# abhineet123/MTF

Measured on AMD Instinct MI355X. Metric: LK iters/sec (warp+grad+Hessian), ESM+SSD+Homography 200x200, higher is better.
Workload: dtype f64; 1 GPU; ESM+SSD+Homography 200x200, 64 independent targets per GPU, full mode, solve+update on device; targets_per_gpu=64, n_pix=40000, channels=1, mode=full, frame=1024x1024 float32, parallelism=replicas x1

## Files before the change

### mtf_amd/csrc/api_track.hip

```cpp
#include "mtfhip_api_internal.h"

extern "C" {

int loop_upload_slab(mtfhip_batch *b, hipStream_t st, bool keep_ncc) {
	const size_t Bt = (size_t)b->B;
	std::memcpy(b->h_stage_b + 45 * sizeof(double) * Bt, b->h_stage_a + 45 * sizeof(double) * Bt, 9 * sizeof(double) * Bt);
	fill_stage(b, b->h_stage_b, nullptr, 1, true);
	if (b->h_stage_b_dev) launch_ingest_host(b->h_stage_b_dev, b->d_slab, b->slab_bytes, st, keep_ncc ? 37 * sizeof(double) * Bt : 0, keep_ncc ? 8 * sizeof(double) * Bt : 0);
	else if (keep_ncc) return fail(MTFHIP_ERR_LOGIC, "track: a held template-initialisation record needs the host-visible staging buffer");
	else HIP_TRY(hipMemcpyAsync(b->d_slab, b->h_stage_b, b->slab_bytes, hipMemcpyHostToDevice, st));
	b->warps_dirty = false;
	return MTFHIP_OK;
}
int loop_lm_state(mtfhip_batch *b, const mtfhip_sm_desc *sm, hipStream_t st, double **lm) {
	if (!b->d_lm) HIP_TRY(hipMalloc(&b->d_lm, sizeof(double) * kLmStride * (size_t)b->B));
	std::vector<double> lm0((size_t)kLmStride * b->B, 0.0);
	for (int t = 0; t < b->B; ++t) lm0[(size_t)kLmStride * t + 1] = sm->lm_delta_init;
	HIP_TRY(hipMemcpyAsync(b->d_lm, lm0.data(), sizeof(double) * lm0.size(), hipMemcpyHostToDevice, st));
	HIP_TRY(hipStreamSynchronize(st));
	*lm = b->d_lm;
	return MTFHIP_OK;
}
bool loop_all_stopped(const mtfhip_sm_desc *sm, int max_passes, int it, const int *d_flags, int n, hipStream_t on, std::vector<int> &h_flags, hipError_t *err) {
	if (!(sm->epsilon > 0) || (it + 1) % 8 != 0 || it + 1 >= max_passes) return false;
	h_flags.resize(n);
	hipError_t e = hipMemcpyAsync(h_flags.data(), d_flags, sizeof(int) * n, hipMemcpyDeviceToHost, on);
	if (e == hipSuccess) e = hipStreamSynchronize(on);
	if (e != hipSuccess) { if (err) *err = e; return false; }
	for (int v : h_flags) if (v) return false;
	return true;
}
int loop_read_back(mtfhip_batch *b, hipStream_t st, unsigned long long pub_seq, int *n_iters, double *corners, const char **h_res) {
	*h_res = b->h_pub;
	if (pub_seq) TRY(wait_host_flag(b, pub_seq));
	else if (b->h_pub_dev) {
		const unsigned long long seq = ++b->acc_seq;
		launch_publish_host(b->d_slab, b->h_pub_dev, b->slab_bytes, b->d_fin_count, b->h_flag_dev, seq, st);
		TRY(wait_host_flag(b, seq));
	} else {
		HIP_TRY(hipMemcpyAsync(b->h_stage_b, b->d_slab, b->slab_bytes, hipMemcpyDeviceToHost, st));
		HIP_TRY(hipStreamSynchronize(st));
		*h_res = b->h_stage_b;
	}
	const size_t Bt = (size_t)b->B;
	const double *p = reinterpret_cast<const double *>(*h_res);
	const double *w = p, *s = p + 9 * Bt, *cr = p + 17 * Bt;
	const int *iters = reinterpret_cast<const int *>(*h_res + b->slab_dbl_bytes) + Bt;
	for (int t = 0; t < b->B; ++t) {
		std::memcpy(b->th[t].warp.m, w + 9 * t, sizeof(double) * 9);
		std::memcpy(b->th[t].state, s + 8 * t, sizeof(double) * 8);
		std::memcpy(b->th[t].corners, cr + 8 * t, sizeof(double) * 8);
		if (n_iters) n_iters[t] = iters[t];
		if (corners) std::memcpy(corners + 8 * t, cr + 8 * t, sizeof(double) * 8);
	}
	return MTFHIP_OK;
}
static int iclk_one_launch_max_pix() {
	static const int v = std::getenv("MTFHIP_ICLK_ONE_LAUNCH_MAX") ? std::atoi(std::getenv("MTFHIP_ICLK_ONE_LAUNCH_MAX")) : 4 * kBlock;
	return v < kIclkTrackMaxPix ? v : kIclkTrackMaxPix;
}
bool iclk_one_launch(const mtfhip_batch *b, const mtfhip_sm_desc *sm) {
	return b->C == 1 && !intensity_mapped(b) && sm->sm == MTFHIP_SM_ICLK && (sm->hess_type == 0 || (sm->hess_type == 2 && b->desc.am == MTFHIP_AM_SSD)) &&
		b->N <= iclk_one_launch_max_pix();
}

static int track_chunk(const mtfhip_batch *b, const mtfhip_sm_desc *sm, const FusedArgs &fa) {
	const char *env_px = std::getenv("MTFHIP_TRACK_CHUNK_PX");
	if (!env_px && !(fa.mode == 1 && fa.materialize)) return b->B;
	const double chunk_px = env_px ? std::atof(env_px) : 2.6e6;
	int chunk = (int)(chunk_px / (double)b->N);
	if (chunk < 1) chunk = 1;
	if (chunk >= b->B || sm->max_iters == 1) return b->B;
	const int n_chunks = (b->B + chunk - 1) / chunk;
	return (b->B + n_chunks - 1) / n_chunks;
}
static int track_queues(const mtfhip_batch *b, const FusedArgs &fa) {
	const char *e_want = std::getenv("MTFHIP_TRACK_STREAMS");
	const int want = e_want ? std::atoi(e_want) : 2;
	if (want < 2 || b->B < 2 || b->d_trace) return 1;
	if (!fa.materialize && want < 12) return 1;
	static const double min_rows = std::getenv("MTFHIP_TRACK_STREAMS_MIN_ROWS") ? std::atof(std::getenv("MTFHIP_TRACK_STREAMS_MIN_ROWS")) : 0.5e6;
	if ((double)b->B * b->N < min_rows && want < 12) return 1;
	return std::min(std::min(want % 10, 4), b->B);
}
int mtfhip_batch_track_targets_per_launch(mtfhip_batch *b, const mtfhip_sm_desc *sm) {
	FLUSH(b);
	if (check_sm(b, sm, "track_targets_per_launch") != MTFHIP_OK) return 0;
	if (iclk_one_launch(b, sm)) return b->B;
	FusedArgs fa;
	if (fused_args(b, sm, fa) != MTFHIP_OK) return 0;
	const int chunk = track_chunk(b, sm, fa), nq = track_queues(b, fa);
	return nq >= 2 ? std::min(chunk, (b->B + nq - 1) / nq) : chunk;
}
int mtfhip_batch_track_queues(mtfhip_batch *b, const mtfhip_sm_desc *sm) {
	FLUSH(b);
	if (check_sm(b, sm, "track_queues") != MTFHIP_OK) return 0;
	if (b->desc.am == MTFHIP_AM_MI) return 1;
	if (iclk_one_launch(b, sm)) return 1;
	FusedArgs fa;
	if (fused_args(b, sm, fa) != MTFHIP_OK) return 0;
	return track_queues(b, fa);
}

static bool track_defers_materialisation(const mtfhip_batch *b, const mtfhip_sm_desc *sm, const FusedArgs &fa, int so_term, bool resume, bool use_step) {
	const char *e = std::getenv("MTFHIP_TRACK_DEFER_MAT");
	if (e && e[0] == '0') return false;
	if (!fa.materialize) return false;
	if (fa.mode == 2) return false;
	if (sm->max_iters < 3) return false;
	if (sm->leven_marq) return false;
	if (b->d_trace) return false;
	if (so_term >= 0) return false;
	if (b->desc.am != MTFHIP_AM_SSD && b->desc.am != MTFHIP_AM_NCC) return false;
	if (b->C != 1) return false;
	if (use_step) return false;
	if (resume) return false;
	return true;
}

static int track_core(mtfhip_batch *b, const mtfhip_sm_desc *sm, int *n_iters, double *corners, bool slab_uploaded, bool resume = false, bool region_mode = false);
static void persist_decomposition(const mtfhip_batch *b, int &nblk, int &rows) {
	fused_decomposition(b->N, b->B, nblk, rows);
	const int per_target = b->ctx->n_cus / b->B;
	if (per_target >= 1 && nblk > per_target) {
		const int total_rows = (b->N + kBlock - 1) / kBlock;
		rows = (total_rows + per_target - 1) / per_target;
		nblk = (total_rows + rows - 1) / rows;
	}
	static const int forced = std::getenv("MTFHIP_PERSIST_NBLK") ? std::atoi(std::getenv("MTFHIP_PERSIST_NBLK")) : 0;
	if (forced > 0 && forced < nblk) {
		const int total_rows = (b->N + kBlock - 1) / kBlock;
		rows = (total_rows + forced - 1) / forced;
		nblk = (total_rows + rows - 1) / rows;
	}
}
static int ensure_persist_words(mtfhip_batch *b, hipStream_t st) {
	if (b->d_persist) return MTFHIP_OK;
	HIP_TRY(hipMalloc(&b->d_persist, 2 * sizeof(int) * (size_t)b->B));
	HIP_TRY(hipMemsetAsync(b->d_persist, 0, 2 * sizeof(int) * (size_t)b->B, st));
	return MTFHIP_OK;
}
static unsigned long long persist_timeout_ticks() {
	const char *e = std::getenv("MTFHIP_PERSIST_TIMEOUT_US");
	const double us = e ? std::atof(e) : 20000.0;
	return (unsigned long long)(us * 100.0);
}
static bool persist_fits(const mtfhip_batch *b, const mtfhip_sm_desc *sm, const FusedArgs &fa) {
	const char *e = std::getenv("MTFHIP_PERSIST");
	if (!(e && e[0] == '1') || !b->persist_ok || fa.materialize || b->ctx->n_cus <= 0 || b->B > b->ctx->n_cus || !b->h_pub_dev) return false;
	if (b->C != 1) return false;
	if (intensity_mapped(b)) return false;
	if (b->B > 8) return false;
	if (sm->max_iters < 2) return false;
	int nblk, rows;
	persist_decomposition(b, nblk, rows);
	return (long)nblk * b->B <= b->ctx->n_cus && nblk <= b->nblk_max;
}
static int lscv_after_track(mtfhip_batch *b, int rc) {
	if (rc == MTFHIP_OK && b && (b->desc.am == MTFHIP_AM_LSCV || b->desc.am == MTFHIP_AM_LRSCV)) b->lscv_first_iter = 0;
	return rc;
}
int mtfhip_batch_track(mtfhip_batch *b, const mtfhip_sm_desc *sm, int *n_iters, double *corners) {
	if (sm && alk_sm(sm->sm)) return alk_track(b, sm, n_iters, corners);
	return lscv_after_track(b, track_core(b, sm, n_iters, corners, false));
}

const bool g_track_dbg_timing = std::getenv("MTFHIP_TRACK_DEBUG_TIMING") != nullptr;
static thread_local std::chrono::steady_clock::time_point g_track_dbg_t[3];
int track_region_impl(mtfhip_batch *b, const mtfhip_sm_desc *sm, const double *region_corners, int *n_iters, double *corners, const mtfhip_grid_desc *grid) {
	if (!b || !sm || !region_corners) return fail(MTFHIP_ERR_INVALID_ARG, "track_region: NULL argument");
	TRY(track_validate(b, sm));
	const bool folded = !region_refreshes(sm);
	const bool dbg = g_track_dbg_timing;
	const char *e_gf = std::getenv("MTFHIP_GRID_FUSED");
	const bool fused_ok = !(e_gf && e_gf[0] == '0');
	const bool region_mode = fused_ok && folded && b->desc.am != MTFHIP_AM_MI && !sm->leven_marq && iclk_one_launch(b, sm) && second_order_term(sm, b->desc.am) < 0 &&
		b->h_stage_a_dev && b->h_pub_dev;
	const auto t0 = std::chrono::steady_clock::now();
	static thread_local std::vector<double> patches;
	bool layout_later = false;
	if (grid) {
		const char *e_ld = std::getenv("MTFHIP_GRID_LAYOUT_DEV");
		layout_later = region_mode && b->desc.ssm != MTFHIP_SSM_HOMOGRAPHY && !grid->dyn_patch_size && !(e_ld && e_ld[0] == '0');
		if (layout_later) {
			M3 Wr;
			if (!rect_to_quad(-0.5, -0.5, 0.5, 0.5, region_corners, Wr)) return fail(MTFHIP_ERR_INVALID_ARG, "grid_layout: degenerate region corners");
			b->deferred_gdesc = *grid;
			std::memcpy(b->deferred_region, region_corners, sizeof(b->deferred_region));
			std::memcpy(b->deferred_region_map, Wr.m, sizeof(b->deferred_region_map));
		} else {
			patches.resize(8 * (size_t)b->B);
			TRY(mtfhip_grid_layout(grid, region_corners, nullptr, patches.data()));
			region_corners = patches.data();
		}
	}
	{
		const int rs = set_region_core(b, layout_later ? nullptr : region_corners, sm, folded, region_mode, layout_later);
		if (rs != MTFHIP_OK) { b->deferred_layout = false; b->deferred_template_check = false; set_corners_finish_deferred(b); return rs; }
	}
	const auto t1 = std::chrono::steady_clock::now();
	const int r = lscv_after_track(b, track_core(b, sm, n_iters, corners, folded, false, region_mode));
	set_corners_finish_deferred(b);
	if (dbg) {
		const auto t2 = std::chrono::steady_clock::now();
		static double acc1 = 0, acc2 = 0, acc3 = 0, acc4 = 0, acc5 = 0, acc6 = 0; static int n = 0;
		auto us = [](std::chrono::steady_clock::time_point a, std::chrono::steady_clock::time_point c) { return std::chrono::duration<double, std::micro>(c - a).count(); };
		acc1 += us(t0, t1); acc2 += us(t1, t2); acc3 += us(t1, g_track_dbg_t[0]); acc4 += us(g_track_dbg_t[0], g_track_dbg_t[1]); acc5 += us(g_track_dbg_t[1], g_track_dbg_t[2]); acc6 += us(g_track_dbg_t[2], t2);
		if (++n % 100 == 0) {
			std::fprintf(stderr, "[track_region] set_region %.1f us, track %.1f us = before the launch %.1f + launch call %.1f + deferred host half %.1f + wait and copy-out %.1f (mean of 100)\n",
				acc1 / 100, acc2 / 100, acc3 / 100, acc4 / 100, acc5 / 100, acc6 / 100);
			acc1 = acc2 = acc3 = acc4 = acc5 = acc6 = 0;
		}
	}
	return r;
}
int mtfhip_batch_track_region(mtfhip_batch *b, const mtfhip_sm_desc *sm, const double *region_corners, int *n_iters, double *corners) {
	return track_region_impl(b, sm, region_corners, n_iters, corners, nullptr);
}

int track_validate(mtfhip_batch *b, const mtfhip_sm_desc *sm) {
	TRY(check_sm(b, sm, "track"));
	if (sm->max_iters <= 0) return fail(MTFHIP_ERR_INVALID_ARG, "track: max_iters must be positive");
	const int so_term = second_order_term(sm, b->desc.am);
	if (b->desc.am == MTFHIP_AM_MI && so_term >= 0 && b->desc.mi_n_bins != 8)
		return fail(MTFHIP_ERR_NOT_IMPLEMENTED, "track: second-order MI Hessians with other than 8 bins go through the per-function entry points");
	if (so_term >= 0 && b->C != 1) return fail(MTFHIP_ERR_NOT_IMPLEMENTED, "track: second-order Hessians of the multi-channel models use the per-function entry points");
	if (so_term > 0 && so_term != 4 && !b->init_pix_hess) return fail(MTFHIP_ERR_LOGIC, "track: init_template was run without sec_ord_hess");
	if (!b->init_pix_vals) return fail(MTFHIP_ERR_LOGIC, "track before init_template");
	if ((b->desc.am == MTFHIP_AM_LSCV || b->desc.am == MTFHIP_AM_LRSCV) && b->lscv_once && sm->leven_marq && sm->sm == MTFHIP_SM_FCLK)
		return fail(MTFHIP_ERR_NOT_IMPLEMENTED, "track: %s once_per_frame with Levenberg-Marquardt FCLK is not available on the device loop (use the per-function entry points)",
			intensity_mapped_name(b));
	return need_image(b);
}
static int track_loop_one_launch(mtfhip_batch *b, const mtfhip_sm_desc *sm, const TrackState &ts, const TrackCtx &cx, unsigned long long &pub_seq) {
	hipStream_t st = b->ctx->stream;
	const BatchView bv = b->view();
	const bool fb_fused = b->fb_fused_req;
	TimedScope tsc(b->ctx, fb_fused ? "grid_fb" : "iclk_track");
	HostPublish pub{nullptr, 0, 0, nullptr, nullptr, 0, 0};
	if (b->h_pub_dev) {
		pub_seq = ++b->acc_seq;
		pub = HostPublish{b->h_pub_dev, b->slab_dbl_bytes, b->B, b->d_fin_count, b->h_flag_dev, pub_seq, publish_fenced()};
	}
	RegionIngest rg{};
	if (cx.region_mode) {
		const double *stage = reinterpret_cast<const double *>(b->h_stage_a_dev);
		rg = region_geometry(b);
		rg.corners = stage + 17 * (size_t)b->B; rg.ncc = stage + 37 * (size_t)b->B;
		rg.d_ncc = b->d_ncc; rg.d_w0 = b->d_w0; rg.d_init_corners_hm = b->d_init_corners_hm;
		if (b->deferred_layout) region_deferred_layout(b, rg);
	}
	const bool dbg_t = g_track_dbg_timing;
	if (dbg_t) g_track_dbg_t[0] = std::chrono::steady_clock::now();
	if (fb_fused) {
		if (cx.region_mode || !pub.host) return fail(MTFHIP_ERR_LOGIC, "track: the one-launch forward-backward frame takes the plain mode with a host record");
		if (!launch_grid_fb(bv, b->ctx->img, b->ctx->prev, *sm, ts, b->d_h0inv, b->d_ncc, b->norm_mult, b->norm_add, b->desc.grad_eps, pub,
				GridFbOut{b->h_fb_dev, b->d_fb, b->fb_fused_reinit ? 1 : 0}, region_geometry(b), st))
			return fail(MTFHIP_ERR_LOGIC, "track: patch too large for the one-launch forward-backward frame");
	} else
		launch_iclk_track(bv, b->ctx->img, *sm, ts, b->d_h0inv, b->d_ncc, b->norm_mult, b->norm_add, b->math_mode == MTFHIP_MATH_FAST, pub, rg, st);
	if (dbg_t) g_track_dbg_t[1] = std::chrono::steady_clock::now();
	set_corners_finish_deferred(b);
	if (dbg_t) g_track_dbg_t[2] = std::chrono::steady_clock::now();
	return MTFHIP_OK;
}
static int track_loop_persist(mtfhip_batch *b, const mtfhip_sm_desc *sm, const FusedArgs &fa, const TrackState &ts, const TrackCtx &cx) {
	hipStream_t st = b->ctx->stream;
	TRY(ensure_persist_words(b, st));
	int nblk_p, rows_p;
	persist_decomposition(b, nblk_p, rows_p);
	FusedArgs fp = fa;
	fp.rows_per_block = rows_p;
	PersistState ps{b->d_persist, reinterpret_cast<unsigned *>(b->d_persist) + b->B, b->persist_gen, persist_timeout_ticks()};
	b->persist_gen += (unsigned)cx.max_passes + 1u;
	TimedScope tsc(b->ctx, "track_persist");
	launch_track_persist(b->view(), b->ctx->img, fp, *sm, ts, b->d_partials, nblk_p, ps, cx.max_passes, st);
	return MTFHIP_OK;
}

struct ChunkRun { BatchView bc; FusedArgs fc, fl; TrackState tc, tl; int nblk_c, t0, nt; double *part; hipStream_t s; bool done; };
static void track_chunk_runs(mtfhip_batch *b, const FusedArgs &fa, const TrackState &ts, int chunk, int n_streams, bool defer, std::vector<ChunkRun> &runs) {
	const BatchView bv = b->view();
	const bool ncc = b->desc.am == MTFHIP_AM_NCC;
	const size_t RL = ncc ? NCC_ACC_COUNT : ACC_COUNT;
	for (int t0 = 0; t0 < b->B; t0 += chunk) {
		const int nt = std::min(chunk, b->B - t0);
		BatchView bc = bv;
		bc.B = nt;
		for (int i = 0; i < MTFHIP_BUF_COUNT; ++i)
			if (bc.buf[i]) bc.buf[i] += (size_t)t0 * b->per_target[i];
		bc.warps += 9 * (size_t)t0; bc.states += 8 * (size_t)t0;
		FusedArgs fc = fa;
		fc.active = fa.active + t0;
		if (fc.w0) fc.w0 += 9 * (size_t)t0;
		TrackState tc{ts.acc + (size_t)t0 * RL, ts.h0 + (size_t)t0 * 64, ts.corners + 8 * (size_t)t0,
			ts.init_corners_hm + 12 * (size_t)t0, ts.active + t0, ts.n_iters + t0, ncc ? ts.ncc + 8 * (size_t)t0 : nullptr,
			ncc ? ts.ncc_tm + 52 * (size_t)t0 : nullptr, 0, ts.lm ? ts.lm + (size_t)kLmStride * t0 : nullptr, nullptr,
			ts.trace ? ts.trace + (size_t)t0 * ts.trace_cap * kTraceStride : nullptr, ts.trace_cap,
			ts.h_extra ? ts.h_extra + (size_t)t0 * b->S * b->S : nullptr, ts.h_extra_scale, ts.fast_finish};
		int nblk_c; { int rows; fused_decomposition(b->N, nt, nblk_c, rows, MTFHIP_SLOTS / n_streams); fc.rows_per_block = rows; }
		if (nblk_c > b->nblk_max) { int rows; fused_decomposition(b->N, nt, nblk_c, rows); fc.rows_per_block = rows; }
		if (fc.rows_per_block < kGridRegenMinRows) fc.grid_regen = 0;
		double *part = b->d_partials + (size_t)t0 * b->nblk_max * RL;
		static const bool serialize = std::getenv("MTFHIP_TRACK_SERIALIZE") && std::getenv("MTFHIP_TRACK_SERIALIZE")[0] == '1';
		const int q = serialize ? n_streams - 1 : (int)(runs.size() % (size_t)n_streams);
		FusedArgs fl = fc;
		fl.materialize = 0; fl.fast_math = 0; fl.grid_regen = 0;
		if (defer) { tc.warp_last = b->d_last_ws + 9 * (size_t)t0; tc.state_last = b->d_last_ws + 9 * (size_t)b->B + 8 * (size_t)t0; tc.need_mat = b->d_need_mat + t0; }
		TrackState tl = tc;
		tl.lean_pass = 1;
		runs.push_back(ChunkRun{bc, fc, fl, tc, tl, nblk_c, t0, nt, part, q == n_streams - 1 ? b->ctx->stream : b->ctx->extra_streams[q], false});
	}
}
static void track_materialise_stopped(mtfhip_batch *b, const ChunkRun &r) {
	BatchView bm = r.bc;
	bm.warps = r.tc.warp_last; bm.states = r.tc.state_last;
	FusedArgs fm = r.fc;
	fm.active = r.tc.need_mat;
	TimedScope tsc(b->ctx, "fused_lk", r.s);
	launch_fused_ssd(bm, b->ctx->img, fm, r.part, r.nblk_c, r.s, nullptr, nullptr);
}
static int track_open_queues(mtfhip_batch *b, int n_streams, double &phase_frac) {
	mtfhip_ctx *c = b->ctx;
	if (n_streams >= 2) {
		if (!c->ev_fork && hipEventCreateWithFlags(&c->ev_fork, hipEventDisableTiming) != hipSuccess) { (void)hipGetLastError(); n_streams = 1; }
		for (int q = 0; q + 1 < n_streams; ++q)
			if (!c->extra_streams[q] && (hipStreamCreateWithFlags(&c->extra_streams[q], hipStreamNonBlocking) != hipSuccess ||
				hipEventCreateWithFlags(&c->ev_join[q], hipEventDisableTiming) != hipSuccess)) { (void)hipGetLastError(); n_streams = 1; break; }
	}
	const char *e_ph = std::getenv("MTFHIP_TRACK_PHASE");
	phase_frac = e_ph ? std::atof(e_ph) : 0.35;
	if (n_streams == 2 && phase_frac > 0) {
		if (!c->d_phase && hipMalloc(&c->d_phase, sizeof(unsigned long long) * 4) != hipSuccess) { (void)hipGetLastError(); c->d_phase = nullptr; }
	}
	return n_streams;
}
struct QueueJoin {
	mtfhip_ctx *c; int n; bool joined = false;
	~QueueJoin() { if (!joined) for (int q = 0; q + 1 < n; ++q) if (c->extra_streams[q]) (void)hipStreamSynchronize(c->extra_streams[q]); }
};
static bool track_takes_step(const mtfhip_batch *b, const FusedArgs &fa, int so_term, int n_streams) {
	const char *e_st = std::getenv("MTFHIP_STEP");
	const char *e_mx = std::getenv("MTFHIP_STEP_MAX_TARGETS");
	const int max_t = e_mx ? std::atoi(e_mx) : 8;
	return (e_st && e_st[0] == '1') && so_term < 0 && !intensity_mapped(b) && n_streams == 1 && b->B <= max_t && track_step_available(b->view(), fa);
}
static int track_chunk_pass(mtfhip_batch *b, const mtfhip_sm_desc *sm, const FusedArgs &fa, const TrackCtx &cx, const ChunkRun &r, int it, bool lean, bool use_step,
	const PhaseCtl &pc) {
	if (use_step) {
		TimedScope tsc(b->ctx, "track_step", r.s);
		launch_track_step(r.bc, b->ctx->img, r.fc, *sm, r.tc, r.part, r.nblk_c, b->d_persist + r.t0, r.s);
		return MTFHIP_OK;
	}
	if (b->desc.am == MTFHIP_AM_SCV) TRY(scv_enqueue(b, r.bc, r.t0, r.fc.active, 0, r.s));
	if (b->desc.am == MTFHIP_AM_LSCV && (!b->lscv_once || it == 0)) TRY(lscv_enqueue(b, r.bc, r.t0, r.fc.active, 0, r.s));
	RscvMap rm;
	if (b->desc.am == MTFHIP_AM_RSCV) TRY(rscv_enqueue(b, r.bc, r.t0, r.fc.active, r.fc, r.s, &rm));
	LrscvMap lm;
	if (b->desc.am == MTFHIP_AM_LRSCV && (!b->lscv_once || it == 0)) TRY(lrscv_enqueue(b, r.bc, r.t0, r.fc.active, r.fc, r.s, &lm));
	{
		TimedScope tsc(b->ctx, "fused_lk", r.s);
		launch_fused_ssd(r.bc, b->ctx->img, lean ? r.fl : r.fc, r.part, r.nblk_c, r.s, &rm, &lm);
	}
	if (cx.so_term >= 0) {
		TimedScope tsc(b->ctx, "second_order", r.s);
		launch_second_order_ssd(r.bc, b->ctx->img, cx.so_term, fa.chained, b->d0_variant, fa.grad_eps, b->hess_eps, b->norm_mult, b->norm_add,
			b->d_d2_part + (size_t)r.t0 * cx.nb2 * 64, cx.nb2, b->d_d2_out + (size_t)r.t0 * b->S * b->S, r.s, 1,
			b->desc.am == MTFHIP_AM_NCC ? SecondOrderNcc{r.part, r.nblk_c, r.tc.ncc} : SecondOrderNcc{nullptr, 0, nullptr});
	}
	TimedScope tsc(b->ctx, "finish_track", r.s);
	launch_finish_track(r.bc, *sm, lean ? r.tl : r.tc, r.part, r.nblk_c, r.s, pc);
	return MTFHIP_OK;
}
static int track_loop_chunked(mtfhip_batch *b, const mtfhip_sm_desc *sm, const FusedArgs &fa, const TrackState &ts, const TrackCtx &cx) {
	hipStream_t st = b->ctx->stream;
	int chunk = track_chunk(b, sm, fa);
	double phase_frac;
	const int n_streams = track_open_queues(b, track_queues(b, fa), phase_frac);
	if (n_streams == 2 && phase_frac > 0 && b->ctx->d_phase) HIP_TRY(hipMemsetAsync(b->ctx->d_phase, 0, sizeof(unsigned long long) * 4, st));
	static const double stagger_env = std::getenv("MTFHIP_TRACK_STAGGER_US") ? std::atof(std::getenv("MTFHIP_TRACK_STAGGER_US")) : -1.0;
	double stagger_us = stagger_env;
	if (stagger_env < 0) stagger_us = 0.25 * ((double)b->B * b->N * 130.0 / 6.5e6 + 8.0) * (2.0 / n_streams);
	const bool use_step = track_takes_step(b, fa, cx.so_term, n_streams);
	if (use_step) TRY(ensure_persist_words(b, st));
	const bool defer = track_defers_materialisation(b, sm, fa, cx.so_term, cx.resume, use_step);
	if (defer) {
		if (!b->d_last_ws) HIP_TRY(hipMalloc(&b->d_last_ws, sizeof(double) * 17 * (size_t)b->B));
		if (!b->d_need_mat) HIP_TRY(hipMalloc(&b->d_need_mat, sizeof(int) * (size_t)b->B));
		HIP_TRY(hipMemsetAsync(b->d_need_mat, 0, sizeof(int) * (size_t)b->B, st));
	}
	if (n_streams >= 2) {
		const int part_sz = (b->B + n_streams - 1) / n_streams;
		if (chunk > part_sz) chunk = part_sz;
		HIP_TRY(hipEventRecord(b->ctx->ev_fork, st));
		for (int q = 0; q + 1 < n_streams; ++q) HIP_TRY(hipStreamWaitEvent(b->ctx->extra_streams[q], b->ctx->ev_fork, 0));
	}
	std::vector<ChunkRun> runs;
	track_chunk_runs(b, fa, ts, chunk, n_streams, defer, runs);
	const auto dbg_t0 = std::chrono::steady_clock::now();
	QueueJoin queue_join{b->ctx, n_streams};
	std::vector<int> h_flags;
	for (size_t g0 = 0; g0 < runs.size(); g0 += (size_t)n_streams) {
		const size_t g1 = std::min(runs.size(), g0 + (size_t)n_streams);
		for (int it = 0; it < cx.max_passes; ++it) {
			bool all_done = true;
			const bool lean = defer && it + 1 < cx.max_passes;
			for (size_t k = g0; k < g1; ++k) {
				ChunkRun &r = runs[k];
				if (r.done) continue;
				if (n_streams >= 2 && it == 0 && k > g0 && stagger_us > 0) launch_queue_delay(stagger_us * (double)(k - g0), r.s);
				PhaseCtl pc{nullptr, nullptr, 0.0};
				if (n_streams == 2 && phase_frac > 0 && b->ctx->d_phase) {
					const int qi = (int)((k - g0) & 1);
					pc = PhaseCtl{b->ctx->d_phase + qi, b->ctx->d_phase + (1 - qi), phase_frac};
				}
				TRY(track_chunk_pass(b, sm, fa, cx, r, it, lean, use_step, pc));
				if (loop_all_stopped(sm, cx.max_passes, it, r.tc.active, r.nt, r.s, h_flags)) r.done = true;
				all_done = all_done && r.done;
			}
			if (all_done) break;
		}
		if (defer && sm->epsilon > 0)
			for (size_t k = g0; k < g1; ++k) track_materialise_stopped(b, runs[k]);
	}
	if (g_track_dbg_timing)
		std::fprintf(stderr, "[track] %d queues, %d passes enqueued in %.1f us\n", n_streams, cx.max_passes,
			std::chrono::duration<double, std::micro>(std::chrono::steady_clock::now() - dbg_t0).count());
	for (int q = 0; q + 1 < n_streams; ++q) {
		HIP_TRY(hipEventRecord(b->ctx->ev_join[q], b->ctx->extra_streams[q]));
		HIP_TRY(hipStreamWaitEvent(st, b->ctx->ev_join[q], 0));
	}
	queue_join.joined = true;
	return MTFHIP_OK;
}

static int track_core(mtfhip_batch *b, const mtfhip_sm_desc *sm, int *n_iters, double *corners, bool slab_uploaded, bool resume, bool region_mode) {
	FLUSH_AM(b);
	TRY(begin_entry(b));
	TRY(track_validate(b, sm));
	TrackCtx cx{second_order_term(sm, b->desc.am), (sm->leven_marq && sm->sm == MTFHIP_SM_FCLK) ? 2 * sm->max_iters : sm->max_iters, 0, resume, region_mode};
	hipStream_t st = b->ctx->stream;
	const bool mi = b->desc.am == MTFHIP_AM_MI, ncc = b->desc.am == MTFHIP_AM_NCC;
	const bool one_launch = !mi && !sm->leven_marq && iclk_one_launch(b, sm) && cx.so_term < 0;
	FusedArgs fa;
	if (!one_launch && !mi) TRY(fused_args(b, sm, fa));
	else { fa.materialize = 0; fa.mode = 2; fa.active = nullptr; fa.rows_per_block = 1; fa.j0_recompute = 0; fa.inline_warp = 0; fa.fast_math = 0; fa.grid_regen = 0; fa.w0 = nullptr; }
	const bool fresh = b->fresh_reinit && one_launch && !region_mode && !slab_uploaded && !resume && b->h_pub_dev && b->d_trace == nullptr;
	b->fresh_reinit = false;
	if (!slab_uploaded && !fresh) TRY(loop_upload_slab(b, st, b->hold_init_pull && b->init_mirror_seq != 0));
	else b->warps_dirty = false;
	fa.active = b->d_active;
	if (ncc && !one_launch && !b->d_ncc_tm) return fail(MTFHIP_ERR_LOGIC, "track before init_template");
	TrackState ts{b->d_acc, b->d_h0, b->d_corners, b->d_init_corners_hm, b->d_active, b->d_iters, ncc ? b->d_ncc : nullptr, ncc ? b->d_ncc_tm : nullptr, 0, nullptr, nullptr,
		b->d_trace, b->trace_cap};
	ts.fresh_reset = fresh ? 1 : 0;
	if (b->d_trace && !resume) HIP_TRY(hipMemsetAsync(b->d_trace, 0, sizeof(double) * kTraceStride * (size_t)b->trace_cap * b->B, st));
	if (mi && b->d_trace) ts.f_ext = b->d_mi_f;
	if (sm->leven_marq) {
		if (resume) ts.lm = b->d_lm;
		else TRY(loop_lm_state(b, sm, st, &ts.lm));
		if (mi) ts.f_ext = b->d_mi_f;
	}
	if (cx.so_term >= 0) {
		cx.nb2 = simple_blocks_per_target(b->N);
		TRY(ensure_second_order_scratch(b));
		ts.h_extra = b->d_d2_out; ts.h_extra_scale = (cx.so_term == 1 || (cx.so_term == 4 && sm->sm == MTFHIP_SM_ESM && sm->hess_type == 2)) ? 0.5 : 1.0;
	}
	{
		const char *e = std::getenv("MTFHIP_FAST_FINISH");
		const bool enabled = !(e && e[0] == '0');
		ts.fast_finish = (enabled && b->math_mode == MTFHIP_MATH_FAST && !ncc && !mi && cx.so_term < 0) ? 1 : 0;
	}
	unsigned long long pub_seq = 0;
	bool persisted = false;
	if (mi) TRY(track_loop_mi(b, sm, ts, cx));
	else if (one_launch) TRY(track_loop_one_launch(b, sm, ts, cx, pub_seq));
	else if ((persisted = cx.so_term < 0 && persist_fits(b, sm, fa))) TRY(track_loop_persist(b, sm, fa, ts, cx));
	else TRY(track_loop_chunked(b, sm, fa, ts, cx));
	const char *h_res;
	TRY(loop_read_back(b, st, pub_seq, n_iters, corners, &h_res));
	const int *act = reinterpret_cast<const int *>(h_res + b->slab_dbl_bytes), *iters = act + b->B;
	if (region_mode)
		for (int t = 0; t < b->B; ++t)
			if (iters[t] < 0) return fail(MTFHIP_ERR_INVALID_ARG, "track_region: degenerate corners for target %d", t);
	if (persisted) {
		bool cut = false;
		for (int t = 0; t < b->B; ++t) cut = cut || act[t] != 0;
		if (cut) {
			b->persist_ok = false;
			HIP_TRY(hipStreamSynchronize(st));
			HIP_TRY(hipMemsetAsync(b->d_persist, 0, 2 * sizeof(int) * (size_t)b->B, st));
			return track_core(b, sm, n_iters, corners, true, true);
		}
	}
	if (!mi) {
		b->it_valid = fa.materialize;
		b->dit_valid = b->jt_valid = fa.materialize && fa.mode != 2;
	}
	loop_done(b);
	return MTFHIP_OK;
}

int mtfhip_batch_track_trace(mtfhip_batch *b, int max_passes) {
	if (!b || max_passes < 0) return fail(MTFHIP_ERR_INVALID_ARG, "track_trace: invalid argument");
	HIP_TRY(hipStreamSynchronize(b->ctx->stream));
	if (b->d_trace) { (void)hipFree(b->d_trace); b->d_trace = nullptr; }
	b->trace_cap = max_passes;
	if (max_passes > 0) {
		HIP_TRY(hipMalloc(&b->d_trace, sizeof(double) * kTraceStride * (size_t)max_passes * b->B));
		HIP_TRY(hipMemsetAsync(b->d_trace, 0, sizeof(double) * kTraceStride * (size_t)max_passes * b->B, b->ctx->stream));
	}
	return MTFHIP_OK;
}
int mtfhip_batch_track_trace_read(mtfhip_batch *b, double *dst) {
	if (!b || !dst) return fail(MTFHIP_ERR_INVALID_ARG, "track_trace_read: NULL argument");
	if (!b->d_trace) return fail(MTFHIP_ERR_LOGIC, "track_trace_read: tracing is off (mtfhip_batch_track_trace)");
	HIP_TRY(hipMemcpyAsync(dst, b->d_trace, sizeof(double) * kTraceStride * (size_t)b->trace_cap * b->B, hipMemcpyDeviceToHost, b->ctx->stream));
	HIP_TRY(hipStreamSynchronize(b->ctx->stream));
	return MTFHIP_OK;
}

}
```

### mtf_amd/csrc/kernels_fused.hip

```cpp
#include "mtfhip_finish_device.h"
#include "mtfhip_fused_device.h"

namespace mtfhip {

template <int SSM, bool CHAINED, int MODE, bool MAT>
__global__ __launch_bounds__(kBlock, MTFHIP_FUSED_WAVES) void k_fused_ssd(BatchView bv, ImgView im, FusedArgs fa, double *partials, int nblk) {
	fused_lk_body<MTFHIP_AM_SSD, SSM, CHAINED, MODE, MAT>(bv, im, fa, partials, nblk);
}
template <int SSM, bool CHAINED, int MODE, bool MAT>
__global__ __launch_bounds__(kBlock, MTFHIP_FUSED_WAVES) void k_fused_ncc(BatchView bv, ImgView im, FusedArgs fa, double *partials, int nblk) {
	fused_lk_body<MTFHIP_AM_NCC, SSM, CHAINED, MODE, MAT>(bv, im, fa, partials, nblk);
}
template <int AM, int SSM, int MODE, bool CHAINED>
__global__ __launch_bounds__(kBlock, MTFHIP_FAST_WAVES) void k_fused_fast(BatchView bv, ImgView im, FusedArgs fa, double *partials, int nblk) {
	fused_lk_body<AM, SSM, CHAINED, MODE, false, true>(bv, im, fa, partials, nblk);
}


__global__ __launch_bounds__(256) void k_finish_track(BatchView bv, mtfhip_sm_desc sm, TrackState ts,
	const double *partials, int nblk, PhaseCtl pc) {
	if (ts.fast_finish) finish_track_fast_body(bv, sm, ts, partials, nblk, blockIdx.x);
	else finish_track_body(bv, sm, ts, partials, nblk, blockIdx.x);
	if (pc.mine && blockIdx.x == 0 && threadIdx.x == 0) {
		const unsigned long long prev = ld_coh(pc.mine), other = ld_coh(pc.other);
		unsigned long long now = wall_clock64();
		if (prev && other && now > prev && now - prev < 50000ull) {
			const unsigned long long min_lag = (unsigned long long)((double)(now - prev) * pc.frac);
			while (now > other && now - other < min_lag) { __builtin_amdgcn_s_sleep(8); now = wall_clock64(); }
		}
		st_coh(pc.mine, now);
	}
}


__global__ __launch_bounds__(64) void k_finish_track_mi(BatchView bv, mtfhip_sm_desc sm, TrackState ts, int sum_std, int gmode,
	const double *mi_H, const double *gpart, int ng, double *rows) {
	const int t = blockIdx.x, lane = threadIdx.x, S = bv.S, B = bv.B;
	const double *Hs = mi_H + 64 * (size_t)t, *H2 = mi_H + 80 * (size_t)B + 64 * (size_t)t;
	double *row = rows + (size_t)t * ACC_COUNT;
	__shared__ double gs[16];
	if (lane < 16) gs[lane] = column_sum(gpart + (size_t)t * ng * 16 + lane, ng, 16);
	if (lane < ACC_COUNT - 36) row[36 + lane] = 0.0;
	const int a = lane >> 3, c = lane & 7;
	if (a <= c) {
		double hv = 0.0;
		if (c < S) { hv = Hs[c * S + a]; if (sum_std) hv = 0.5 * (hv + H2[c * S + a]); }
		row[ACC_H + a * 8 - (a * (a - 1)) / 2 + (c - a)] = -hv;
	}
	__syncthreads();
	if (lane < S) {
		const double gt = gs[lane], g0 = gs[8 + lane];
		row[ACC_G + lane] = gmode == 0 ? g0 : (gmode == 1 ? gt : (gmode == 2 ? 2.0 * gt : gt - g0));
	}
	__syncthreads();
	finish_track_body(bv, sm, ts, rows, 1, t);
}


void launch_fused_ssd(const BatchView &bv, const ImgView &im, const FusedArgs &fa, double *partials, int nblk,
	hipStream_t st, const RscvMap *rm, const LrscvMap *lm) {
	const bool mapped = bv.am == MTFHIP_AM_RSCV ? (rm && rm->map) : (bv.am == MTFHIP_AM_LRSCV && lm && lm->map);
	const FusedKey k = fused_select(FUSED_ROUTE_LOOP, bv.am, bv.C, bv.ssm, fa.mode, fa.chained, fa.materialize, fa.fast_math, mapped);
	if (!k.served) return;
	if (k.am == MTFHIP_AM_RSCV) { launch_fused_rscv(bv, im, fa, partials, nblk, *rm, st); return; }
	if (k.am == MTFHIP_AM_LRSCV) { launch_fused_lrscv(bv, im, fa, partials, nblk, *lm, st); return; }
	if (k.mc) { launch_fused_mc(bv, im, fa, partials, nblk, st); return; }
	const dim3 g = grid2(nblk, bv.B);
	const bool launched = fused_visit<FusedUnit<FUSED_ROUTE_LOOP, false, MTFHIP_AM_SSD, MTFHIP_AM_NCC>>(k, [&](auto AM, auto SSM, auto CH, auto MD, auto MAT, auto FAST) {
		if constexpr (FAST())
			MTFHIP_LAUNCH((k_fused_fast<AM(), SSM(), MD(), CH()>), g, dim3(kBlock), 0, st, bv, im, fa, partials, nblk);
		else if constexpr (AM() == MTFHIP_AM_NCC)
			MTFHIP_LAUNCH((k_fused_ncc<SSM(), CH(), MD(), MAT()>), g, dim3(kBlock), 0, st, bv, im, fa, partials, nblk);
		else {
			const size_t tab = MAT() && fa.grid_regen ? sizeof(double2) * (size_t)(fa.g_resx + fa.g_resy) : 0;
			MTFHIP_LAUNCH((k_fused_ssd<SSM(), CH(), MD(), MAT()>), g, dim3(kBlock), tab, st, bv, im, fa, partials, nblk);
		}
	});
	if (!launched) note_launch_error(hipErrorInvalidDeviceFunction, __FILE__, __LINE__);
}
void launch_finish_track(const BatchView &bv, const mtfhip_sm_desc &sm, const TrackState &ts, const double *partials,
	int nblk, hipStream_t st, PhaseCtl pc) {
	MTFHIP_LAUNCH(k_finish_track, dim3(bv.B), dim3(nblk > 8 ? 256 : (bv.am == MTFHIP_AM_NCC ? 128 : 64)), 0, st, bv, sm, ts, partials, nblk, pc);
}

void launch_finish_track_mi(const BatchView &bv, const mtfhip_sm_desc &sm, const TrackState &ts, int sum_std, int gmode,
	const double *mi_H, const double *gpart, int ng, double *rows, hipStream_t st) {
	MTFHIP_LAUNCH(k_finish_track_mi, dim3(bv.B), dim3(64), 0, st, bv, sm, ts, sum_std, gmode, mi_H, gpart, ng, rows);
}

__global__ void k_kernarg_probe(BatchView bv, ImgView im, FusedArgs fa, double *out) {
	const char *kernarg = (const char *)__builtin_amdgcn_kernarg_segment_ptr();
	const double *kw = reinterpret_cast<const double *>(kernarg + sizeof(BatchView) + sizeof(ImgView) + offsetof(FusedArgs, iw));
	if (threadIdx.x < 17) out[threadIdx.x] = kw[threadIdx.x];
	if (threadIdx.x == 17) out[17] = (double)(bv.B + im.w + fa.mode);
}
bool kernarg_layout_verified(hipStream_t st) {
	static int state = -1;
	if (state >= 0) return state == 1;
	state = 0;
	double *d_out = nullptr;
	if (hipMalloc(&d_out, sizeof(double) * 18) != hipSuccess) { (void)hipGetLastError(); return false; }
	BatchView bv{}; ImgView im{}; FusedArgs fa{};
	bv.B = 1; im.w = 2; fa.mode = 3; fa.inline_warp = 1;
	for (int q = 0; q < 9; ++q) fa.iw[q] = 0.5 + 1.25 * q;
	for (int q = 0; q < 8; ++q) fa.is[q] = -3.0 - 0.75 * q;
	double h[18] = {0};
	hipLaunchKernelGGL(k_kernarg_probe, dim3(1), dim3(64), 0, st, bv, im, fa, d_out);
	bool ok = hipGetLastError() == hipSuccess && hipMemcpyAsync(h, d_out, sizeof(h), hipMemcpyDeviceToHost, st) == hipSuccess &&
		hipStreamSynchronize(st) == hipSuccess;
	(void)hipFree(d_out);
	for (int q = 0; ok && q < 9; ++q) ok = h[q] == fa.iw[q];
	for (int q = 0; ok && q < 8; ++q) ok = h[9 + q] == fa.is[q];
	state = ok ? 1 : 0;
	return ok;
}

#ifdef MTFHIP_FIN_TRACE
void debug_fin_trace(unsigned long long *out) { (void)hipMemcpyFromSymbol(out, HIP_SYMBOL(g_fin_trace), sizeof(unsigned long long) * 16); }
#endif
}
```

### mtf_amd/csrc/kernels_interface.hip

```cpp
#include "mtfhip_device.h"
#include "mtfhip_grid_device.h"

namespace mtfhip {


struct SlabIngest { const uint4 *src; uint4 *dst; unsigned n16; const unsigned *src_tail; unsigned *dst_tail; unsigned n_tail; };
__global__ __launch_bounds__(kBlock) void k_init_grid(BatchView bv, const double *w0_all, int resx, int resy,
	double lo_x, double lo_y, double hi_x, double hi_y, int force_unit_z, SlabIngest ing, int write_curr) {
	const int t = blockIdx.y;
	if (ing.src) {
		const unsigned i = (blockIdx.y * gridDim.x + blockIdx.x) * kBlock + threadIdx.x;
		if (i < ing.n16) ing.dst[i] = ing.src[i];
		if (i < ing.n_tail) ing.dst_tail[i] = ing.src_tail[i];
	}
	const Warp9 W = load_warp(w0_all + 9 * t);
	double2 *ip = reinterpret_cast<double2 *>(bv.buf[MTFHIP_BUF_INIT_PTS]) + (size_t)t * bv.NP;
	double2 *cp = reinterpret_cast<double2 *>(bv.buf[MTFHIP_BUF_CURR_PTS]) + (size_t)t * bv.NP;
	double *iz = bv.buf[MTFHIP_BUF_INIT_Z] + (size_t)t * bv.NP;
	double *cz = bv.buf[MTFHIP_BUF_CURR_Z] + (size_t)t * bv.NP;
	double2 *ih = reinterpret_cast<double2 *>(bv.buf[MTFHIP_BUF_INIT_HXY]) + (size_t)t * bv.NP;
	double2 *ch = reinterpret_cast<double2 *>(bv.buf[MTFHIP_BUF_CURR_HXY]) + (size_t)t * bv.NP;
	for (int i = blockIdx.x * kBlock + threadIdx.x; i < bv.NP; i += gridDim.x * kBlock) {
		const int col = i % resx, row = i / resx;
		const double nx = lattice_coord(col, resx, lo_x, hi_x, (hi_x - lo_x) / (resx - 1)), ny = lattice_coord(row, resy, lo_y, hi_y, (hi_y - lo_y) / (resy - 1));
// ... 154 lines not shown
__global__ __launch_bounds__(kBlock) void k_img_grad_mc(int NP, int C, ImgView im, const double *pts_all, const double *gp_all,
	double *grad_all, double eps, double pix_mult) {
	const int t = blockIdx.y, P = NP * C;
	double *grad = grad_all + (size_t)t * P * 2;
	const double mult = pix_mult / (2 * eps);
	for (int q = blockIdx.x * kBlock + threadIdx.x; q < P; q += gridDim.x * kBlock) {
		const int i = q / C, ch = q % C;
		double ix, dx, iy, dy;
		if (gp_all) {
			const double2 *g = reinterpret_cast<const double2 *>(gp_all + ((size_t)t * NP + i) * 8);
			ix = pix_val_mc(im, g[0].x, g[0].y, ch); dx = pix_val_mc(im, g[1].x, g[1].y, ch);
			iy = pix_val_mc(im, g[2].x, g[2].y, ch); dy = pix_val_mc(im, g[3].x, g[3].y, ch);
		} else {
			const double2 p = (reinterpret_cast<const double2 *>(pts_all) + (size_t)t * NP)[i];
			ix = pix_val_mc(im, p.x + eps, p.y, ch); dx = pix_val_mc(im, p.x - eps, p.y, ch);
			iy = pix_val_mc(im, p.x, p.y + eps, ch); dy = pix_val_mc(im, p.x, p.y - eps, ch);
		}
		grad[q] = (ix - dx) * mult;
		grad[P + q] = (iy - dy) * mult;
	}
}

__global__ __launch_bounds__(kBlock) void k_pix_jacobian(BatchView bv, int variant, const double *grad_all, double *J_all) {
	const int t = blockIdx.y, N = bv.N, S = bv.S, NP = bv.NP, C = bv.C;
	const Warp9 W = load_warp(bv.warps + 9 * t);
	const double *st = bv.states + 8 * t;
	const double2 *ip = reinterpret_cast<const double2 *>(bv.buf[MTFHIP_BUF_INIT_PTS]) + (size_t)t * NP;
	const double2 *cp = reinterpret_cast<const double2 *>(bv.buf[MTFHIP_BUF_CURR_PTS]) + (size_t)t * NP;
	const double *cz = bv.buf[MTFHIP_BUF_CURR_Z] + (size_t)t * NP;
	const double *grad = grad_all + (size_t)t * N * 2;
	double *J = J_all + (size_t)t * N * S;
	for (int i = blockIdx.x * kBlock + threadIdx.x; i < N; i += gridDim.x * kBlock) {
		const int pt = C == 1 ? i : i / C;
		double2 p0 = ip[pt];
		double x = p0.x, y = p0.y;
		double gx = grad[i], gy = grad[N + i];
		double r[8];
		if (bv.ssm == MTFHIP_SSM_HOMOGRAPHY) {
			if (variant == MTFHIP_JAC_INIT) {
				hom_row(r, gx, gy, x, y, x, y);
			} else if (variant == MTFHIP_JAC_PIX) {
				double2 c = cp[pt];
				double inv_d = 1.0 / cz[pt];
				hom_row(r, gx * inv_d, gy * inv_d, x, y, c.x, c.y);
			} else if (variant == MTFHIP_JAC_WARPED) {
				double2 c = cp[pt];
				double inv_det = 1.0 / cz[pt];
				double dwx_dx = (W.m[0] - W.m[6] * c.x), dwx_dy = (W.m[1] - W.m[7] * c.x);
				double dwy_dx = (W.m[3] - W.m[6] * c.y), dwy_dy = (W.m[4] - W.m[7] * c.y);
				double Ix = (dwx_dx * gx + dwy_dx * gy) * inv_det;
				double Iy = (dwx_dy * gx + dwy_dy * gy) * inv_det;
				hom_row(r, Ix, Iy, x, y, x, y);
			} else {
				double2 c = cp[pt];
				double a = (W.m[0] - W.m[6] * c.x), b = (W.m[1] - W.m[7] * c.x);
				double cc = (W.m[3] - W.m[6] * c.y), d = (W.m[4] - W.m[7] * c.y);
				double inv_factor = 1.0 / (a * d - b * cc);
				double Ix = (d * gx - cc * gy) * inv_factor;
				double Iy = (a * gy - b * gx) * inv_factor;
				hom_row(r, Ix, Iy, x, y, c.x, c.y);
			}
		} else {
			double a = st[2] + 1, b = st[3], c = st[4], d = st[5] + 1;
			double Ixx = gx * x, Ixy = gx * y, Iyy = gy * y, Iyx = gy * x;
			if (variant == MTFHIP_JAC_INIT || variant == MTFHIP_JAC_PIX) {
				r[0] = gx; r[1] = gy; r[2] = Ixx; r[3] = Ixy; r[4] = Iyx; r[5] = Iyy;
			} else if (variant == MTFHIP_JAC_WARPED) {
				r[0] = gx * a + gy * c; r[1] = gx * b + gy * d;
				r[2] = Ixx * a + Iyx * c; r[3] = Ixy * a + Iyy * c;
				r[4] = Ixx * b + Iyx * d; r[5] = Ixy * b + Iyy * d;
			} else {
				double inv_det = 1.0 / (a * d - b * c);
				r[0] = (gx * d - gy * c) * inv_det; r[1] = (gy * a - gx * b) * inv_det;
				r[2] = (Ixx * d - Iyx * c) * inv_det; r[3] = (Ixy * d - Iyy * c) * inv_det;
				r[4] = (Iyx * a - Ixx * b) * inv_det; r[5] = (Iyy * a - Ixy * b) * inv_det;
			}
		}
		for (int s = 0; s < S; ++s) J[(size_t)s * N + i] = r[s];
	}
}


__global__ __launch_bounds__(kBlock) void k_mean_jacobian(const double *a, const double *b, double *o, size_t n) {
	for (size_t i = (size_t)blockIdx.x * kBlock + threadIdx.x; i < n; i += (size_t)gridDim.x * kBlock)
		o[i] = (a[i] + b[i]) / 2.0;
}

__global__ __launch_bounds__(kBlock) void k_negate(const double *a, double *o, size_t n) {
	for (size_t i = (size_t)blockIdx.x * kBlock + threadIdx.x; i < n; i += (size_t)gridDim.x * kBlock) o[i] = -a[i];
}



__global__ __launch_bounds__(kBlock) void k_ssd_residual(BatchView bv, double *partials, int nblk) {
	__shared__ double lds[4 * 1];
	const int t = blockIdx.y, N = bv.N;
	const double *It = bv.buf[MTFHIP_BUF_IT] + (size_t)t * N;
	const double *I0 = bv.buf[MTFHIP_BUF_I0] + (size_t)t * N;
	double *r = bv.buf[MTFHIP_BUF_DF_DI0] + (size_t)t * N;
	double acc[1] = {0.0};
	for (int i = blockIdx.x * kBlock + threadIdx.x; i < N; i += nblk * kBlock) {
		double d = It[i] - I0[i];
		r[i] = d;
		acc[0] = fma(d, d, acc[0]);
	}
	block_reduce_store<1>(acc, partials + ((size_t)t * nblk + blockIdx.x) * ACC_COUNT + ACC_RR, lds);
}

__global__ __launch_bounds__(kBlock) void k_gemv(int N, int S, const double *v1_all, const double *J1_all,
	const double *v2_all, const double *J2_all, int sum_mode, double *partials, int nblk) {
	__shared__ double lds[4 * 16];
	const int t = blockIdx.y;
	const double *v1 = v1_all + (size_t)t * N, *J1 = J1_all + (size_t)t * N * S;
	const double *v2 = v2_all ? v2_all + (size_t)t * N : nullptr;
	const double *J2 = J2_all ? J2_all + (size_t)t * N * S : nullptr;
	double acc[16];
#pragma unroll
	for (int k = 0; k < 16; ++k) acc[k] = 0.0;
	for (int i = blockIdx.x * kBlock + threadIdx.x; i < N; i += nblk * kBlock) {
		double a = v1[i];
		double b = v2 ? v2[i] : 0.0;
#pragma unroll
		for (int s = 0; s < kMaxS; ++s) {
			if (s < S) {
				double j1 = J1[(size_t)s * N + i];
				if (J2 && sum_mode) {
					acc[s] = fma(a, j1 + J2[(size_t)s * N + i], acc[s]);
				} else {
					acc[s] = fma(a, j1, acc[s]);
					if (J2) acc[8 + s] = fma(b, J2[(size_t)s * N + i], acc[8 + s]);
				}
			}
		}
	}
	double *dst = partials + ((size_t)t * nblk + blockIdx.x) * ACC_COUNT;
	__shared__ double outv[16];
	block_reduce_store<16>(acc, outv, lds);
	__syncthreads();
	if (threadIdx.x < 8) dst[ACC_G + threadIdx.x] = outv[threadIdx.x];
	else if (threadIdx.x < 16) dst[ACC_G2 + threadIdx.x - 8] = outv[threadIdx.x];
}

__global__ __launch_bounds__(kBlock) void k_gram(int N, int S, const double *J_all, double *partials, int nblk) {
	__shared__ double lds[4 * 36];
	const int t = blockIdx.y;
	const double *J = J_all + (size_t)t * N * S;
	double acc[36];
#pragma unroll
	for (int k = 0; k < 36; ++k) acc[k] = 0.0;
	for (int i = blockIdx.x * kBlock + threadIdx.x; i < N; i += nblk * kBlock) {
		double r[kMaxS];
#pragma unroll
		for (int s = 0; s < kMaxS; ++s) r[s] = s < S ? J[(size_t)s * N + i] : 0.0;
		int k = 0;
#pragma unroll
		for (int a = 0; a < kMaxS; ++a)
#pragma unroll
			for (int b = a; b < kMaxS; ++b) { acc[k] = fma(r[a], r[b], acc[k]); ++k; }
	}
	block_reduce_store<36>(acc, partials + ((size_t)t * nblk + blockIdx.x) * ACC_COUNT + ACC_H, lds);
}

enum { NCC_I0_MEAN = 0, NCC_C = 1, NCC_IT_MEAN = 2, NCC_B = 3, NCC_F = 4, NCC_GMEAN = 5, NCC_SC = 8 };

__global__ __launch_bounds__(kBlock) void k_vec_sum(int N, const double *v_all, double *partials, int nblk) {
	__shared__ double lds[4];
	const int t = blockIdx.y;
	const double *v = v_all + (size_t)t * N;
	double acc[1] = {0.0};
	for (int i = blockIdx.x * kBlock + threadIdx.x; i < N; i += nblk * kBlock) acc[0] += v[i];
	block_reduce_store<1>(acc, partials + ((size_t)t * nblk + blockIdx.x) * ACC_COUNT + ACC_RR, lds);
}
__global__ __launch_bounds__(kBlock) void k_ncc_centered(BatchView bv, const double *sc_all, double *partials, int nblk) {
	__shared__ double lds[4 * 4];
	__shared__ double outv[4];
	const int t = blockIdx.y, N = bv.N;
	const double *I0 = bv.buf[MTFHIP_BUF_I0] + (size_t)t * N, *It = bv.buf[MTFHIP_BUF_IT] + (size_t)t * N;
	const double m0 = sc_all[t * NCC_SC + NCC_I0_MEAN], mt = sc_all[t * NCC_SC + NCC_IT_MEAN];
	double acc[4] = {0, 0, 0, 0};
	for (int i = blockIdx.x * kBlock + threadIdx.x; i < N; i += nblk * kBlock) {
		const double a0 = I0[i] - m0, at = It[i] - mt;
		acc[0] = fma(a0, at, acc[0]); acc[1] = fma(at, at, acc[1]); acc[2] = fma(a0, a0, acc[2]);
	}
	block_reduce_store<4>(acc, outv, lds);
	__syncthreads();
	if (threadIdx.x < 3) partials[((size_t)t * nblk + blockIdx.x) * ACC_COUNT + ACC_G + threadIdx.x] = outv[threadIdx.x];
}
__global__ __launch_bounds__(kBlock) void k_ncc_grad(BatchView bv, const double *sc_all, int curr, double *out_all,
	double *partials, int nblk) {
	__shared__ double lds[4];
	const int t = blockIdx.y, N = bv.N;
	const double *I0 = bv.buf[MTFHIP_BUF_I0] + (size_t)t * N, *It = bv.buf[MTFHIP_BUF_IT] + (size_t)t * N;
	double *out = out_all + (size_t)t * N;
	const double *sc = sc_all + t * NCC_SC;
	const double m0 = sc[NCC_I0_MEAN], c = sc[NCC_C], mt = sc[NCC_IT_MEAN], b = sc[NCC_B], f = sc[NCC_F];
	double acc[1] = {0.0};
	for (int i = blockIdx.x * kBlock + threadIdx.x; i < N; i += nblk * kBlock) {
		const double i0c_c = (I0[i] - m0) / c, itc_b = (It[i] - mt) / b;
		const double v = curr ? (i0c_c - f * itc_b) / b : (itc_b - f * i0c_c) / c;
		out[i] = v;
		acc[0] += v;
	}
	block_reduce_store<1>(acc, partials + ((size_t)t * nblk + blockIdx.x) * ACC_COUNT + ACC_RR, lds);
}
__global__ __launch_bounds__(kBlock) void k_sub_mean(int N, double *v_all, const double *sc_all) {
	const int t = blockIdx.y;
	double *v = v_all + (size_t)t * N;
	const double m = sc_all[t * NCC_SC + NCC_GMEAN];
	for (int i = blockIdx.x * kBlock + threadIdx.x; i < N; i += gridDim.x * kBlock) v[i] -= m;
}
__global__ __launch_bounds__(kBlock) void k_col_sum(int N, int S, const double *J_all, double *partials, int nblk) {
	__shared__ double lds[4 * 8];
	__shared__ double outv[8];
	const int t = blockIdx.y;
	const double *J = J_all + (size_t)t * N * S;
	double acc[8] = {0, 0, 0, 0, 0, 0, 0, 0};
	for (int i = blockIdx.x * kBlock + threadIdx.x; i < N; i += nblk * kBlock) {
#pragma unroll
		for (int s = 0; s < kMaxS; ++s)
			if (s < S) acc[s] += J[(size_t)s * N + i];
	}
	block_reduce_store<8>(acc, outv, lds);
	__syncthreads();
	if (threadIdx.x < 8) partials[((size_t)t * nblk + blockIdx.x) * ACC_COUNT + ACC_G + threadIdx.x] = outv[threadIdx.x];
}
__global__ __launch_bounds__(kBlock) void k_ncc_hess(BatchView bv, const double *sc_all, const double *colmean_all,
	const double *J_all, double *partials, int nblk) {
	__shared__ double lds[4 * 52];
	__shared__ double outv[52];
	const int t = blockIdx.y, N = bv.N, S = bv.S;
	const double *J = J_all + (size_t)t * N * S;
	const double *I0 = bv.buf[MTFHIP_BUF_I0] + (size_t)t * N, *It = bv.buf[MTFHIP_BUF_IT] + (size_t)t * N;
	const double *sc = sc_all + t * NCC_SC, *cm = colmean_all + t * 8;
	const double m0 = sc[NCC_I0_MEAN], c = sc[NCC_C], mt = sc[NCC_IT_MEAN], b = sc[NCC_B];
	double acc[52];
#pragma unroll
	for (int k = 0; k < 52; ++k) acc[k] = 0.0;
	for (int i = blockIdx.x * kBlock + threadIdx.x; i < N; i += nblk * kBlock) {
		const double i0c_c = (I0[i] - m0) / c, itc_b = (It[i] - mt) / b;
		double r[kMaxS];
#pragma unroll
		for (int s = 0; s < kMaxS; ++s) r[s] = s < S ? (J[(size_t)s * N + i] - cm[s]) / b : 0.0;
		int k = 0;
#pragma unroll
		for (int a = 0; a < kMaxS; ++a)
#pragma unroll
			for (int b2 = a; b2 < kMaxS; ++b2) { acc[k] = fma(r[a], r[b2], acc[k]); ++k; }
#pragma unroll
		for (int s = 0; s < kMaxS; ++s) { acc[36 + s] = fma(r[s], itc_b, acc[36 + s]); acc[44 + s] = fma(r[s], i0c_c, acc[44 + s]); }
	}
	block_reduce_store<52>(acc, outv, lds);
	__syncthreads();
	double *dst = partials + ((size_t)t * nblk + blockIdx.x) * ACC_COUNT;
	if (threadIdx.x < 44) dst[threadIdx.x] = outv[threadIdx.x];
	else if (threadIdx.x < 52) dst[ACC_G2 + threadIdx.x - 44] = outv[threadIdx.x];
}


__global__ __launch_bounds__(128) void k_finish_rows(const double *partials, int nblk, int row_len, double *out) {
	const int t = blockIdx.x, k = blockIdx.y * 128 + threadIdx.x;
	if (k >= row_len) return;
	out[(size_t)t * row_len + k] = column_sum(partials + (size_t)t * nblk * row_len + k, nblk, row_len);
}
__device__ __forceinline__ void publish_arrive(int *count, unsigned long long *flag_host, unsigned long long seq, int fenced) {
	if (fenced) __builtin_amdgcn_fence(__ATOMIC_RELEASE, "agent"); else wait_stores_acked();
	__syncthreads();
	if (threadIdx.x == 0) {
		const int done = fenced ? __hip_atomic_fetch_add(count, 1, __ATOMIC_ACQ_REL, __HIP_MEMORY_SCOPE_AGENT)
		                        : __hip_atomic_fetch_add(count, 1, __ATOMIC_RELAXED, __HIP_MEMORY_SCOPE_AGENT);
		if (done == (int)gridDim.x - 1) {
			__hip_atomic_store(count, 0, __ATOMIC_RELAXED, __HIP_MEMORY_SCOPE_AGENT);
			if (fenced) { __threadfence_system(); __hip_atomic_store(flag_host, seq, __ATOMIC_RELEASE, __HIP_MEMORY_SCOPE_SYSTEM); }
			else __hip_atomic_store(flag_host, seq, __ATOMIC_RELAXED, __HIP_MEMORY_SCOPE_SYSTEM);
		}
	}
}
__global__ __launch_bounds__(1024) void k_finish_host(const double *partials, int nblk, int row_len, double *out_host, int *count,
	unsigned long long *flag_host, unsigned long long seq, int fenced) {
	__shared__ double part[8][128];
	const int t = blockIdx.x, k = threadIdx.x & 127, j = threadIdx.x >> 7, G = blockDim.x >> 7;
	const double *p = partials + (size_t)t * nblk * row_len;
	double mine = 0.0;
	if (k < row_len && j < nblk) mine = column_sum(p + (size_t)j * row_len + k, (nblk - j + G - 1) / G, G * row_len);
	if (G > 1) {
		part[j][k] = mine;
		__syncthreads();
		if (j == 0) for (int g = 1; g < G; ++g) mine += part[g][k];
	}
	if (j == 0 && k < row_len) __hip_atomic_store(out_host + (size_t)t * row_len + k, mine, __ATOMIC_RELAXED, __HIP_MEMORY_SCOPE_SYSTEM);
	publish_arrive(count, flag_host, seq, fenced);
}
__global__ __launch_bounds__(256) void k_publish_host(const unsigned *src, unsigned *dst_host, unsigned n_words, int *count,
	unsigned long long *flag_host, unsigned long long seq, int fenced) {
	for (unsigned i = blockIdx.x * 256 + threadIdx.x; i < n_words; i += gridDim.x * 256)
		__hip_atomic_store(dst_host + i, src[i], __ATOMIC_RELAXED, __HIP_MEMORY_SCOPE_SYSTEM);
	publish_arrive(count, flag_host, seq, fenced);
}
__global__ __launch_bounds__(256) void k_ingest_host(const uint4 *src_host, uint4 *dst, unsigned n16, const unsigned *src_tail, unsigned *dst_tail, unsigned n_tail,
	unsigned skip_lo, unsigned skip_hi) {
	const unsigned i = blockIdx.x * 256 + threadIdx.x;
	if (i < n16 && !(i >= skip_lo && i < skip_hi)) dst[i] = src_host[i];
	if (i < n_tail) dst_tail[i] = src_tail[i];
}
__global__ __launch_bounds__(64) void k_finish(const double *partials, int nblk, double *out) {
	const int t = blockIdx.x, k = threadIdx.x;
	if (k >= ACC_COUNT) return;
	const double *p = partials + (size_t)t * nblk * ACC_COUNT + k;
	double s0 = 0, s1 = 0, s2 = 0, s3 = 0;
	int b = 0;
	for (; b + 3 < nblk; b += 4) {
		s0 += p[(size_t)b * ACC_COUNT]; s1 += p[(size_t)(b + 1) * ACC_COUNT];
		s2 += p[(size_t)(b + 2) * ACC_COUNT]; s3 += p[(size_t)(b + 3) * ACC_COUNT];
	}
	for (; b < nblk; ++b) s0 += p[(size_t)b * ACC_COUNT];
	out[(size_t)t * ACC_COUNT + k] = (s0 + s1) + (s2 + s3);
}


__global__ void k_queue_delay(unsigned long long ticks) {
	const unsigned long long t0 = wall_clock64();
	while (wall_clock64() - t0 < ticks) __builtin_amdgcn_s_sleep(8);
}
void launch_queue_delay(double microseconds, hipStream_t st) {
	static double ticks_per_us = 0;
	if (ticks_per_us == 0) {
		int dev = 0, khz = 0;
		if (hipGetDevice(&dev) != hipSuccess || hipDeviceGetAttribute(&khz, hipDeviceAttributeWallClockRate, dev) != hipSuccess || khz <= 0) { (void)hipGetLastError(); khz = 100000; }
		ticks_per_us = khz / 1000.0;
	}
	if (microseconds <= 0) return;
	MTFHIP_LAUNCH(k_queue_delay, dim3(1), dim3(64), 0, st, (unsigned long long)(microseconds * ticks_per_us));
}

void launch_init_grid(const BatchView &bv, const double *dev_w0, int resx, int resy, double lo_x, double lo_y,
	double hi_x, double hi_y, int force_unit_z, hipStream_t st) {
	MTFHIP_LAUNCH(k_init_grid, grid2(simple_blocks_per_target(bv.N), bv.B), dim3(kBlock), 0, st, bv, dev_w0, resx, resy,
		lo_x, lo_y, hi_x, hi_y, force_unit_z, SlabIngest{nullptr, nullptr, 0, nullptr, nullptr, 0}, 1);
}
bool launch_init_grid_ingest(const BatchView &bv, const double *host_w0_dev, int resx, int resy, double lo_x, double lo_y,
	double hi_x, double hi_y, int force_unit_z, const void *src_host, void *dst, size_t bytes, int write_curr, hipStream_t st) {
	const unsigned n16 = (unsigned)(bytes / 16), n_tail = (unsigned)((bytes % 16) / 4);
	const dim3 g = grid2(simple_blocks_per_target(bv.N), bv.B);
	if ((size_t)g.x * g.y * kBlock < std::max(n16, n_tail)) return false;
	const SlabIngest ing{static_cast<const uint4 *>(src_host), static_cast<uint4 *>(dst), n16,
		reinterpret_cast<const unsigned *>(static_cast<const char *>(src_host) + 16 * (size_t)n16),
		reinterpret_cast<unsigned *>(static_cast<char *>(dst) + 16 * (size_t)n16), n_tail};
	MTFHIP_LAUNCH(k_init_grid, g, dim3(kBlock), 0, st, bv, host_w0_dev, resx, resy, lo_x, lo_y, hi_x, hi_y, force_unit_z, ing, write_curr);
	return true;
}
void launch_apply_warp(const BatchView &bv, hipStream_t st) {
	MTFHIP_LAUNCH(k_apply_warp, grid2(simple_blocks_per_target(bv.N), bv.B), dim3(kBlock), 0, st, bv);
}
void launch_grad_pts(const BatchView &bv, double eps, hipStream_t st) {
	MTFHIP_LAUNCH(k_grad_pts, grid2(simple_blocks_per_target(bv.N), bv.B), dim3(kBlock), 0, st, bv, eps);
}
void launch_sample(const BatchView &bv, const ImgView &im, const double *pts, double *out, double mult, double add,
	hipStream_t st) {
	if (bv.C > 1) { MTFHIP_LAUNCH(k_sample_mc, grid2(simple_blocks_per_target(bv.N), bv.B), dim3(kBlock), 0, st, bv.NP, bv.C, im, pts, out, mult, add); return; }
	MTFHIP_LAUNCH(k_sample, grid2(simple_blocks_per_target(bv.N), bv.B), dim3(kBlock), 0, st, bv.N, im, pts, out, mult, add);
}
void launch_update_model(const BatchView &bv, const ImgView &im, const double *pts, double *I0, double mult, double add,
	double frame_count, double alpha, int running_avg, hipStream_t st) {
	MTFHIP_LAUNCH(k_update_model, grid2(simple_blocks_per_target(bv.N), bv.B), dim3(kBlock), 0, st, bv.N, im, pts, I0, mult, add,
		frame_count, alpha, running_avg);
}
void launch_img_grad(const BatchView &bv, const ImgView &im, const double *pts, double *grad, double eps, double mult,
	hipStream_t st) {
	if (bv.C > 1) {
		MTFHIP_LAUNCH(k_img_grad_mc, grid2(simple_blocks_per_target(bv.N), bv.B), dim3(kBlock), 0, st, bv.NP, bv.C, im, pts, (const double *)nullptr, grad, eps, mult);
		return;
	}
	MTFHIP_LAUNCH(k_img_grad, grid2(simple_blocks_per_target(bv.N), bv.B), dim3(kBlock), 0, st, bv.N, im, pts, grad, eps, mult);
}
void launch_warped_img_grad(const BatchView &bv, const ImgView &im, const double *gp, double *grad, double eps,
	double mult, hipStream_t st) {
	if (bv.C > 1) {
		MTFHIP_LAUNCH(k_img_grad_mc, grid2(simple_blocks_per_target(bv.N), bv.B), dim3(kBlock), 0, st, bv.NP, bv.C, im, (const double *)nullptr, gp, grad, eps, mult);
		return;
	}
	MTFHIP_LAUNCH(k_warped_img_grad, grid2(simple_blocks_per_target(bv.N), bv.B), dim3(kBlock), 0, st, bv.N, im, gp, grad, eps, mult);
}
void launch_pix_jacobian(const BatchView &bv, int variant, const double *grad, double *J, hipStream_t st) {
	MTFHIP_LAUNCH(k_pix_jacobian, grid2(simple_blocks_per_target(bv.N), bv.B), dim3(kBlock), 0, st, bv, variant, grad, J);
}
void launch_mean_jacobian(const BatchView &bv, hipStream_t st) {
	size_t n = (size_t)bv.B * bv.N * bv.S;
	int nb = (int)((n + kBlock * 4 - 1) / (kBlock * 4));
	MTFHIP_LAUNCH(k_mean_jacobian, dim3(nb), dim3(kBlock), 0, st, bv.buf[MTFHIP_BUF_J0], bv.buf[MTFHIP_BUF_JT],
		bv.buf[MTFHIP_BUF_JM], n);
}
void launch_negate(const double *src, double *dst, size_t n, hipStream_t st) {
	int nb = (int)((n + kBlock * 4 - 1) / (kBlock * 4));
	MTFHIP_LAUNCH(k_negate, dim3(nb), dim3(kBlock), 0, st, src, dst, n);
}
void launch_ssd_residual(const BatchView &bv, double *partials, int nblk, hipStream_t st) {
	MTFHIP_LAUNCH(k_ssd_residual, grid2(nblk, bv.B), dim3(kBlock), 0, st, bv, partials, nblk);
}
void launch_gemv(const BatchView &bv, const double *v1, const double *J1, const double *v2, const double *J2,
	int sum_mode, double *partials, int nblk, hipStream_t st) {
	MTFHIP_LAUNCH(k_gemv, grid2(nblk, bv.B), dim3(kBlock), 0, st, bv.N, bv.S, v1, J1, v2, J2, sum_mode, partials, nblk);
}
void launch_gram(const BatchView &bv, const double *J, double *partials, int nblk, hipStream_t st) {
	MTFHIP_LAUNCH(k_gram, grid2(nblk, bv.B), dim3(kBlock), 0, st, bv.N, bv.S, J, partials, nblk);
}
void launch_vec_sum(const BatchView &bv, const double *v, double *partials, int nblk, hipStream_t st) {
	MTFHIP_LAUNCH(k_vec_sum, grid2(nblk, bv.B), dim3(kBlock), 0, st, bv.N, v, partials, nblk);
}
void launch_ncc_centered(const BatchView &bv, const double *sc, double *partials, int nblk, hipStream_t st) {
	MTFHIP_LAUNCH(k_ncc_centered, grid2(nblk, bv.B), dim3(kBlock), 0, st, bv, sc, partials, nblk);
}
void launch_ncc_grad(const BatchView &bv, const double *sc, int curr, double *out, double *partials, int nblk, hipStream_t st) {
	MTFHIP_LAUNCH(k_ncc_grad, grid2(nblk, bv.B), dim3(kBlock), 0, st, bv, sc, curr, out, partials, nblk);
}
void launch_sub_mean(const BatchView &bv, double *v, const double *sc, hipStream_t st) {
	MTFHIP_LAUNCH(k_sub_mean, grid2(simple_blocks_per_target(bv.N), bv.B), dim3(kBlock), 0, st, bv.N, v, sc);
}
void launch_col_sum(const BatchView &bv, const double *J, double *partials, int nblk, hipStream_t st) {
	MTFHIP_LAUNCH(k_col_sum, grid2(nblk, bv.B), dim3(kBlock), 0, st, bv.N, bv.S, J, partials, nblk);
}
void launch_ncc_hess(const BatchView &bv, const double *sc, const double *colmean, const double *J, double *partials,
	int nblk, hipStream_t st) {
	MTFHIP_LAUNCH(k_ncc_hess, grid2(nblk, bv.B), dim3(kBlock), 0, st, bv, sc, colmean, J, partials, nblk);
}
void launch_finish_host(double *partials, int nblk, int row_len, double *out_host, int *count, unsigned long long *flag_host,
	unsigned long long seq, int B, hipStream_t st) {
	const int G = nblk >= 256 ? 8 : (nblk >= 64 ? 4 : 1);
	MTFHIP_LAUNCH(k_finish_host, dim3(B), dim3(128 * G), 0, st, partials, nblk, row_len, out_host, count, flag_host, seq, publish_fenced());
}
void launch_publish_host(const void *src, void *dst_host, size_t bytes, int *count, unsigned long long *flag_host,
	unsigned long long seq, hipStream_t st) {
	const unsigned n_words = (unsigned)(bytes / 4);
	const unsigned blocks = std::max(1u, std::min(64u, (n_words + 1023) / 1024));
	MTFHIP_LAUNCH(k_publish_host, dim3(blocks), dim3(256), 0, st, static_cast<const unsigned *>(src), static_cast<unsigned *>(dst_host),
		n_words, count, flag_host, seq, publish_fenced());
}
void launch_ingest_host(const void *src_host, void *dst, size_t bytes, hipStream_t st, size_t skip_off, size_t skip_len) {
	const unsigned n16 = (unsigned)(bytes / 16), n_tail = (unsigned)((bytes % 16) / 4);
	const unsigned blocks = std::max(1u, (std::max(n16, n_tail) + 255) / 256);
	MTFHIP_LAUNCH(k_ingest_host, dim3(blocks), dim3(256), 0, st, static_cast<const uint4 *>(src_host), static_cast<uint4 *>(dst), n16,
		reinterpret_cast<const unsigned *>(static_cast<const char *>(src_host) + 16 * (size_t)n16),
		reinterpret_cast<unsigned *>(static_cast<char *>(dst) + 16 * (size_t)n16), n_tail, (unsigned)(skip_off / 16), (unsigned)((skip_off + skip_len) / 16));
}
void launch_finish_rows(double *partials, int nblk, int row_len, double *out, int B, hipStream_t st) {
	MTFHIP_LAUNCH(k_finish_rows, dim3(B, (row_len + 127) / 128), dim3(128), 0, st, partials, nblk, row_len, out);
}
void launch_finish(double *partials, int nblk, double *out, int B, hipStream_t st) {
	MTFHIP_LAUNCH(k_finish, dim3(B), dim3(64), 0, st, partials, nblk, out);
}

void launch_mean_planes(const double *a, const double *b, double *o, size_t n, hipStream_t st) {
	MTFHIP_LAUNCH(k_mean_jacobian, dim3((unsigned)std::min<size_t>((n + kBlock - 1) / kBlock, 4096)), dim3(kBlock), 0, st, a, b, o, n);
}

}
```

### mtf_amd/csrc/mtfhip_api_internal.h

```cpp
#ifndef MTFHIP_API_INTERNAL_H
#define MTFHIP_API_INTERNAL_H
#include "mtfhip_internal.h"

#include <algorithm>
#include <chrono>
#include <thread>
#include <cmath>
#include <cstdarg>
#include <cstdio>
#include <cstdlib>
#include <cstring>
#include <map>
#include <string>
#include <vector>

using namespace mtfhip;

namespace mtfhip {
void launch_init_grid(const BatchView &bv, const double *dev_w0, int resx, int resy, double lo_x, double lo_y,
	double hi_x, double hi_y, int force_unit_z, hipStream_t st);
}

extern thread_local std::string g_last_error;
static int fail(int code, const char *fmt, ...) {
// ... 287 lines not shown
	return MTFHIP_OK;
}

static void fill_stage(const mtfhip_batch *b, char *stage, const double *w0 , int active, bool zero_iters) {
	const size_t Bt = (size_t)b->B;
	double *p = reinterpret_cast<double *>(stage);
	double *w = p, *s = p + 9 * Bt, *cr = p + 17 * Bt, *ic = p + 25 * Bt, *nc = p + 37 * Bt, *pw0 = p + 45 * Bt;
	int *act = reinterpret_cast<int *>(stage + b->slab_dbl_bytes), *it = act + Bt;
	for (int t = 0; t < b->B; ++t) {
		const TargetHost &h = b->th[t];
		std::memcpy(w + 9 * t, h.warp.m, sizeof(double) * 9);
		std::memcpy(s + 8 * t, h.state, sizeof(double) * 8);
		std::memcpy(cr + 8 * t, h.corners, sizeof(double) * 8);
		std::memcpy(ic + 12 * t, h.init_corners_hm, sizeof(double) * 12);
		double *q = nc + 8 * t;
		q[0] = h.I0_mean; q[1] = h.c; q[2] = h.It_mean; q[3] = h.b; q[4] = h.f; q[5] = h.gmean; q[6] = q[7] = 0;
		if (w0) std::memcpy(pw0 + 9 * t, w0 + 9 * t, sizeof(double) * 9);
		act[t] = active;
		if (zero_iters) it[t] = 0;
	}
}

static int push_warps(mtfhip_batch *b) {
	const int k = b->wflip; b->wflip ^= 1;
	HIP_TRY(hipEventSynchronize(b->ev_w[k]));
	double *w = b->h_wstage[k], *s = w + 9 * (size_t)b->B;
	for (int t = 0; t < b->B; ++t) {
		std::memcpy(&w[9 * t], b->th[t].warp.m, sizeof(double) * 9);
		std::memcpy(&s[8 * t], b->th[t].state, sizeof(double) * 8);
	}
	HIP_TRY(hipMemcpyAsync(b->d_warps, w, sizeof(double) * 17 * (size_t)b->B, hipMemcpyHostToDevice, b->ctx->stream));
	HIP_TRY(hipEventRecord(b->ev_w[k], b->ctx->stream));
	return MTFHIP_OK;
}

static inline bool ssd_like(const mtfhip_batch *b) {
	return b->desc.am == MTFHIP_AM_SSD || b->desc.am == MTFHIP_AM_SCV || b->desc.am == MTFHIP_AM_RSCV || b->desc.am == MTFHIP_AM_LSCV ||
		b->desc.am == MTFHIP_AM_LRSCV;
}
static inline bool intensity_mapped(const mtfhip_batch *b) {
	return b->desc.am == MTFHIP_AM_SCV || b->desc.am == MTFHIP_AM_RSCV || b->desc.am == MTFHIP_AM_LSCV || b->desc.am == MTFHIP_AM_LRSCV;
}
static inline const char *intensity_mapped_name(const mtfhip_batch *b) {
	return b->desc.am == MTFHIP_AM_SCV ? "SCV" : (b->desc.am == MTFHIP_AM_RSCV ? "RSCV" : (b->desc.am == MTFHIP_AM_LSCV ? "LSCV" : "LRSCV"));
}
int scv_capture(mtfhip_batch *b);
int scv_enqueue(mtfhip_batch *b, const BatchView &bv, int t0, const int *active, int from_it, hipStream_t st);
int scv_refuse(const mtfhip_batch *b, const char *fn, int sec_ord_hess);
int rscv_capture(mtfhip_batch *b);
int rscv_enqueue(mtfhip_batch *b, const BatchView &bv, int t0, const int *active, const FusedArgs &fa, hipStream_t st, RscvMap *rm);
int rscv_update_pix_vals(mtfhip_batch *b, const double *dp);
int rscv_it_kind(const FusedArgs *fa);
int lscv_capture(mtfhip_batch *b);
int lscv_enqueue(mtfhip_batch *b, const BatchView &bv, int t0, const int *active, int from_it, hipStream_t st);
static inline bool lscv_due(const mtfhip_batch *b) { return b->desc.am == MTFHIP_AM_LSCV && !(b->lscv_once && !b->lscv_first_iter); }
int lscv_check_geometry(const mtfhip_batch *b, int nx, int ny, int sx, int sy, const char *fn);
int lscv_geometry(mtfhip_batch *b, size_t map_lds_budget);
int lrscv_capture(mtfhip_batch *b);
int lrscv_enqueue(mtfhip_batch *b, const BatchView &bv, int t0, const int *active, const FusedArgs &fa, hipStream_t st, LrscvMap *lm);
int lrscv_update_pix_vals(mtfhip_batch *b, const double *dp);
static inline bool lrscv_due(const mtfhip_batch *b) { return b->desc.am == MTFHIP_AM_LRSCV && !(b->lscv_once && !b->lscv_first_iter); }
static inline BatchView fused_view(mtfhip_batch *b, FusedArgs &fa) {
	fa.inline_warp = 0;
	if (b->warps_dirty && b->B == 1) {
		b->warps_dirty = false;
		fa.inline_warp = 1;
		std::memcpy(fa.iw, b->th[0].warp.m, sizeof(double) * 9);
		std::memcpy(fa.is, b->th[0].state, sizeof(double) * 8);
		return b->view_raw();
	}
	return b->view();
}
static void update_corners(mtfhip_batch *b, int t) {
	TargetHost &h = b->th[t];
	for (int q = 0; q < 4; ++q) {
		const double *c = &h.init_corners_hm[3 * q];
		const double *W = h.warp.m;
		double x = W[0] * c[0] + W[1] * c[1] + W[2] * c[2];
		double y = W[3] * c[0] + W[4] * c[1] + W[5] * c[2];
		if (b->desc.ssm == MTFHIP_SSM_HOMOGRAPHY) {
			double d = W[6] * c[0] + W[7] * c[1] + W[8] * c[2];
			x = x / d; y = y / d;
		}
		h.corners[2 * q] = x; h.corners[2 * q + 1] = y;
	}
}

int launch_error_pending();
static inline void cpu_relax() {
#if defined(__x86_64__) || defined(__i386__)
	__builtin_ia32_pause();
#elif defined(__aarch64__)
	__asm__ __volatile__("yield");
#endif
}
static int wait_host_flag(mtfhip_batch *b, unsigned long long seq) {
	TRY(launch_error_pending());
	const auto t0 = std::chrono::steady_clock::now();
	bool yielding = false;
	for (unsigned spins = 0;; ++spins) {
		if (__atomic_load_n(b->h_flag, __ATOMIC_ACQUIRE) == seq) return MTFHIP_OK;
		if (yielding) std::this_thread::yield(); else cpu_relax();
		if ((spins & 0x3ff) == 0x3ff || yielding) {
			const auto dt = std::chrono::steady_clock::now() - t0;
			if (dt > std::chrono::milliseconds(50)) break;
			if (dt > std::chrono::microseconds(1000)) yielding = true;
		}
	}
	HIP_TRY(hipStreamSynchronize(b->ctx->stream));
	if (__atomic_load_n(b->h_flag, __ATOMIC_ACQUIRE) == seq) return MTFHIP_OK;
	return fail(MTFHIP_ERR_HIP, "device results were not delivered to host memory");
}
static int pull_init_mirrors(mtfhip_batch *b) {
	if (!b->init_mirror_seq) return MTFHIP_OK;
	const bool ncc_am = b->desc.am == MTFHIP_AM_NCC;
	if (b->init_rec_device) {
		static thread_local std::vector<double> h0v, ncv, tmv;
		const size_t Bt = (size_t)b->B;
		h0v.resize(64 * Bt); ncv.resize(8 * Bt); tmv.resize(52 * Bt);
		HIP_TRY(hipMemcpyAsync(h0v.data(), b->d_h0, sizeof(double) * 64 * Bt, hipMemcpyDeviceToHost, b->ctx->stream));
		if (ncc_am) {
			HIP_TRY(hipMemcpyAsync(ncv.data(), b->d_ncc, sizeof(double) * 8 * Bt, hipMemcpyDeviceToHost, b->ctx->stream));
			HIP_TRY(hipMemcpyAsync(tmv.data(), b->d_ncc_tm, sizeof(double) * 52 * Bt, hipMemcpyDeviceToHost, b->ctx->stream));
		}
		HIP_TRY(hipStreamSynchronize(b->ctx->stream));
		for (int t = 0; t < b->B; ++t) {
			TargetHost &h = b->th[t];
			std::memcpy(h.h0, &h0v[64 * (size_t)t], sizeof(double) * 64);
			if (ncc_am) {
				const double *r = &ncv[8 * (size_t)t], *m = &tmv[52 * (size_t)t];
				h.I0_mean = r[0]; h.c = r[1]; h.It_mean = r[2]; h.b = r[3]; h.f = r[4]; h.gmean = r[5];
				std::memcpy(h.ncc_sj0, m, sizeof(double) * 8);
				std::memcpy(h.ncc_i0j0, m + 8, sizeof(double) * 8);
				std::memcpy(h.ncc_gram0, m + 16, sizeof(double) * 36);
			}
		}
		b->init_mirror_seq = 0; b->init_rec_device = false;
		return MTFHIP_OK;
	}
	const unsigned long long seq = b->init_mirror_seq;
	const auto t0 = std::chrono::steady_clock::now();
	bool ok = false;
	for (unsigned spins = 0;; ++spins) {
		if (__atomic_load_n(b->h_init_flag, __ATOMIC_ACQUIRE) == seq) { ok = true; break; }
		cpu_relax();
		if ((spins & 0x3ff) == 0x3ff && std::chrono::steady_clock::now() - t0 > std::chrono::milliseconds(50)) break;
	}
	if (!ok) {
		HIP_TRY(hipStreamSynchronize(b->ctx->stream));
		if (__atomic_load_n(b->h_init_flag, __ATOMIC_ACQUIRE) != seq) return fail(MTFHIP_ERR_HIP, "the template initialisation's results were not delivered to host memory");
	}
	const bool ncc = b->desc.am == MTFHIP_AM_NCC;
	for (int t = 0; t < b->B; ++t) {
		const double *r = b->h_init_rec + (size_t)t * mtfhip::kInitRec;
		TargetHost &h = b->th[t];
		std::memcpy(h.h0, r, sizeof(double) * 64);
		if (ncc) {
			h.I0_mean = r[64]; h.c = r[65]; h.It_mean = r[66]; h.b = r[67]; h.f = r[68]; h.gmean = r[69];
			std::memcpy(h.ncc_sj0, r + 72, sizeof(double) * 8);
			std::memcpy(h.ncc_i0j0, r + 80, sizeof(double) * 8);
			std::memcpy(h.ncc_gram0, r + 88, sizeof(double) * 36);
		}
	}
	b->init_mirror_seq = 0;
	return MTFHIP_OK;
}
static int read_rows(mtfhip_batch *b, int nblk, int row_len) {
	if (b->h_acc_dev) {
		const unsigned long long seq = ++b->acc_seq;
		launch_finish_host(b->d_partials, nblk, row_len, b->h_acc_dev, b->d_fin_count, b->h_flag_dev, seq, b->B, b->ctx->stream);
		return wait_host_flag(b, seq);
	}
	if (row_len == ACC_COUNT) launch_finish(b->d_partials, nblk, b->d_acc, b->B, b->ctx->stream);
	else launch_finish_rows(b->d_partials, nblk, row_len, b->d_acc, b->B, b->ctx->stream);
	HIP_TRY(hipMemcpyAsync(b->h_acc, b->d_acc, sizeof(double) * row_len * b->B, hipMemcpyDeviceToHost, b->ctx->stream));
	HIP_TRY(hipStreamSynchronize(b->ctx->stream));
	return MTFHIP_OK;
}
static int read_acc(mtfhip_batch *b, int nblk) { return read_rows(b, nblk, ACC_COUNT); }

static int need_image(mtfhip_batch *b) {
	if (!b->ctx->img.data) return fail(MTFHIP_ERR_LOGIC, "no current image: call mtfhip_image_upload/borrow first");
	if (b->ctx->img.channels != b->C)
		return fail(MTFHIP_ERR_INVALID_ARG, "ImageBase::setCurrImg::Input image has %d channel(s), the appearance model expects %d", b->ctx->img.channels, b->C);
	return MTFHIP_OK;
}
static int single_channel(const mtfhip_batch *b, const char *fn) {
	if (b->C != 1) return fail(MTFHIP_ERR_NOT_IMPLEMENTED, "%s: multi-channel appearance models use the per-function entry points", fn);
	return MTFHIP_OK;
}
static int j_buf_ok(int id) { return id == MTFHIP_BUF_J0 || id == MTFHIP_BUF_JT || id == MTFHIP_BUF_JM; }

static int resolve_pts(mtfhip_batch *b, const double *host, int own_buf, size_t per_target, const double **out) {
	if (!host) {
		if (!b->buf[own_buf]) return fail(MTFHIP_ERR_LOGIC, "device points not available yet");
		*out = b->buf[own_buf];
		return MTFHIP_OK;
	}
	HIP_TRY(hipMemcpyAsync(b->d_scratch_pts, host, sizeof(double) * per_target * b->B, hipMemcpyHostToDevice, b->ctx->stream));
	*out = b->d_scratch_pts;
	return MTFHIP_OK;
}

extern "C" {

static inline void touch(mtfhip_batch *b, int id) { ++b->lz.ver[id]; }
static inline void touch_all(mtfhip_batch *b) { for (int i = 0; i < MTFHIP_BUF_COUNT; ++i) ++b->lz.ver[i]; }
int lazy_flush(mtfhip_batch *b, bool pts = true);
int ensure_df(mtfhip_batch *b);
static inline int begin_entry(mtfhip_batch *b) {
	if (b) { touch_all(b); b->lz.it_epoch = -1; TRY(ensure_df(b)); }
	return MTFHIP_OK;
}
static int ensure_one(mtfhip_batch *b, bool curr);
void stale_clear(mtfhip_batch *b, bool df0, bool dft);
int protect_stale(mtfhip_batch *b, bool w0, bool wt);
int lazy_try_similarity(mtfhip_batch *b);
int do_cmpt_pix_jacobian(mtfhip_batch *b, int variant, int grad_buf, int dst_buf);
static int do_mean_jacobian(mtfhip_batch *b);
static int lazy_flush_ctx(mtfhip_ctx *c) {
	for (mtfhip_batch *b : c->batches) {
		const bool hold = b->hold_init_pull;
		if (!b->lz.any()) b->hold_init_pull = true;
		const int rc = lazy_flush(b, false);
		b->hold_init_pull = hold;
		if (rc) return rc;
		++b->lz.epoch;
	}
	return MTFHIP_OK;
}
#define FLUSH(b) do { if (b) { int _rc = lazy_flush(b); if (_rc) return _rc; } } while (0)
#define FLUSH_AM(b) do { if (b) { int _rc = lazy_flush(b, false); if (_rc) return _rc; } } while (0)

static inline mtfhip::MiJ0Rebuild mi_j0_rebuild(const mtfhip_batch *b) {
	mtfhip::MiJ0Rebuild rb{nullptr, nullptr, nullptr, 0, 0};
	const bool ok = b->C == 1 && b->j0_is_template && b->j0_recompute_enabled && b->j0_template_corners_epoch == b->corners_epoch &&
		b->buf[MTFHIP_BUF_DI0_DX] && b->buf[MTFHIP_BUF_INIT_PTS] && (b->unit_z || b->buf[MTFHIP_BUF_INIT_Z]);
	if (ok) {
		rb.dI0 = b->buf[MTFHIP_BUF_DI0_DX]; rb.pts = b->buf[MTFHIP_BUF_INIT_PTS];
		rb.z = b->unit_z ? nullptr : b->buf[MTFHIP_BUF_INIT_Z];
		rb.hom = b->desc.ssm == MTFHIP_SSM_HOMOGRAPHY; rb.init_variant = b->j0_variant == MTFHIP_JAC_INIT;
	}
	return rb;
}

static inline mtfhip::RegionIngest region_geometry(const mtfhip_batch *b) {
	const bool homg = b->desc.ssm == MTFHIP_SSM_HOMOGRAPHY;
	mtfhip::RegionIngest rg{};
	rg.lo_x = homg ? -0.5 : 1 - b->desc.resx / 2.0; rg.lo_y = homg ? -0.5 : 1 - b->desc.resy / 2.0;
	rg.hi_x = homg ? 0.5 : b->desc.resx / 2.0; rg.hi_y = homg ? 0.5 : b->desc.resy / 2.0;
	rg.resx = b->desc.resx; rg.resy = b->desc.resy; rg.force_unit_z = homg ? 0 : 1;
	return rg;
}
static inline void region_deferred_layout(const mtfhip_batch *b, mtfhip::RegionIngest &rg) {
	const mtfhip_grid_desc &gd = b->deferred_gdesc;
	rg.layout = 1;
	rg.grid = mtfhip::GridLayoutHD{gd.grid_size_x, gd.grid_size_y, gd.patch_size_x, gd.patch_size_y, gd.dyn_patch_size ? 1 : 0, gd.patch_centroid_inside ? 1 : 0};
	std::memcpy(rg.region_map, b->deferred_region_map, sizeof(rg.region_map));
}

enum { LAZY_CURR_JAC = 0, LAZY_DIFF_JAC = 1, LAZY_INIT_JAC = 2 };
int ensure_pts(mtfhip_batch *b);
const float *ensure_pair_image(mtfhip_ctx *c);
const float *pair_image_if_it_pays(mtfhip_ctx *c, int n_candidates);
int set_corners_core(mtfhip_batch *b, const double *corners, bool for_track, bool defer_grid = false, bool layout_later = false);
void set_corners_finish_deferred(mtfhip_batch *b);
int do_update_grad_pts(mtfhip_batch *b, double grad_eps);
int gemv_to_host(mtfhip_batch *b, const double *v1, int j1, const double *v2, int j2, int sum_mode, double *g, int diff);
int mi_blocks(const mtfhip_batch *b);
int push_ncc(mtfhip_batch *b);
int ncc_template_moments(mtfhip_batch *b);
int ncc_lazy_outputs(mtfhip_batch *b, int trig, int j_a, bool hess_mean, double *g);
int ncc_hessian_from_cache(mtfhip_batch *b, int j_buf, int kind, double *H);
int ncc_assemble(const mtfhip_batch *b, const mtfhip_sm_desc *sm, bool hess_mean, const double *M, TargetHost &h, double *f, double *g, double *H);
void ncc_refresh_mirrors(const mtfhip_batch *b, TargetHost &h, const double *M);
int check_sm(const mtfhip_batch *b, const mtfhip_sm_desc *sm, const char *fn);
bool template_init_fused_ok(const mtfhip_batch *b, const mtfhip_sm_desc *sm);
int init_template_fused(mtfhip_batch *b, const mtfhip_sm_desc *sm, const mtfhip::RegionIngest *rg = nullptr, bool publish_host = true);
int set_region_core(mtfhip_batch *b, const double *corners, const mtfhip_sm_desc *sm, bool for_track, bool defer_grid = false, bool layout_later = false);
static inline bool region_refreshes(const mtfhip_sm_desc *sm) { return sm->sm == MTFHIP_SM_ESM || (sm->sm == MTFHIP_SM_FCLK && sm->hess_type == 0); }
int fused_args(const mtfhip_batch *b, const mtfhip_sm_desc *sm, FusedArgs &fa);
int second_order_term(const mtfhip_sm_desc *sm, int am = MTFHIP_AM_SSD);
void assemble(const mtfhip_batch *b, const mtfhip_sm_desc *sm, const double *acc, const double *h0, double *f, double *g, double *H);
int assemble_rows(mtfhip_batch *b, const mtfhip_sm_desc *sm, bool hess_mean, int nblk, const double *so, double so_scale, double *f, double *g, double *H);
int store_h0(mtfhip_batch *b, const double *H0, bool with_inverse);
struct MiPlan {
	enum { H_CONST, H_SELF_JT, H_CURR_JT, H_CURR_JM, H_SUM_STD, H_INIT_J0 };
	int hk;
	bool iclk, esm, fclk, self, need_jt, orig_jac, need_mean;
	explicit MiPlan(const mtfhip_sm_desc *sm) {
		iclk = sm->sm == MTFHIP_SM_ICLK; esm = sm->sm == MTFHIP_SM_ESM; fclk = sm->sm == MTFHIP_SM_FCLK;
		const int ht = sm->hess_type;
		hk = ht == 0 ? H_CONST
			: esm ? (ht <= 2 ? H_SELF_JT : (ht == 3 ? H_CURR_JM : (ht == 4 ? H_SUM_STD : H_CURR_JT)))
			: fclk ? (ht == 1 ? H_SELF_JT : H_CURR_JT)
			: (ht == 1 ? H_SELF_JT : H_INIT_J0);
		self = hk == H_SELF_JT;
		need_jt = !iclk || self;
		orig_jac = esm && sm->jac_type == 0;
		need_mean = orig_jac || hk == H_CURR_JM;
	}
};
int mi_iterate(mtfhip_batch *b, const mtfhip_sm_desc *sm, double *f, double *g, double *H);
struct TrackCtx { int so_term, max_passes, nb2; bool resume, region_mode; };
int track_loop_mi(mtfhip_batch *b, const mtfhip_sm_desc *sm, mtfhip::TrackState &ts, const TrackCtx &cx);
int loop_upload_slab(mtfhip_batch *b, hipStream_t st, bool keep_ncc);
int loop_lm_state(mtfhip_batch *b, const mtfhip_sm_desc *sm, hipStream_t st, double **lm);
bool loop_all_stopped(const mtfhip_sm_desc *sm, int max_passes, int it, const int *d_flags, int n, hipStream_t on, std::vector<int> &h_flags, hipError_t *err = nullptr);
int loop_read_back(mtfhip_batch *b, hipStream_t st, unsigned long long pub_seq, int *n_iters, double *corners, const char **h_res);
static inline void loop_done(mtfhip_batch *b) {
	b->pts_stale = true;
	b->stage_a_busy = false;
}
bool iclk_one_launch(const mtfhip_batch *b, const mtfhip_sm_desc *sm);
int track_validate(mtfhip_batch *b, const mtfhip_sm_desc *sm);
int track_region_impl(mtfhip_batch *b, const mtfhip_sm_desc *sm, const double *region_corners, int *n_iters, double *corners, const mtfhip_grid_desc *grid);
extern const bool g_track_dbg_timing;
static inline bool alk_sm(int sm) { return sm == MTFHIP_SM_FALK || sm == MTFHIP_SM_IALK; }
int alk_init_template(mtfhip_batch *b, const mtfhip_sm_desc *sm);
int alk_iterate(mtfhip_batch *b, const mtfhip_sm_desc *sm, double *f, double *g, double *H);
int alk_track(mtfhip_batch *b, const mtfhip_sm_desc *sm, int *n_iters, double *corners);
int nn_dataset_enqueue(mtfhip_batch *b, const mtfhip_nn_desc *d, const double *dev_perturbations_in, double *dev_perturbations_out, double *dev_features,
	int row_lo, int row_count, const double *base_dev, const int *done);
int score_block_dev(mtfhip_batch *b, const double *dev_states, int lo, int cnt, double *wts, double *sim, int likelihood_func,
	double measurement_sigma, double max_similarity, const mtfhip::PfPeerPush *peer = nullptr);
int refuse_intensity_mapped(const mtfhip_batch *b, const char *fn, const char *what);
}
#endif
```

### mtf_amd/csrc/mtfhip_finish_device.h

```cpp
#ifndef MTFHIP_FINISH_DEVICE_H
#define MTFHIP_FINISH_DEVICE_H
#include "mtfhip_device.h"

namespace mtfhip {

#ifdef MTFHIP_FIN_TRACE
__device__ unsigned long long g_fin_trace[16];
#define FIN_STAMP(k) do { if (t == 0 && threadIdx.x == 0) g_fin_trace[k] = clock64(); } while (0)
#else
#define FIN_STAMP(k) do { } while (0)
#endif

template <bool COH = false, bool ADDITIVE = false>
__device__ __forceinline__ void finish_track_body(const BatchView &bv, const mtfhip_sm_desc &sm, const TrackState &ts,
	const double *partials, int nblk, int t) {
	auto LD = [](const double *p) -> double { if constexpr (COH) return ld_coh(p); else return *p; };
	auto LDI = [](const int *p) -> int { if constexpr (COH) return ld_coh(p); else return *p; };
	auto ST = [](double *p, double v) { if constexpr (COH) st_coh(p, v); else *p = v; };
	auto STI = [](int *p, int v) { if constexpr (COH) st_coh(p, v); else *p = v; };
	auto stop_target = [&](const double *w_old, const double *s_old) {
		STI(ts.active + t, 0);
		if (ts.lean_pass) {
			for (int q = 0; q < 9; ++q) ST(ts.warp_last + 9 * t + q, w_old[q]);
			for (int q = 0; q < 8; ++q) ST(ts.state_last + 8 * t + q, s_old[q]);
			STI(ts.need_mat + t, 1);
		}
	};
	FIN_STAMP(0);
	__shared__ double acc_s[NCC_ACC_COUNT];
	__shared__ double A[8][9];
	__shared__ double dps[8];
	__shared__ double h0s[64], Ws[9], crs[8], ics[12], tms[52], ncs[2], sos[8];
	const int lane = threadIdx.x;
	const bool wv0 = lane < 64;
	const int S = bv.S;
	const bool ncc = bv.am == MTFHIP_AM_NCC;
	const int RL = ncc ? (int)NCC_ACC_COUNT : (int)ACC_COUNT;
	const int act = LDI(ts.active + t);
	const int n_it_prev = LDI(ts.n_iters + t);
	double v_h0 = 0, v_w = 0, v_cr = 0, v_ic = 0, v_acc = 0, v_tm = 0, v_nc = 0, v_so = 0;
	if (wv0) {
		v_h0 = ts.h0[(size_t)t * 64 + lane];
		if (lane < 9) v_w = LD(bv.warps + 9 * t + lane);
		if ((ADDITIVE || ts.lean_pass) && lane < 8) v_so = LD(bv.states + 8 * t + lane);
		if (lane < 8) v_cr = LD(ts.corners + 8 * t + lane);
		if (lane < 12) v_ic = ts.init_corners_hm[12 * t + lane];
		if (ncc) {
			if (lane < 52) v_tm = ts.ncc_tm[(size_t)t * 52 + lane];
			if (lane < 2) v_nc = ts.ncc[(size_t)t * 8 + lane];
		}
	}
	__shared__ double part_s[3][80];
	const int n_runs = (nblk > 8 && blockDim.x >= 240) ? 3 : 1;
	const int run_len = n_runs == 1 ? nblk : ((nblk + 3 * 8 - 1) / (3 * 8)) * 8;
	{
		const int run = n_runs == 1 ? 0 : lane / 80, col = n_runs == 1 ? lane : lane % 80;
		if (col < RL && run < n_runs) {
			const int b0 = run * run_len, b1 = (b0 + run_len < nblk) ? b0 + run_len : nblk;
			const double *p = partials + (size_t)t * nblk * RL + col;
			auto ld = [&](size_t off) -> double { return LD(p + off); };
			double s0 = 0, s1 = 0, s2 = 0, s3 = 0, s4 = 0, s5 = 0, s6 = 0, s7 = 0;
			int b = b0;
			for (; b + 7 < b1; b += 8) {
				s0 += ld((size_t)b * RL); s1 += ld((size_t)(b + 1) * RL);
				s2 += ld((size_t)(b + 2) * RL); s3 += ld((size_t)(b + 3) * RL);
				s4 += ld((size_t)(b + 4) * RL); s5 += ld((size_t)(b + 5) * RL);
				s6 += ld((size_t)(b + 6) * RL); s7 += ld((size_t)(b + 7) * RL);
			}
			for (; b < b1; ++b) s0 += ld((size_t)b * RL);
			const double v = ((s0 + s1) + (s2 + s3)) + ((s4 + s5) + (s6 + s7));
			if (n_runs == 1) v_acc = v; else part_s[run][col] = v;
		}
	}
	if (!act) return;
	FIN_STAMP(1);
	if (wv0) {
		h0s[lane] = v_h0;
		if (lane < 9) Ws[lane] = v_w;
		if (lane < 8) { crs[lane] = v_cr; sos[lane] = v_so; }
		if (lane < 12) ics[lane] = v_ic;
		if (lane < 52) tms[lane] = v_tm;
		if (lane < 2) ncs[lane] = v_nc;
	}
	if (n_runs > 1) {
		__syncthreads();
		if (lane < RL) v_acc = (part_s[0][lane] + part_s[1][lane]) + part_s[2][lane];
	}
	if (lane < RL) { acc_s[lane] = v_acc; ST(ts.acc + (size_t)t * RL + lane, v_acc); }
	__syncthreads();
	FIN_STAMP(2);
	const int i = (lane >> 3) & 7, j = lane & 7;
	double *lmp = ts.lm ? ts.lm + (size_t)t * kLmStride : nullptr;
	double lm_delta = 0.0;
	int lm_iter_id = n_it_prev;
	bool undo = false;
	if (lmp) {
		const double f_now = ts.f_ext ? LD(ts.f_ext + t) : (ncc ? 0.0 : -acc_s[ACC_RR] / 2);
		const double prev_f = LD(lmp + 0);
		lm_delta = LD(lmp + 1);
		const bool state_reset = LD(lmp + 2) != 0.0;
		lm_iter_id = (int)LD(lmp + 3);
		double f_use = f_now;
		if (ncc) {
			const double nN0 = (double)bv.N, mt0 = acc_s[NCC_IT] / nN0, b20 = acc_s[NCC_IT2] - nN0 * mt0 * mt0;
			f_use = (acc_s[NCC_I0IT] - nN0 * ncs[0] * mt0) / (sqrt(b20) * ncs[1]);
		}
		if (!state_reset) {
			if (lm_iter_id > 0) {
				if (f_use < prev_f) { lm_delta *= sm.lm_delta_update; undo = true; }
				else if (f_use > prev_f) lm_delta /= sm.lm_delta_update;
			}
		}
		__syncthreads();
		if (lane == 0) {
			ST(lmp + 1, lm_delta);
			if (undo) ST(lmp + 2, 1.0);
			else { ST(lmp + 2, 0.0); if (!state_reset) ST(lmp + 0, f_use); }
		}
	}
	const bool use_h0 = (sm.hess_type == 0) || (sm.sm == MTFHIP_SM_ICLK && !ts.h_from_acc);
	const bool sum_h0 = (sm.sm == MTFHIP_SM_ESM) && (sm.hess_type == 2 || (sm.hess_type == 4 && !ts.h_from_acc));
	const double gscale = (sm.sm == MTFHIP_SM_ESM) ? 0.5 : 1.0;
	const double nN = (double)bv.N;
	const double n_mt = ncc ? acc_s[NCC_IT] / nN : 0.0, n_m0 = ncs[0], n_c = ncc ? ncs[1] : 1.0;
	const double n_b2 = ncc ? acc_s[NCC_IT2] - nN * n_mt * n_mt : 1.0, n_b = ncc ? sqrt(n_b2) : 1.0;
	const double n_f = ncc ? (acc_s[NCC_I0IT] - nN * n_m0 * n_mt) / (n_b * n_c) : 0.0;
	auto mom = [&](int which, int c0, int ct, int s) -> double {
		const double v0 = c0 >= 0 ? tms[c0 + s] : acc_s[NCC_ITJ0 + s], vt = acc_s[ct + s];
		return which == 0 ? v0 : (which == 1 ? vt : (v0 + vt) / 2);
	};
	auto n_ut = [&](int which, int s) { return (mom(which, -1, NCC_ITJ, s) - n_mt * mom(which, 0, NCC_SJ, s)) / n_b2; };
	auto n_u0 = [&](int which, int s) { return (mom(which, 8, NCC_I0J, s) - n_m0 * mom(which, 0, NCC_SJ, s)) / (n_b * n_c); };
	auto n_hess = [&](int kind, int which, int r, int c, int kk) -> double {
		const double gram = which == 0 ? tms[16 + kk] : acc_s[NCC_GRAM + kk];
		const double G = -(gram - mom(which, 0, NCC_SJ, r) * mom(which, 0, NCC_SJ, c) / nN) / n_b2;
		const double utr = n_ut(which, r), utc = n_ut(which, c);
		if (kind == 2) return G + utr * utc;
		const double u0r = n_u0(which, r), u0c = n_u0(which, c);
		return n_f * G - utr * u0c - u0r * utc + 3 * (kind == 1 ? utr * utc : u0r * u0c);
	};
	auto h_entry = [&](int r, int c) -> double {
		if (r >= S || c >= S) return r == c ? -1.0 : 0.0;
		const int a = r < c ? r : c, b2 = r < c ? c : r;
		const int kk = a * 8 - (a * (a - 1)) / 2 + (b2 - a);
		if (ncc) {
			const int ht = sm.hess_type;
			const double h0v = h0s[b2 * S + a];
			const double ex = ts.h_extra ? ts.h_extra_scale * ts.h_extra[(size_t)t * S * S + c * S + r] : 0.0;
			if (ht == 0) return h0v;
			if (sm.sm == MTFHIP_SM_ICLK) return n_hess(0, 0, r, c, kk) + ex;
			if (sm.sm == MTFHIP_SM_FCLK || ht == 1 || ht == 5) return n_hess(ht == 1 ? 2 : 1, 1, r, c, kk) + ex;
			if (ht == 2) return 0.5 * (n_hess(2, 1, r, c, kk) + h0v);
			if (ht == 3) return n_hess(1, 2, r, c, kk) + ex;
			return 0.5 * (n_hess(0, 0, r, c, kk) + n_hess(1, 1, r, c, kk)) + ex;
		}
		double v = use_h0 ? h0s[c * S + r] : -acc_s[ACC_H + kk];
		if (sum_h0) v = (v + h0s[c * S + r]) * 0.5;
		if (ts.h_extra) v += ts.h_extra_scale * ts.h_extra[(size_t)t * S * S + c * S + r];
		return v;
	};
	auto g_entry = [&](int s) -> double {
		if (!ncc) return gscale * acc_s[ACC_G + s];
		auto cj = [&](int which) { return n_u0(which, s) - n_f * n_ut(which, s); };
		auto ij = [&](int which) { return (n_b / n_c) * (n_ut(which, s) - n_f * n_u0(which, s)); };
		if (sm.sm == MTFHIP_SM_FCLK) return cj(1);
		if (sm.sm == MTFHIP_SM_ICLK) return ij(0);
		if (sm.jac_type == 0) return cj(2);
		return 0.5 * (cj(1) - ij(0));
	};
	auto pow2_scale = [](double d) -> double { return d != 0 ? ldexp(1.0, -(ilogb(fabs(d)) / 2)) : 1.0; };
	const bool pivoting = ncc || ts.h_from_acc || ts.h_extra != nullptr;
	const double si = pow2_scale(h_entry(i, i)), sj = pow2_scale(h_entry(j, j));
	double *trec = (ts.trace && n_it_prev < ts.trace_cap) ? ts.trace + ((size_t)t * ts.trace_cap + n_it_prev) * kTraceStride : nullptr;
	if (wv0) {
		const double hij = h_entry(i, j), gi = (j == 0 && i < S) ? g_entry(i) : 0.0;
		A[i][j] = hij * si * sj * ((lmp && i == j && i < S) ? 1.0 + lm_delta : 1.0);
		if (j == 0) A[i][8] = gi * si;
		if (trec) {
			trec[8 * i + j] = (i < S && j < S) ? hij : 0.0;
			if (j == 0) trec[64 + i] = gi;
			if (lane == 0) {
				trec[88] = ts.f_ext ? LD(ts.f_ext + t) : (ncc ? n_f : -acc_s[ACC_RR] / 2);
				trec[90] = undo ? 1.0 : 0.0; trec[91] = lm_delta; trec[92] = 1.0;
			}
		}
	}
	__syncthreads();
	FIN_STAMP(3);
#pragma unroll
	for (int k = 0; k < 8; ++k) {
		if (pivoting) {
			int pr = k;
			double best = fabs(A[k][k]);
#pragma unroll
			for (int r = k + 1; r < 8; ++r) { const double v = fabs(A[r][k]); if (v > best) { best = v; pr = r; } }
			const int src = i == k ? pr : (i == pr ? k : i);
			const double mine = A[src][j], rhs = A[src][8];
			__syncthreads();
			if (wv0) { A[i][j] = mine; if (j == 0) A[i][8] = rhs; }
			__syncthreads();
		}
		const double piv = A[k][k], aik = A[i][k], akj = A[k][j], bk = A[k][8];
		const double f = (i != k && piv != 0) ? aik / piv : 0.0;
		__syncthreads();
		if (wv0 && i != k) {
			A[i][j] -= f * akj;
			if (j == 0) A[i][8] -= f * bk;
		}
		__syncthreads();
	}
	if (wv0 && j == 0) {
		const double d = A[i][i];
		dps[i] = (i < S && d != 0) ? -(A[i][8] / d) * si : 0.0;
	}
	__syncthreads();
	FIN_STAMP(4);
	__shared__ double xs[9], nxy[8];
	const bool hom = bv.ssm == MTFHIP_SSM_HOMOGRAPHY;
	if (lane < 8) {
		const double v = undo ? LD(lmp + 4 + lane) : dps[lane];
		if (lmp && !undo) ST(lmp + 4 + lane, v);
		dps[lane] = v;
		if (trec) trec[72 + lane] = v;
	}
	__syncthreads();
	double dp[8];
#pragma unroll
	for (int s = 0; s < 8; ++s) dp[s] = dps[s];
	double Wn[9];
	double *Wp = bv.warps + 9 * t, *st = bv.states + 8 * t;
	if constexpr (ADDITIVE) {
		double sn[8];
#pragma unroll
		for (int s = 0; s < 8; ++s) sn[s] = sos[s] + (undo ? -dp[s] : dp[s]);
		if (hom) {
			Wn[0] = 1 + sn[0]; Wn[1] = sn[1]; Wn[2] = sn[2]; Wn[3] = sn[3]; Wn[4] = 1 + sn[4]; Wn[5] = sn[5];
			Wn[6] = sn[6]; Wn[7] = sn[7]; Wn[8] = 1;
		} else {
			Wn[0] = 1 + sn[2]; Wn[1] = sn[3]; Wn[2] = sn[0]; Wn[3] = sn[4]; Wn[4] = 1 + sn[5]; Wn[5] = sn[1];
			Wn[6] = 0; Wn[7] = 0; Wn[8] = 1;
		}
		double sq = 0;
#pragma unroll
		for (int q = 0; q < 8; ++q) if (lane == q) sq = sn[q];
		if (lane < S) ST(st + lane, sq);
	} else {
	double U[9];
	if (hom) {
		U[0] = 1 + dp[0]; U[1] = dp[1]; U[2] = dp[2]; U[3] = dp[3]; U[4] = 1 + dp[4]; U[5] = dp[5];
		U[6] = dp[6]; U[7] = dp[7]; U[8] = 1;
	} else {
		U[0] = 1 + dp[2]; U[1] = dp[3]; U[2] = dp[0]; U[3] = dp[4]; U[4] = 1 + dp[5]; U[5] = dp[1];
		U[6] = 0; U[7] = 0; U[8] = 1;
	}
	if ((sm.sm == MTFHIP_SM_ICLK) != undo) {
		double c[9];
		c[0] = U[4] * U[8] - U[5] * U[7]; c[1] = U[2] * U[7] - U[1] * U[8]; c[2] = U[1] * U[5] - U[2] * U[4];
		c[3] = U[5] * U[6] - U[3] * U[8]; c[4] = U[0] * U[8] - U[2] * U[6]; c[5] = U[2] * U[3] - U[0] * U[5];
		c[6] = U[3] * U[7] - U[4] * U[6]; c[7] = U[1] * U[6] - U[0] * U[7]; c[8] = U[0] * U[4] - U[1] * U[3];
		double det = U[0] * c[0] + U[1] * c[3] + U[2] * c[6];
		double inv_det = 1.0 / det;
#pragma unroll
		for (int q = 0; q < 9; ++q) c[q] *= inv_det;
		double n22 = c[8];
		double cq = 0;
#pragma unroll
		for (int q = 0; q < 9; ++q) if (lane == q) cq = c[q];
		if (lane < 9) xs[lane] = cq / n22;
		__syncthreads();
#pragma unroll
		for (int q = 0; q < 9; ++q) U[q] = xs[q];
		__syncthreads();
		U[0] = 1 + (U[0] - 1); U[4] = 1 + (U[4] - 1); U[8] = 1;
		if (!hom) { U[6] = 0; U[7] = 0; }
	}
	double Wo[9];
#pragma unroll
	for (int q = 0; q < 9; ++q) Wo[q] = Ws[q];
#pragma unroll
	for (int r = 0; r < 3; ++r)
#pragma unroll
		for (int c2 = 0; c2 < 3; ++c2)
			Wn[3 * r + c2] = Wo[3 * r] * U[c2] + Wo[3 * r + 1] * U[3 + c2] + Wo[3 * r + 2] * U[6 + c2];
	if (hom) {
		double n22 = Wn[8];
		double wq = 0;
#pragma unroll
		for (int q = 0; q < 9; ++q) if (lane == q) wq = Wn[q];
		if (lane < 9) xs[lane] = wq / n22;
		__syncthreads();
#pragma unroll
		for (int q = 0; q < 9; ++q) Wn[q] = xs[q];
		if (lane == 0) {
			ST(st + 0, Wn[0] - 1); ST(st + 1, Wn[1]); ST(st + 2, Wn[2]); ST(st + 3, Wn[3]); ST(st + 4, Wn[4] - 1); ST(st + 5, Wn[5]);
			ST(st + 6, Wn[6]); ST(st + 7, Wn[7]);
		}
	} else if (lane == 0) {
		ST(st + 0, Wn[2]); ST(st + 1, Wn[5]); ST(st + 2, Wn[0] - 1); ST(st + 3, Wn[1]); ST(st + 4, Wn[3]); ST(st + 5, Wn[4] - 1);
	}
	}
	{
		double wq = 0;
#pragma unroll
		for (int q = 0; q < 9; ++q) if (lane == q) wq = Wn[q];
		if (lane < 9) ST(Wp + lane, wq);
	}
	double *cr = ts.corners + 8 * t;
	if (lane < 4) {
		const int q = lane;
		double X = ics[3 * q], Y = ics[3 * q + 1], Z = ics[3 * q + 2];
		double nx = Wn[0] * X + Wn[1] * Y + Wn[2] * Z, ny = Wn[3] * X + Wn[4] * Y + Wn[5] * Z;
		if (hom) {
			double d = Wn[6] * X + Wn[7] * Y + Wn[8] * Z;
			nx = nx / d; ny = ny / d;
		}
		nxy[2 * q] = nx; nxy[2 * q + 1] = ny;
		ST(cr + 2 * q, nx); ST(cr + 2 * q + 1, ny);
		if (trec) { trec[80 + 2 * q] = nx; trec[81 + 2 * q] = ny; }
	}
	__syncthreads();
	FIN_STAMP(5);
	if (lane != 0) return;
	double change = 0;
#pragma unroll
	for (int q = 0; q < 4; ++q) {
		double ddx = crs[2 * q] - nxy[2 * q], ddy = crs[2 * q + 1] - nxy[2 * q + 1];
		change += ddx * ddx + ddy * ddy;
	}
	const int n_it = n_it_prev + 1;
	STI(ts.n_iters + t, n_it);
	if (trec) trec[89] = (double)n_it_prev;
	if (lmp) {
		const int id = lm_iter_id + ((undo && sm.sm == MTFHIP_SM_FCLK && !ADDITIVE) ? 0 : 1);
		ST(lmp + 3, (double)id);
		if ((!undo && change < sm.epsilon) || id >= sm.max_iters) stop_target(Ws, sos);
	} else if (change < sm.epsilon || n_it >= sm.max_iters) stop_target(Ws, sos);
	FIN_STAMP(6);
}


template <bool COH = false>
__device__ __forceinline__ void finish_track_fast_body(const BatchView &bv, const mtfhip_sm_desc &sm, const TrackState &ts,
	const double *partials, int nblk, int t) {
	auto LD = [](const double *p) -> double { if constexpr (COH) return ld_coh(p); else return *p; };
	auto LDI = [](const int *p) -> int { if constexpr (COH) return ld_coh(p); else return *p; };
	auto ST = [](double *p, double v) { if constexpr (COH) st_coh(p, v); else *p = v; };
	auto STI = [](int *p, int v) { if constexpr (COH) st_coh(p, v); else *p = v; };
	auto stop_target = [&](const double *w_old, const double *s_old) {
		STI(ts.active + t, 0);
		if (ts.lean_pass) {
			for (int q = 0; q < 9; ++q) ST(ts.warp_last + 9 * t + q, w_old[q]);
			for (int q = 0; q < 8; ++q) ST(ts.state_last + 8 * t + q, s_old[q]);
			STI(ts.need_mat + t, 1);
		}
	};
	__shared__ double f_acc[ACC_COUNT], f_h0[64], f_w[9], f_cr[8], f_ic[12], f_lm[kLmStride + 1], f_part[3][80], f_so[8];
	const int lane = threadIdx.x;
	const bool wv0 = lane < 64;
	const int S = bv.S;
	constexpr int RL = ACC_COUNT;
	const int act = LDI(ts.active + t);
	FIN_STAMP(0);
	const int n_it_prev = LDI(ts.n_iters + t);
	double *lmp = ts.lm ? ts.lm + (size_t)t * kLmStride : nullptr;
	double v_h0 = 0, v_w = 0, v_cr = 0, v_ic = 0, v_acc = 0, v_lm = 0, v_f = 0, v_so = 0;
	if (wv0) {
		if (ts.lean_pass && lane < 8) v_so = LD(bv.states + 8 * t + lane);
		if (lmp && lane < kLmStride) v_lm = LD(lmp + lane);
		if (ts.f_ext && lane == 0) v_f = LD(ts.f_ext + t);
		v_h0 = ts.h0[(size_t)t * 64 + lane];
		if (lane < 9) v_w = LD(bv.warps + 9 * t + lane);
		if (lane < 8) v_cr = LD(ts.corners + 8 * t + lane);
		if (lane < 12) v_ic = ts.init_corners_hm[12 * t + lane];
	}
	const int n_runs = (nblk > 8 && blockDim.x >= 240) ? 3 : 1;
	const int run_len = n_runs == 1 ? nblk : ((nblk + 3 * 8 - 1) / (3 * 8)) * 8;
	{
		const int run = n_runs == 1 ? 0 : lane / 80, col = n_runs == 1 ? lane : lane % 80;
		if (col < RL && run < n_runs) {
			const int b0 = run * run_len, b1 = (b0 + run_len < nblk) ? b0 + run_len : nblk;
			const double *p = partials + (size_t)t * nblk * RL + col;
			auto ld = [&](size_t off) -> double { return LD(p + off); };
			double s0 = 0, s1 = 0, s2 = 0, s3 = 0, s4 = 0, s5 = 0, s6 = 0, s7 = 0;
			int b = b0;
			for (; b + 7 < b1; b += 8) {
				s0 += ld((size_t)b * RL); s1 += ld((size_t)(b + 1) * RL);
				s2 += ld((size_t)(b + 2) * RL); s3 += ld((size_t)(b + 3) * RL);
				s4 += ld((size_t)(b + 4) * RL); s5 += ld((size_t)(b + 5) * RL);
				s6 += ld((size_t)(b + 6) * RL); s7 += ld((size_t)(b + 7) * RL);
			}
			for (; b < b1; ++b) s0 += ld((size_t)b * RL);
			const double v = ((s0 + s1) + (s2 + s3)) + ((s4 + s5) + (s6 + s7));
			if (n_runs == 1) v_acc = v; else f_part[run][col] = v;
		}
	}
	if (!act) return;
	FIN_STAMP(1);
	if (wv0) {
		f_h0[lane] = v_h0;
		if (lane < 9) f_w[lane] = v_w;
		if (lane < 8) { f_cr[lane] = v_cr; f_so[lane] = v_so; }
		if (lane < 12) f_ic[lane] = v_ic;
		if (lane < kLmStride) f_lm[lane] = v_lm;
		if (lane == 0) f_lm[kLmStride] = v_f;
	}
	if (n_runs > 1) {
		__syncthreads();
		if (lane < RL) v_acc = (f_part[0][lane] + f_part[1][lane]) + f_part[2][lane];
	}
	if (lane < RL) { f_acc[lane] = v_acc; ST(ts.acc + (size_t)t * RL + lane, v_acc); }
	__syncthreads();
	if (!wv0) return;
	FIN_STAMP(2);
	double lm_delta = 0.0;
	int lm_iter_id = n_it_prev;
	bool undo = false;
	const double f_now = ts.f_ext ? f_lm[kLmStride] : -f_acc[ACC_RR] / 2;
	if (lmp) {
		const double prev_f = f_lm[0];
		lm_delta = f_lm[1];
		const bool state_reset = f_lm[2] != 0.0;
		lm_iter_id = (int)f_lm[3];
		if (!state_reset && lm_iter_id > 0) {
			if (f_now < prev_f) { lm_delta *= sm.lm_delta_update; undo = true; }
			else if (f_now > prev_f) lm_delta /= sm.lm_delta_update;
		}
		if (lane == 0) {
			ST(lmp + 1, lm_delta);
			if (undo) ST(lmp + 2, 1.0);
			else { ST(lmp + 2, 0.0); if (!state_reset) ST(lmp + 0, f_now); }
		}
	}
	const bool use_h0 = (sm.hess_type == 0) || (sm.sm == MTFHIP_SM_ICLK);
	const bool sum_h0 = (sm.sm == MTFHIP_SM_ESM) && (sm.hess_type == 2 || sm.hess_type == 4);
	const double gscale = (sm.sm == MTFHIP_SM_ESM) ? 0.5 : 1.0;
	double aH[36], aG[8], hI[36];
#pragma unroll
	for (int k = 0; k < 36; ++k) aH[k] = f_acc[ACC_H + k];
#pragma unroll
	for (int k = 0; k < 8; ++k) aG[k] = f_acc[ACC_G + k];
#pragma unroll
	for (int r = 0; r < 8; ++r)
#pragma unroll
		for (int c = 0; c <= r; ++c) hI[r * (r + 1) / 2 + c] = f_h0[(r * S + c) & 63];
	double M[8][8], y[8];
#pragma unroll
	for (int r = 0; r < 8; ++r) {
#pragma unroll
		for (int c = 0; c <= r; ++c) {
			const int kk = c * 8 - (c * (c - 1)) / 2 + (r - c);
			const double h0v = hI[r * (r + 1) / 2 + c];
			double v = use_h0 ? h0v : -aH[kk];
			if (sum_h0) v = (v + h0v) * 0.5;
			M[r][c] = r < S ? v : (r == c ? -1.0 : 0.0);
		}
		y[r] = r < S ? gscale * aG[r] : 0.0;
	}
	FIN_STAMP(3);
	double *trec = (ts.trace && n_it_prev < ts.trace_cap) ? ts.trace + ((size_t)t * ts.trace_cap + n_it_prev) * kTraceStride : nullptr;
	if (trec && lane == 0) {
#pragma unroll
		for (int r = 0; r < 8; ++r) {
#pragma unroll
			for (int c = 0; c < 8; ++c) trec[8 * r + c] = (r < S && c < S) ? (c <= r ? M[r][c] : M[c][r]) : 0.0;
			trec[64 + r] = y[r];
		}
		trec[88] = f_now; trec[90] = undo ? 1.0 : 0.0; trec[91] = lm_delta; trec[92] = 1.0;
	}
	double dp[8];
	if (!undo) {
		if (lmp) {
#pragma unroll
			for (int r = 0; r < 8; ++r) if (r < S) M[r][r] *= 1.0 + lm_delta;
		}
		double inv[8];
#pragma unroll
		for (int k = 0; k < 8; ++k) {
			const double d = M[k][k];
			inv[k] = d != 0 ? rcp_fast(d) : 0.0;
			double l[8];
#pragma unroll
			for (int i = k + 1; i < 8; ++i) l[i] = M[i][k] * inv[k];
#pragma unroll
			for (int i = k + 1; i < 8; ++i) {
#pragma unroll
				for (int j = k + 1; j <= i; ++j) M[i][j] = fma(-l[i], M[j][k], M[i][j]);
			}
#pragma unroll
			for (int i = k + 1; i < 8; ++i) { M[i][k] = l[i]; y[i] = fma(-l[i], y[k], y[i]); }
		}
#pragma unroll
		for (int k = 7; k >= 0; --k) {
			double x = y[k] * inv[k];
#pragma unroll
			for (int i = k + 1; i < 8; ++i) x = fma(-M[i][k], dp[i], x);
			dp[k] = x;
		}
#pragma unroll
		for (int k = 0; k < 8; ++k) dp[k] = k < S ? -dp[k] : 0.0;
		if (lmp) {
#pragma unroll
			for (int q = 0; q < 8; ++q) if (lane == q) ST(lmp + 4 + q, dp[q]);
		}
	} else {
#pragma unroll
		for (int q = 0; q < 8; ++q) dp[q] = f_lm[4 + q];
	}
	FIN_STAMP(4);
	const bool hom = bv.ssm == MTFHIP_SSM_HOMOGRAPHY;
	double U[9];
	if (hom) {
		U[0] = 1 + dp[0]; U[1] = dp[1]; U[2] = dp[2]; U[3] = dp[3]; U[4] = 1 + dp[4]; U[5] = dp[5]; U[6] = dp[6]; U[7] = dp[7]; U[8] = 1;
	} else {
		U[0] = 1 + dp[2]; U[1] = dp[3]; U[2] = dp[0]; U[3] = dp[4]; U[4] = 1 + dp[5]; U[5] = dp[1]; U[6] = 0; U[7] = 0; U[8] = 1;
	}
	if ((sm.sm == MTFHIP_SM_ICLK) != undo) {
		double c[9];
		c[0] = U[4] * U[8] - U[5] * U[7]; c[1] = U[2] * U[7] - U[1] * U[8]; c[2] = U[1] * U[5] - U[2] * U[4];
		c[3] = U[5] * U[6] - U[3] * U[8]; c[4] = U[0] * U[8] - U[2] * U[6]; c[5] = U[2] * U[3] - U[0] * U[5];
		c[6] = U[3] * U[7] - U[4] * U[6]; c[7] = U[1] * U[6] - U[0] * U[7]; c[8] = U[0] * U[4] - U[1] * U[3];
		const double ic8 = rcp_fast(c[8]);
#pragma unroll
		for (int q = 0; q < 8; ++q) U[q] = c[q] * ic8;
		U[8] = 1;
		if (!hom) { U[6] = 0; U[7] = 0; }
	}
	double Wn[9];
#pragma unroll
	for (int r = 0; r < 3; ++r) {
		const double w0 = f_w[3 * r], w1 = f_w[3 * r + 1], w2 = f_w[3 * r + 2];
#pragma unroll
		for (int c2 = 0; c2 < 3; ++c2) Wn[3 * r + c2] = fma(w0, U[c2], fma(w1, U[3 + c2], w2 * U[6 + c2]));
	}
	if (hom) {
		const double in22 = rcp_fast(Wn[8]);
#pragma unroll
		for (int q = 0; q < 8; ++q) Wn[q] *= in22;
		Wn[8] = 1;
	}
	double St[8];
	if (hom) { St[0] = Wn[0] - 1; St[1] = Wn[1]; St[2] = Wn[2]; St[3] = Wn[3]; St[4] = Wn[4] - 1; St[5] = Wn[5]; St[6] = Wn[6]; St[7] = Wn[7]; }
	else { St[0] = Wn[2]; St[1] = Wn[5]; St[2] = Wn[0] - 1; St[3] = Wn[1]; St[4] = Wn[3]; St[5] = Wn[4] - 1; St[6] = 0; St[7] = 0; }
	double Cr[8], change = 0;
#pragma unroll
	for (int q = 0; q < 4; ++q) {
		const double X = f_ic[3 * q], Y = f_ic[3 * q + 1], Z = f_ic[3 * q + 2];
		double nx = fma(Wn[0], X, fma(Wn[1], Y, Wn[2] * Z)), ny = fma(Wn[3], X, fma(Wn[4], Y, Wn[5] * Z));
		if (hom) { const double idn = rcp_fast(fma(Wn[6], X, fma(Wn[7], Y, Wn[8] * Z))); nx *= idn; ny *= idn; }
		const double ddx = f_cr[2 * q] - nx, ddy = f_cr[2 * q + 1] - ny;
		change += ddx * ddx + ddy * ddy;
		Cr[2 * q] = nx; Cr[2 * q + 1] = ny;
	}
	FIN_STAMP(5);
	double wq = 0, sq = 0, cq = 0;
#pragma unroll
	for (int q = 0; q < 9; ++q) if (lane == q) wq = Wn[q];
#pragma unroll
	for (int q = 0; q < 8; ++q) if (lane == q) { sq = St[q]; cq = Cr[q]; }
	if (lane < 9) ST(bv.warps + 9 * t + lane, wq);
	if (lane < S) ST(bv.states + 8 * t + lane, sq);
	if (lane < 8) ST(ts.corners + 8 * t + lane, cq);
	if (lane != 0) return;
	if (trec) {
#pragma unroll
		for (int q = 0; q < 8; ++q) { trec[72 + q] = dp[q]; trec[80 + q] = Cr[q]; }
		trec[89] = (double)n_it_prev;
	}
	const int n_it = n_it_prev + 1;
	STI(ts.n_iters + t, n_it);
	if (lmp) {
		const int id = lm_iter_id + ((undo && sm.sm == MTFHIP_SM_FCLK) ? 0 : 1);
		ST(lmp + 3, (double)id);
		if ((!undo && change < sm.epsilon) || id >= sm.max_iters) stop_target(f_w, f_so);
	} else if (change < sm.epsilon || n_it >= sm.max_iters) stop_target(f_w, f_so);
	FIN_STAMP(6);
}

}
#endif
```

### mtf_amd/csrc/mtfhip_grid_device.h

```cpp
#pragma once
#include "mtfhip_device.h"

namespace mtfhip {

__device__ __forceinline__ double lattice_coord(int i, int n, double lo, double hi, double step) {
	return (n == 1 || i == n - 1) ? hi : lo + i * step;
}
__device__ __forceinline__ double grid_point_sum(double a_nx, double b_ny, double c_1) { return a_nx + b_ny + c_1; }
__device__ __forceinline__ void grid_point_xy(const double *W0, double nx, double ny, double &X, double &Y) {
	X = grid_point_sum(W0[0] * nx, W0[1] * ny, W0[2] * 1.0);
	Y = grid_point_sum(W0[3] * nx, W0[4] * ny, W0[5] * 1.0);
}
__device__ __forceinline__ double grid_point_z(const double *W0, double nx, double ny) { return W0[6] * nx + W0[7] * ny + W0[8] * 1.0; }

template <int K>
__device__ __forceinline__ void block_allsum(double *v, double *lds ) {
	const int lane = threadIdx.x & 63, wave = threadIdx.x >> 6;
#pragma unroll
	for (int k = 0; k < K; ++k)
#pragma unroll
		for (int m = 32; m >= 1; m >>= 1) v[k] += __shfl_xor(v[k], m);
	__syncthreads();
	if (lane == 0) {
#pragma unroll
		for (int k = 0; k < K; ++k) lds[wave * K + k] = v[k];
	}
	__syncthreads();
#pragma unroll
	for (int k = 0; k < K; ++k) v[k] = (lds[k] + lds[K + k]) + (lds[2 * K + k] + lds[3 * K + k]);
}

template <int K>
__device__ __forceinline__ void block_allsum_dpp(double *v, double *lds ) {
	const int lane = threadIdx.x & 63, wave = threadIdx.x >> 6;
#pragma unroll
	for (int k = 0; k < K; ++k) v[k] = wave_sum_dpp(v[k]);
	__syncthreads();
	if (lane == 0) {
#pragma unroll
		for (int k = 0; k < K; ++k) lds[wave * K + k] = v[k];
	}
	__syncthreads();
#pragma unroll
	for (int k = 0; k < K; ++k) v[k] = (lds[k] + lds[K + k]) + (lds[2 * K + k] + lds[3 * K + k]);
}

__device__ __forceinline__ double swap_add32(double a, double b) {
	const auto lo = __builtin_amdgcn_permlane32_swap(__double2loint(a), __double2loint(b), false, false);
	const auto hi = __builtin_amdgcn_permlane32_swap(__double2hiint(a), __double2hiint(b), false, false);
	return __hiloint2double(hi[0], lo[0]) + __hiloint2double(hi[1], lo[1]);
}
__device__ __forceinline__ double swap_add16(double a, double b) {
	const auto lo = __builtin_amdgcn_permlane16_swap(__double2loint(a), __double2loint(b), false, false);
	const auto hi = __builtin_amdgcn_permlane16_swap(__double2hiint(a), __double2hiint(b), false, false);
	return __hiloint2double(hi[0], lo[0]) + __hiloint2double(hi[1], lo[1]);
}
__device__ __forceinline__ double row_sum_dpp(double x) {
#define MTFHIP_ROW_STEP(CTRL) { \
		const int tl = __builtin_amdgcn_update_dpp(0, __double2loint(x), CTRL, 0xF, 0xF, false), th = __builtin_amdgcn_update_dpp(0, __double2hiint(x), CTRL, 0xF, 0xF, false); \
		x += __hiloint2double(th, tl); }
	MTFHIP_ROW_STEP(0xB1) MTFHIP_ROW_STEP(0x4E) MTFHIP_ROW_STEP(0x141) MTFHIP_ROW_STEP(0x140)
#undef MTFHIP_ROW_STEP
	return x;
}
__device__ __forceinline__ void block_allsum_h12(double *v, double *lds) {
	const int lane = threadIdx.x & 63, wave = threadIdx.x >> 6;
	double h6[6], h3[3];
#pragma unroll
	for (int j = 0; j < 6; ++j) h6[j] = swap_add32(v[j], v[j + 6]);
#pragma unroll
	for (int j = 0; j < 3; ++j) h3[j] = row_sum_dpp(swap_add16(h6[j], h6[j + 3]));
	if ((lane & 15) == 0) {
		const int base = wave * 12 + ((lane & 32) ? 6 : 0) + ((lane & 16) ? 3 : 0);
#pragma unroll
		for (int j = 0; j < 3; ++j) lds[base + j] = h3[j];
	}
	__syncthreads();
	const int k = lane < 12 ? lane : 0;
	const double mine = (lds[k] + lds[12 + k]) + (lds[24 + k] + lds[36 + k]);
#pragma unroll
	for (int q = 0; q < 12; ++q) v[q] = readlane_f64(mine, q);
}

__device__ __forceinline__ void publish_target(const HostPublish &pub, int t, double wq, double sq, double cq, int n_it) {
	const int lane = threadIdx.x;
	double *p = reinterpret_cast<double *>(pub.host);
	const size_t Bt = (size_t)pub.B;
	if (lane < 9) __hip_atomic_store(p + 9 * (size_t)t + lane, wq, __ATOMIC_RELAXED, __HIP_MEMORY_SCOPE_SYSTEM);
	if (lane < 8) {
		__hip_atomic_store(p + 9 * Bt + 8 * (size_t)t + lane, sq, __ATOMIC_RELAXED, __HIP_MEMORY_SCOPE_SYSTEM);
		__hip_atomic_store(p + 17 * Bt + 8 * (size_t)t + lane, cq, __ATOMIC_RELAXED, __HIP_MEMORY_SCOPE_SYSTEM);
	}
	if (lane == 0) __hip_atomic_store(reinterpret_cast<int *>(pub.host + pub.dbl_bytes) + Bt + t, n_it, __ATOMIC_RELAXED, __HIP_MEMORY_SCOPE_SYSTEM);
	if (pub.fenced) __builtin_amdgcn_fence(__ATOMIC_RELEASE, "agent");
	else wait_stores_acked();
	if (lane == 0) {
		const int done = pub.fenced ? __hip_atomic_fetch_add(pub.count, 1, __ATOMIC_ACQ_REL, __HIP_MEMORY_SCOPE_AGENT)
		                            : __hip_atomic_fetch_add(pub.count, 1, __ATOMIC_RELAXED, __HIP_MEMORY_SCOPE_AGENT);
		if (done == (int)gridDim.x - 1) {
			__hip_atomic_store(pub.count, 0, __ATOMIC_RELAXED, __HIP_MEMORY_SCOPE_AGENT);
			if (pub.fenced) {
				__threadfence_system();
				__hip_atomic_store(pub.flag, pub.seq, __ATOMIC_RELEASE, __HIP_MEMORY_SCOPE_SYSTEM);
			} else __hip_atomic_store(pub.flag, pub.seq, __ATOMIC_RELAXED, __HIP_MEMORY_SCOPE_SYSTEM);
		}
	}
}

template <int K>
__device__ __forceinline__ void init_allsum(double *v, double *lds ) {
	const int lane = threadIdx.x & 63, wave = threadIdx.x >> 6;
#pragma unroll
	for (int k = 0; k < K; ++k) v[k] = wave_sum_dpp(v[k]);
	__syncthreads();
	if (lane == 0) {
#pragma unroll
		for (int k = 0; k < K; ++k) lds[wave * K + k] = v[k];
	}
	__syncthreads();
#pragma unroll
	for (int k = 0; k < K; ++k) v[k] = (lds[k] + lds[K + k]) + (lds[2 * K + k] + lds[3 * K + k]);
}

__device__ __forceinline__ void invert_definite_wave(int S, const double *Hs , double *a, double *out ) {
	const int lane = threadIdx.x & 63, i = lane >> 3, j = lane & 7;
	constexpr int LD = 17;
	const bool in = i < S && j < S;
	const double di = i < S ? fabs(Hs[i * S + i]) : 1.0, dj = j < S ? fabs(Hs[j * S + j]) : 1.0;
	const double sci = di > 0 ? 1.0 / sqrt(di) : 1.0, scj = dj > 0 ? 1.0 / sqrt(dj) : 1.0;
	a[i * LD + j] = in ? Hs[j * S + i] * sci * scj : (i == j ? 1.0 : 0.0);
	a[i * LD + 8 + j] = i == j ? 1.0 : 0.0;
	__builtin_amdgcn_wave_barrier();
	bool singular = false;
	for (int k = 0; k < S; ++k) {
		int piv = k; double best = fabs(a[k * LD + k]);
		for (int r = k + 1; r < S; ++r) { const double v = fabs(a[r * LD + k]); if (v > best) { best = v; piv = r; } }
		if (best == 0) { singular = true; break; }
		__builtin_amdgcn_wave_barrier();
		if (piv != k && i == 0) {
			const double t0 = a[piv * LD + j], t1 = a[piv * LD + 8 + j];
			a[piv * LD + j] = a[k * LD + j]; a[piv * LD + 8 + j] = a[k * LD + 8 + j];
			a[k * LD + j] = t0; a[k * LD + 8 + j] = t1;
		}
		__builtin_amdgcn_wave_barrier();
		const double p = a[k * LD + k];
		__builtin_amdgcn_wave_barrier();
		if (i == 0) { a[k * LD + j] /= p; a[k * LD + 8 + j] /= p; }
		__builtin_amdgcn_wave_barrier();
		const double f = a[i * LD + k], r0 = a[k * LD + j], r1 = a[k * LD + 8 + j];
		__builtin_amdgcn_wave_barrier();
		if (i != k && f != 0) { a[i * LD + j] -= f * r0; a[i * LD + 8 + j] -= f * r1; }
		__builtin_amdgcn_wave_barrier();
	}
	if (in) out[j * S + i] = singular ? 0.0 : a[i * LD + 8 + j] * sci * scj;
}

}
```

### mtf_amd/csrc/mtfhip_internal.h

```cpp
#ifndef MTFHIP_INTERNAL_H
#define MTFHIP_INTERNAL_H

#include <cstdlib>
#include <hip/hip_runtime.h>
#include "../../include/mtfhip.h"
#include "mtfhip_fused_dispatch.h"

namespace mtfhip {

struct ImgView {
	const float *data;
	int h, w, stride;
	int channels = 1;
};

struct BatchView {
	int B, N, S, ssm, am;
	int NP, C;
	int unit_z;
	double *buf[MTFHIP_BUF_COUNT];
	double *warps;
	double *states;
};

enum {
	ACC_H = 0,
	ACC_G = 36,
	ACC_RR = 44,
	ACC_G2 = 45,
	ACC_COUNT = 56
};
enum {
	NCC_GRAM = 0,
	NCC_SJ = 36,
	NCC_ITJ = 44,
	NCC_I0J = 52,
	NCC_ITJ0 = 60,
	NCC_IT = 68, NCC_IT2 = 69, NCC_I0IT = 70,
	NCC_ACC_COUNT = 72
};

void note_launch_error(hipError_t e, const char *file, int line);
#define MTFHIP_LAUNCH(...) do { hipLaunchKernelGGL(__VA_ARGS__); const hipError_t _le = hipGetLastError(); \
	if (_le != hipSuccess) ::mtfhip::note_launch_error(_le, __FILE__, __LINE__); } while (0)
constexpr int kBlock = 256;
constexpr int kGridTabMax = 2048;
constexpr int kGridRegenMinRows = 8;
#ifndef MTFHIP_SLOTS
#define MTFHIP_SLOTS 512
#endif
#ifndef MTFHIP_MIN_ROWS
#define MTFHIP_MIN_ROWS 4
#endif
constexpr int kMaxS = 8;

inline void fused_decomposition(int N, int B, int &nblk, int &rows, int slots = MTFHIP_SLOTS) {
	const int total_rows = (N + kBlock - 1) / kBlock;
	int nb_max = (total_rows + MTFHIP_MIN_ROWS - 1) / MTFHIP_MIN_ROWS;
	if (nb_max < 1) nb_max = 1;
	if (B < 1) B = 1;
	double best = 1e300;
	int best_nb = 1;
	for (int nb = 1; nb <= nb_max; ++nb) {
		const int r = (total_rows + nb - 1) / nb;
		const int real_nb = (total_rows + r - 1) / r;
		const long blocks = (long)B * real_nb;
		const long rounds = (blocks + slots - 1) / slots;
		const double cost = (double)rounds * (r + 1.5);
		if (cost < best - 1e-9) { best = cost; best_nb = real_nb; }
	}
	rows = (total_rows + best_nb - 1) / best_nb;
	nblk = (total_rows + rows - 1) / rows;
}
inline int fused_blocks_per_target(int N, int B) { int nb, r; fused_decomposition(N, B, nb, r); return nb; }
inline int simple_blocks_per_target(int N) {
	int nb = (N + kBlock * 4 - 1) / (kBlock * 4);
	return nb < 1 ? 1 : nb;
}

struct TrackState {
	double *acc;
	double *h0;
	double *corners;
	double *init_corners_hm;
	int *active;
	int *n_iters;
	const double *ncc;
	const double *ncc_tm;
	int h_from_acc;
	double *lm;
	const double *f_ext;
	double *trace;
	int trace_cap;
	const double *h_extra;
	double h_extra_scale;
	int fast_finish;
	int fresh_reset;
	double *warp_last = nullptr;
	double *state_last = nullptr;
	int *need_mat = nullptr;
	int lean_pass = 0;
};
constexpr int kLmStride = 12;
constexpr int kTraceStride = 96;

struct PersistState {
	int *arrive;
	unsigned *gen;
	unsigned gen_base;
	unsigned long long timeout_ticks;
};

__host__ __device__ inline bool rect_to_quad_hd(double lo_x, double lo_y, double hi_x, double hi_y, const double *q, double *H) {
	const double x0 = q[0], y0 = q[1], x1 = q[2], y1 = q[3], x2 = q[4], y2 = q[5], x3 = q[6], y3 = q[7];
	const double dx1 = x1 - x2, dx2 = x3 - x2, sx = x0 - x1 + x2 - x3;
	const double dy1 = y1 - y2, dy2 = y3 - y2, sy = y0 - y1 + y2 - y3;
	double a, b, c, d, e, f, g, h;
	if (sx == 0 && sy == 0) {
		a = x1 - x0; b = x3 - x0; c = x0; d = y1 - y0; e = y3 - y0; f = y0; g = 0; h = 0;
		if (a * e - b * d == 0) return false;
	} else {
		const double den = dx1 * dy2 - dy1 * dx2;
		if (den == 0) return false;
		g = (sx * dy2 - dx2 * sy) / den; h = (dx1 * sy - sx * dy1) / den;
		a = x1 - x0 + g * x1; b = x3 - x0 + h * x3; c = x0;
		d = y1 - y0 + g * y1; e = y3 - y0 + h * y3; f = y0;
	}
	const double wx = hi_x - lo_x, wy = hi_y - lo_y;
	const double rows[3][3] = {{a, b, c}, {d, e, f}, {g, h, 1.0}};
	double m[9];
	for (int r = 0; r < 3; ++r) {
		m[3 * r] = rows[r][0] / wx; m[3 * r + 1] = rows[r][1] / wy;
		m[3 * r + 2] = rows[r][2] - rows[r][0] * lo_x / wx - rows[r][1] * lo_y / wy;
	}
	if (m[8] == 0 || !(m[8] - m[8] == 0)) return false;
	if (m[8] == 1.0) for (int i = 0; i < 9; ++i) H[i] = m[i];
	else for (int i = 0; i < 9; ++i) H[i] = m[i] / m[8];
	H[8] = 1;
	return true;
}

__host__ __device__ inline bool quad_degenerate_hd(const double *q) {
	const double x0 = q[0], y0 = q[1], x1 = q[2], y1 = q[3], x2 = q[4], y2 = q[5], x3 = q[6], y3 = q[7];
	const double dx1 = x1 - x2, dx2 = x3 - x2, sx = x0 - x1 + x2 - x3;
	const double dy1 = y1 - y2, dy2 = y3 - y2, sy = y0 - y1 + y2 - y3;
	if (sx == 0 && sy == 0) return (x1 - x0) * (y3 - y0) - (x3 - x0) * (y1 - y0) == 0;
	return dx1 * dy2 - dy1 * dx2 == 0;
}

struct GridLayoutHD { int grid_size_x, grid_size_y, patch_size_x, patch_size_y, dyn_patch_size, patch_centroid_inside; };
__host__ __device__ inline double lin_spaced_hd(int i, int n, double lo, double hi) { return (n == 1 || i == n - 1) ? hi : lo + i * ((hi - lo) / (n - 1)); }
__host__ __device__ inline void grid_pt_hd(const double *Wr, int resx, int resy, int idx, double *x, double *y) {
	const int r = idx / resx, c = idx % resx;
	const double ny = lin_spaced_hd(r, resy, -0.5, 0.5), nx = lin_spaced_hd(c, resx, -0.5, 0.5);
	const double X = Wr[0] * nx + Wr[1] * ny + Wr[2], Y = Wr[3] * nx + Wr[4] * ny + Wr[5], Z = Wr[6] * nx + Wr[7] * ny + Wr[8];
	*x = X / Z; *y = Y / Z;
}
__host__ __device__ inline void grid_patch_corners_hd(const GridLayoutHD &g, const double *Wr, int k, double *pc) {
	const int extra = (g.dyn_patch_size || g.patch_centroid_inside) ? 1 : 0;
	const int resx = g.grid_size_x + extra, resy = g.grid_size_y + extra;
	const bool surround = extra != 0;
	const int sub_x = g.grid_size_x + 1;
	const int row = k / g.grid_size_x, col = k % g.grid_size_x;
	for (int q = 0; q < 8; ++q) pc[q] = 0.0;
	if (surround) {
		const int id[4] = {row * sub_x + col, row * sub_x + col + 1, (row + 1) * sub_x + col + 1, (row + 1) * sub_x + col};
		for (int q = 0; q < 4; ++q) grid_pt_hd(Wr, resx, resy, id[q], pc + 2 * q, pc + 2 * q + 1);
	}
	if (!g.dyn_patch_size) {
		double cx, cy;
		if (g.patch_centroid_inside) {
			cx = (pc[0] + pc[2] + pc[4] + pc[6]) / 4.0;
			cy = (pc[1] + pc[3] + pc[5] + pc[7]) / 4.0;
		} else grid_pt_hd(Wr, resx, resy, k, &cx, &cy);
		const double half_x = g.patch_size_x / 2.0, half_y = g.patch_size_y / 2.0;
		const double min_x = cx - half_x, min_y = cy - half_y;
		const double max_x = min_x + g.patch_size_x, max_y = min_y + g.patch_size_y;
		pc[0] = pc[6] = min_x; pc[2] = pc[4] = max_x;
		pc[1] = pc[3] = min_y; pc[5] = pc[7] = max_y;
	}
}

struct RegionIngest {
	const double *corners;
	const double *ncc;
	double *d_ncc, *d_w0, *d_init_corners_hm;
	double lo_x, lo_y, hi_x, hi_y;
	int resx, resy, force_unit_z;
	int layout;
	GridLayoutHD grid;
	double region_map[9];
};

struct HostPublish {
	char *host;
	size_t dbl_bytes;
	int B;
	int *count;
	unsigned long long *flag, seq;
	int fenced;
};
inline int publish_fenced() {
	static const int v = [] { const char *e = std::getenv("MTFHIP_PUBLISH_FENCE"); return (e && e[0] == '1') ? 1 : 0; }();
	return v;
}

struct FusedArgs {
	int mode;
	int chained;
	int materialize;
	int hess_mean;
	int j0_init_variant;
	int j0_recompute;
	int rows_per_block;
	double grad_eps;
	double norm_mult, norm_add;
	const int *active;
	int inline_warp;
	double iw[9], is[8];
	int fast_math;
	int grid_regen;
	int g_resx, g_resy;
	double g_lo_x, g_lo_y, g_hi_x, g_hi_y;
	double g_step_x, g_step_y;
	const double *w0;
};

struct RscvMap {
	const double *map = nullptr;
	int nb = 0, linear = 0;
};
struct LrscvMap {
	const double *map = nullptr;
	const double *wts = nullptr;
	int nb = 0, R = 0, affine = 0, linear = 0;
};

bool kernarg_layout_verified(hipStream_t st);
void launch_queue_delay(double microseconds, hipStream_t st);
void launch_apply_warp(const BatchView &bv, hipStream_t st);
void launch_grad_pts(const BatchView &bv, double eps, hipStream_t st);
void launch_sample(const BatchView &bv, const ImgView &im, const double *pts, double *out,
	double mult, double add, hipStream_t st);
void launch_update_model(const BatchView &bv, const ImgView &im, const double *pts, double *I0, double mult, double add,
	double frame_count, double alpha, int running_avg, hipStream_t st);
void launch_img_grad(const BatchView &bv, const ImgView &im, const double *pts, double *grad,
	double eps, double mult, hipStream_t st);
void launch_warped_img_grad(const BatchView &bv, const ImgView &im, const double *grad_pts, double *grad,
	double eps, double mult, hipStream_t st);
void launch_pix_jacobian(const BatchView &bv, int variant, const double *grad, double *J, hipStream_t st);
void launch_mean_jacobian(const BatchView &bv, hipStream_t st);
void launch_finish_track_mi(const BatchView &bv, const mtfhip_sm_desc &sm, const TrackState &ts, int sum_std, int gmode,
	const double *mi_H, const double *gpart, int ng, double *rows, hipStream_t st);
void launch_ssd_residual(const BatchView &bv, double *partials, int nblk, hipStream_t st);
void launch_negate(const double *src, double *dst, size_t n, hipStream_t st);
void launch_gemv(const BatchView &bv, const double *v1, const double *J1, const double *v2, const double *J2,
	int sum_mode, double *partials, int nblk, hipStream_t st);
void launch_gram(const BatchView &bv, const double *J, double *partials, int nblk, hipStream_t st);
void launch_vec_sum(const BatchView &bv, const double *v, double *partials, int nblk, hipStream_t st);
void launch_ncc_centered(const BatchView &bv, const double *sc, double *partials, int nblk, hipStream_t st);
void launch_ncc_grad(const BatchView &bv, const double *sc, int curr, double *out, double *partials, int nblk, hipStream_t st);
void launch_sub_mean(const BatchView &bv, double *v, const double *sc, hipStream_t st);
void launch_col_sum(const BatchView &bv, const double *J, double *partials, int nblk, hipStream_t st);
void launch_ncc_hess(const BatchView &bv, const double *sc, const double *colmean, const double *J, double *partials,
	int nblk, hipStream_t st);
enum {
	MI_NB = 16,
	MI_HIST_INIT = 0, MI_HIST_CURR = 16, MI_LOG_INIT = 32, MI_LOG_CURR = 48,
	MI_JOINT = 64, MI_JOINT_LOG = 320, MI_T_CURR = 576, MI_T_INIT = 832,
	MI_SELF_JOINT = 1088, MI_T_SELF = 1344, MI_SIZE = 1600
};
void launch_mi_hist(const BatchView &bv, int nb, double norm_mult, const double *A, const double *Bv, double *partials,
	int nblk, int row_len, hipStream_t st);
void launch_mi_hist_finish(const BatchView &bv, int nb, double pre_seed, double norm_mult, int mode, int first_init,
	const double *partials, int nblk, int row_len, double *tb, double *f_out, hipStream_t st);
void launch_mi_factor(const BatchView &bv, int nb, int curr, double *tb, hipStream_t st);
void launch_mi_grad(const BatchView &bv, int nb, double norm_mult, const double *A, const double *Bv, const double *tb,
	int table_off, double *out, hipStream_t st);
void launch_mi_hess(const BatchView &bv, int nb, double norm_mult, const double *A, const double *Bv, const double *tb,
	int table_off, int transpose_q, const double *J, double *partials, int nblk, int row_len, hipStream_t st);
void launch_mi_hess_finish(const BatchView &bv, int nb, const double *partials, int nblk, int row_len, const double *tb,
	int joint_off, int hist_off, int transpose_q, double *out, hipStream_t st);
void launch_mi_tables_iter(const BatchView &bv, int nb, double pre_seed, double norm_mult, int with_self, const double *partials, int nblk,
	int row_len, double *tb, double *f_out, hipStream_t st);
void launch_mi_hist_self(const BatchView &bv, int nb, double norm_mult, const double *A, const double *Bv, double *partials,
	int nblk, int row_len, hipStream_t st);
struct MiJ0Rebuild { const double *dI0, *pts, *z; int hom, init_variant; };
void launch_mi_grad_gemv(const BatchView &bv, int nb, double norm_mult, const double *It, const double *I0, const double *tb,
	const double *Jt, const double *J0, const MiJ0Rebuild &rb, double *df_dIt, double *df_dI0, double *partials, int nblk, hipStream_t st);
struct MiFastPlan {
	int nb = 8;
	int hk;
	int hrow;
	int j0_mode;
	int j0_init_variant;
	int need_dft, need_df0, g_mean;
	int nonchained = 0;
	int hist_from_joint = 0;
	double grad_eps, norm_mult, norm_add, hist_norm;
	const int *active;
	const double *tb;
	const double *poly = nullptr;
};
void launch_mi_poly_tables(const BatchView &bv, const double *tb, double hist_norm, int with_self, double *poly, hipStream_t st);
void launch_mi_tables_poly(const BatchView &bv, int nb, double pre_seed, double norm_mult, int with_self, const double *partials, int nblk, int row_len,
	double *tb, double *f_out, double *poly, hipStream_t st);
int mi_poly_size(int nb = 8);
void launch_mi_pass_hist(const BatchView &bv, const ImgView &im, const MiFastPlan &pl, double *partials, int nblk, int row_len, hipStream_t st);
void launch_mi_pass_grad_hess(const BatchView &bv, const ImgView &im, const MiFastPlan &pl, double *partials, int nblk, hipStream_t st);
void launch_mi_finish_fast(const BatchView &bv, const mtfhip_sm_desc &sm, const TrackState &ts, const MiFastPlan &pl, int gmode, int do_track,
	const double *partials, int nblk, double *out_H, double *out_g, double *rows, hipStream_t st);
void launch_mi_score_candidates(const BatchView &bv, const ImgView &im, const MiFastPlan &pl, const double *dev_states, int lo, int cnt,
	double *partials, int nblk, int row_len, double pre_seed, double alpha, int likelihood_func, double measurement_sigma, double max_similarity,
	double *wts, double *sim, hipStream_t st);
int mi_fast_row_len(int nb = 8);
enum { PF_SAMPLER_STATE = 0,
	PF_SAMPLER_HOM_CORNERS = 1,
	PF_SAMPLER_AFF_PTS1 = 2,
	PF_SAMPLER_AFF_PTS2 = 3,
	PF_SAMPLER_AFF_GEOM = 4 };
struct PfLaunch {
	int n, S;
	int dynamic_model, update_type, sampler, nz, likelihood_func, resampling_type, mean_type;
	double ar_coeff, measurement_sigma, max_similarity;
	double sigma[8], mean[8], init_corners[8], init_corners_hm[12], aux_inv[9], canon[6];
	unsigned long long seed;
	unsigned iter;
	const double *normals, *uniforms;
	int n_distr;
	const double *distr_uniforms;
	double min_distr_wt, min_eff_particles;
};
struct PfBuffers {
	double *st, *ar;
	double *prop, *prop_ar;
	double *next, *next_ar;
	double *wts, *sim;
	double *cum, *sub16, *chunk_tot, *chunk_incl;
	double *parts, *gparts, *out;
	int *res_order;
	double *distr_sigma, *distr_mean, *distr_cum, *distr_wts, *scan_stats;
	int *distr_ids, *resample_flag;
	int *ids, *counters;
};
constexpr int kPfMaxPeers = 8;
struct PfPeerPush {
	int world, rank;
	double *wts[kPfMaxPeers];
	unsigned long long *counters[kPfMaxPeers];
	unsigned *arrive;
};
struct PfPeerWait {
	int world, rank;
	const unsigned long long *counters;
	unsigned long long expected[kPfMaxPeers];
	int *err;
};
void launch_pf_propose(int ssm, const PfLaunch &p, const PfBuffers &bf, const double *st_in, const double *ar_in, double *st_out, double *ar_out, hipStream_t st);
void launch_score_block(const BatchView &bv, const ImgView &im, const double *states, int lo, int cnt, double alpha, double norm_mult,
	double norm_add, const double *ncc_sc, double *wts, double *sim, int likelihood_func, double measurement_sigma, double max_similarity,
	int fast_math, const PfPeerPush *peer , const double *hull , const float *pair , hipStream_t st);
void launch_pf_peer_push(const PfPeerPush &peer, const double *wts, int lo, int cnt, hipStream_t st);
void launch_pf_peer_wait(const PfPeerWait &w, hipStream_t st);
void launch_pf_scan(const PfLaunch &p, const PfBuffers &bf, const PfPeerWait *wait, hipStream_t st);
struct PfSelectPlan { int local = 0; const PfPeerWait *wait = nullptr; const double *pert_in = nullptr; double *pert_out = nullptr; int estimate = 1; };
int pf_local_max();
void launch_pf_select(int ssm, const PfLaunch &p, const PfBuffers &bf, int lookahead, double *host_out ,
	unsigned long long *host_flag, unsigned long long seq, const PfSelectPlan &plan, hipStream_t st);
void launch_pf_fill(int n, int S, const double *dev_state, double *states, double *ars, hipStream_t st);
void launch_pf_residual_prep(int n, const double *total, double *wts, double *keys, int *idx, const int *flag, hipStream_t st);
void launch_pf_residual_copies(int n, const double *wts, const int *order, int *copies, hipStream_t st);
void launch_pf_residual_map(int n, const int *order, const int *copies, const int *starts, int *ids, hipStream_t st);
int pf_parts_per_block();
int pf_chunk();
void launch_finish(double *partials, int nblk, double *out, int B, hipStream_t st);
void launch_finish_rows(double *partials, int nblk, int row_len, double *out, int B, hipStream_t st);
void launch_finish_host(double *partials, int nblk, int row_len, double *out_host, int *count, unsigned long long *flag_host,
	unsigned long long seq, int B, hipStream_t st);
void launch_publish_host(const void *src, void *dst_host, size_t bytes, int *count, unsigned long long *flag_host,
	unsigned long long seq, hipStream_t st);
void launch_fused_ssd(const BatchView &bv, const ImgView &im, const FusedArgs &fa, double *partials,
	int nblk, hipStream_t st, const RscvMap *rm = nullptr, const LrscvMap *lm = nullptr);
void launch_fused_lrscv(const BatchView &bv, const ImgView &im, const FusedArgs &fa, double *partials, int nblk, const LrscvMap &lm,
	hipStream_t st);
void launch_fused_rscv(const BatchView &bv, const ImgView &im, const FusedArgs &fa, double *partials, int nblk, const RscvMap &rm,
	hipStream_t st);
void launch_hess_pts(const BatchView &bv, double eps, hipStream_t st);
void launch_img_hess(const BatchView &bv, const ImgView &im, const double *pts, double *hess, double eps, double mult, hipStream_t st);
void launch_warped_img_hess(const BatchView &bv, const ImgView &im, const double *pts, const double *hp, double *hess, double eps,
	double mult, hipStream_t st);
void launch_pix_hessian(const BatchView &bv, int variant, const double *hess, const double *grad, double *D, hipStream_t st);
void launch_weighted_plane_sum(const BatchView &bv, const double *d2a, const double *d2b, const double *w, double *partials, int nblk,
	double *out, hipStream_t st);
void launch_mean_planes(const double *a, const double *b, double *o, size_t n, hipStream_t st);
struct SecondOrderNcc { const double *rows; int nblk; const double *sc; };
struct SecondOrderMi { const double *tb; double hist_norm; };
void launch_second_order_ssd(const BatchView &bv, const ImgView &im, int term, int chained, int d0_variant, double grad_eps,
	double hess_eps, double norm_mult, double norm_add, double *partials, int nblk, double *out, hipStream_t st, int own_pts = 0,
	SecondOrderNcc nc = SecondOrderNcc{nullptr, 0, nullptr}, SecondOrderMi mi = SecondOrderMi{nullptr, 0.0});
void launch_hist_eq(float *gray, int rows, int cols, unsigned *hist256, float *lut256, hipStream_t st);
void launch_to_gray(const void *raw, int rows, int cols, size_t stride_bytes, int channels, int depth_f32, float *out, hipStream_t st);
void launch_sym5(const float *src, float *tmp, float *dst, int rows, int cols, const float kx[3], const float ky[3], hipStream_t st);
void launch_pyr_down(const float *src, int srows, int scols, float *dst, int drows, int dcols, hipStream_t st);
void launch_resize_linear(const float *src, int srows, int scols, float *dst, int drows, int dcols, hipStream_t st);
struct NnArgs {
	const double *perts_in;
	double *perts_out;
	double sigma[8], mean[8];
	unsigned long long seed;
	double base[9];
	int row_lo;
	double norm_mult, norm_add;
	const double *base_dev;
	const int *done;
};
void launch_pair_image(const ImgView &im, float *pair , hipStream_t st);
hipError_t launch_nn_dataset(const BatchView &bv, const ImgView &im, const NnArgs &a, int count, double *feat, double *warps, const double *hull, hipStream_t st);
size_t nn_warps_bytes(int count);
bool nn_two_launch_ok(const BatchView &bv, const ImgView &im, int fast_math);
struct NnBest { double dist; int idx; int pad; };
constexpr int kNnSearchMaxFeat = 8000;
int nn_search_resident(int ncc, int F);
int nn_search_blocks(int n_samples, int resident);
void launch_nn_search(int ncc, const double *feat, int n_samples, int F, const double *queries, int Q, NnBest *partials , int nblk,
	const int *done, hipStream_t st);
void launch_nn_search_finish(const NnBest *partials, int nblk, int Q, int *idx, double *dist, hipStream_t st);
void launch_nn_pick_update(int ssm, const NnBest *partials, int nblk, const double *perts, int n_samples, double *state, int *ctl, double *log, int it,
	double epsilon, hipStream_t st);
void launch_sample_candidates(const BatchView &bv, const ImgView &im, const double *dev_states, int C, double norm_mult,
	double norm_add, double *dev_feat, hipStream_t st);
constexpr int kIclkTrackMaxPix = 8 * kBlock;
struct GridFbOut { double *host; double *dev; int reinit; };
bool launch_grid_fb(const BatchView &bv, const ImgView &im, const ImgView &imp, const mtfhip_sm_desc &sm, const TrackState &ts, const double *h0inv,
	const double *ncc_sc, double norm_mult, double norm_add, double grad_eps, const HostPublish &pub, const GridFbOut &fo, const RegionIngest &rg, hipStream_t st);
bool launch_iclk_track(const BatchView &bv, const ImgView &im, const mtfhip_sm_desc &sm, const TrackState &ts,
	const double *h0inv, const double *ncc_sc, double norm_mult, double norm_add, int fast_math, const HostPublish &pub, const RegionIngest &rg, hipStream_t st);
void launch_ingest_host(const void *src_host, void *dst, size_t bytes, hipStream_t st, size_t skip_off = 0, size_t skip_len = 0);
void launch_fused_mc(const BatchView &bv, const ImgView &im, const FusedArgs &fa, double *partials, int nblk, hipStream_t st);
constexpr int kInitRec = 128;
constexpr int kTemplateInitMaxPix = 4 * 256;
struct InitPublish { double *host; int *count; unsigned long long *flag, seq; int fenced; };
void launch_template_init(const BatchView &bv, const ImgView &im, double grad_eps, double norm_mult, double norm_add, double *h0, double *h0inv,
	double *ncc, double *ncc_tm, const InitPublish &pub, const RegionIngest &rg, hipStream_t st);
bool track_step_available(const BatchView &bv, const FusedArgs &fa);
void launch_track_step(const BatchView &bv, const ImgView &im, const FusedArgs &fa, const mtfhip_sm_desc &sm, const TrackState &ts,
	double *partials, int nblk, int *arrive, hipStream_t st);
void launch_track_persist(const BatchView &bv, const ImgView &im, const FusedArgs &fa, const mtfhip_sm_desc &sm, const TrackState &ts,
	double *partials, int nblk, const PersistState &ps, int max_passes, hipStream_t st);
bool launch_init_grid_ingest(const BatchView &bv, const double *host_w0_dev, int resx, int resy, double lo_x, double lo_y,
	double hi_x, double hi_y, int force_unit_z, const void *src_host, void *dst, size_t bytes, int write_curr, hipStream_t st);
struct PhaseCtl { unsigned long long *mine; const unsigned long long *other; double frac; };
void launch_finish_track(const BatchView &bv, const mtfhip_sm_desc &sm, const TrackState &ts, const double *partials,
	int nblk, hipStream_t st, PhaseCtl pc = PhaseCtl{nullptr, nullptr, 0.0});

struct AlkArgs {
	int ialk;
	int materialize;
	int rows_per_block;
	double grad_eps, norm_mult, norm_add;
	const int *active;
};
void launch_alk_pass(const BatchView &bv, const ImgView &im, const AlkArgs &a, double *partials, int nblk, hipStream_t st);
void launch_alk_finish(const BatchView &bv, const mtfhip_sm_desc &sm, const TrackState &ts, const double *partials, int nblk, hipStream_t st);

constexpr int kScvMaxBins = 256;
struct ScvArgs {
	int nb, hist, linear;
	int from_it;
	double norm_mult, norm_add;
	const unsigned short *code;
	const double *i0o;
	const int *active;
};
int scv_hist_blocks(int N);
void launch_scv_codes(int N, int B, int nb, const double *i0o, unsigned short *code, hipStream_t st);
void launch_scv_update(const BatchView &bv, const ImgView &im, const ScvArgs &a, double *part, double *map, double *I0, hipStream_t st);

constexpr int kRscvMaxBins = 256;
struct RscvArgs {
	int nb, kind;
	double norm_mult, norm_add, grad_eps;
	const unsigned char *code;
	const double *it_orig;
	const int *active;
	unsigned *part;
	unsigned *arrive;
	double *map;
};
int rscv_hist_blocks(int N);
void launch_rscv_codes(int N, int B, int nb, const double *i0, unsigned char *code, hipStream_t st);
void launch_rscv_hist(const BatchView &bv, const ImgView &im, const RscvArgs &a, hipStream_t st);
void launch_rscv_apply(int N, int B, int nb, int linear, const double *map, const double *it_orig, double *It, hipStream_t st);

constexpr int kLscvMaxBins = 256;
constexpr int kLscvLdsBudget = 64 * 1024;
struct LscvArgs {
	int nb, nx, ny, ncx, ncell;
	int from_it;
	int affine, linear;
	double norm_mult, norm_add;
	const unsigned short *code;
	const double *i0o;
	const unsigned short *cell;
	const int *crng;
	const double *wts;
	const int *active;
	unsigned *tot;
	unsigned *arrive;
	double *map;
	double *aff;
};
int lscv_hist_blocks(int N);
void launch_lscv_update(const BatchView &bv, const ImgView &im, const LscvArgs &a, double *I0, hipStream_t st);

constexpr int kLrscvFusedStaticLds = 8 * 1024;
struct LrscvArgs {
	int nb, kind;
	int nx, ny, ncx, ncell;
	int affine;
	double norm_mult, norm_add, grad_eps;
	const unsigned char *code;
	const double *it_orig;
	const unsigned short *cell;
	const int *crng;
	const int *active;
	unsigned *tot;
	unsigned *arrive;
	double *map;
	double *aff;
};
void launch_lrscv_hist(const BatchView &bv, const ImgView &im, const LrscvArgs &a, hipStream_t st);
void launch_lrscv_apply(int N, int B, const LrscvMap &lm, const double *it_orig, double *It, hipStream_t st);

}
#endif
```

Measured before the change: 1.783 million iters/s.

## Fuse track prologue memsets into ingest kernel and publish results from finish kernel

Adds a track prologue kernel that copies the host staging slab and, in the same launch, zeroes the need-materialise flags, phase words and publish counter and initialises the LM state. This removes several memsets and a blocking host-to-device LM upload with its stream sync. The chunked loop's finish kernel now writes each stopped or last-pass target straight to the host-visible publish buffer, so the separate publish kernel at read-back is skipped. The finish kernel also raises its wave priority, and the stagger estimate changes when materialisation is deferred. The new path adds cross-kernel counting that must match the number of targets, which is a correctness risk.

```diff
diff --git a/mtf_amd/csrc/api_track.hip b/mtf_amd/csrc/api_track.hip
--- a/mtf_amd/csrc/api_track.hip
+++ b/mtf_amd/csrc/api_track.hip
@@ -2,13 +2,18 @@
 
 extern "C" {
 
-int loop_upload_slab(mtfhip_batch *b, hipStream_t st, bool keep_ncc) {
+int loop_upload_slab(mtfhip_batch *b, hipStream_t st, bool keep_ncc, const LoopWords *lw) {
 	const size_t Bt = (size_t)b->B;
 	std::memcpy(b->h_stage_b + 45 * sizeof(double) * Bt, b->h_stage_a + 45 * sizeof(double) * Bt, 9 * sizeof(double) * Bt);
 	fill_stage(b, b->h_stage_b, nullptr, 1, true);
-	if (b->h_stage_b_dev) launch_ingest_host(b->h_stage_b_dev, b->d_slab, b->slab_bytes, st, keep_ncc ? 37 * sizeof(double) * Bt : 0, keep_ncc ? 8 * sizeof(double) * Bt : 0);
+	const size_t skip_off = keep_ncc ? 37 * sizeof(double) * Bt : 0, skip_len = keep_ncc ? 8 * sizeof(double) * Bt : 0;
+	if (b->h_stage_b_dev && lw) { TimedScope tsc(b->ctx, "track_prologue", st); launch_track_prologue(b->h_stage_b_dev, b->d_slab, b->slab_bytes, skip_off, skip_len, *lw, st); }
+	else if (b->h_stage_b_dev) launch_ingest_host(b->h_stage_b_dev, b->d_slab, b->slab_bytes, st, skip_off, skip_len);
 	else if (keep_ncc) return fail(MTFHIP_ERR_LOGIC, "track: a held template-initialisation record needs the host-visible staging buffer");
-	else HIP_TRY(hipMemcpyAsync(b->d_slab, b->h_stage_b, b->slab_bytes, hipMemcpyHostToDevice, st));
+	else {
+		HIP_TRY(hipMemcpyAsync(b->d_slab, b->h_stage_b, b->slab_bytes, hipMemcpyHostToDevice, st));
+		if (lw) { TimedScope tsc(b->ctx, "track_prologue", st); launch_track_prologue(nullptr, nullptr, 0, 0, 0, *lw, st); }
+	}
 	b->warps_dirty = false;
 	return MTFHIP_OK;
 }
@@ -35,7 +40,7 @@
 	if (pub_seq) TRY(wait_host_flag(b, pub_seq));
 	else if (b->h_pub_dev) {
 		const unsigned long long seq = ++b->acc_seq;
-		launch_publish_host(b->d_slab, b->h_pub_dev, b->slab_bytes, b->d_fin_count, b->h_flag_dev, seq, st);
+		{ TimedScope tsc(b->ctx, "publish_host", st); launch_publish_host(b->d_slab, b->h_pub_dev, b->slab_bytes, b->d_fin_count, b->h_flag_dev, seq, st); }
 		TRY(wait_host_flag(b, seq));
 	} else {
 		HIP_TRY(hipMemcpyAsync(b->h_stage_b, b->d_slab, b->slab_bytes, hipMemcpyDeviceToHost, st));
@@ -320,6 +325,13 @@
 	TimedScope tsc(b->ctx, "fused_lk", r.s);
 	launch_fused_ssd(bm, b->ctx->img, fm, r.part, r.nblk_c, r.s, nullptr, nullptr);
 }
+static double track_phase_frac() {
+	const char *e_ph = std::getenv("MTFHIP_TRACK_PHASE");
+	return e_ph ? std::atof(e_ph) : 0.35;
+}
+static void track_phase_words(mtfhip_ctx *c) {
+	if (!c->d_phase && hipMalloc(&c->d_phase, sizeof(unsigned long long) * 4) != hipSuccess) { (void)hipGetLastError(); c->d_phase = nullptr; }
+}
 static int track_open_queues(mtfhip_batch *b, int n_streams, double &phase_frac) {
 	mtfhip_ctx *c = b->ctx;
 	if (n_streams >= 2) {
@@ -328,10 +340,9 @@
 			if (!c->extra_streams[q] && (hipStreamCreateWithFlags(&c->extra_streams[q], hipStreamNonBlocking) != hipSuccess ||
 				hipEventCreateWithFlags(&c->ev_join[q], hipEventDisableTiming) != hipSuccess)) { (void)hipGetLastError(); n_streams = 1; break; }
 	}
-	const char *e_ph = std::getenv("MTFHIP_TRACK_PHASE");
-	phase_frac = e_ph ? std::atof(e_ph) : 0.35;
+	phase_frac = track_phase_frac();
 	if (n_streams == 2 && phase_frac > 0) {
-		if (!c->d_phase && hipMalloc(&c->d_phase, sizeof(unsigned long long) * 4) != hipSuccess) { (void)hipGetLastError(); c->d_phase = nullptr; }
+		track_phase_words(c);
 	}
 	return n_streams;
 }
@@ -345,8 +356,9 @@
 	const int max_t = e_mx ? std::atoi(e_mx) : 8;
 	return (e_st && e_st[0] == '1') && so_term < 0 && !intensity_mapped(b) && n_streams == 1 && b->B <= max_t && track_step_available(b->view(), fa);
 }
+struct FinishCtl { PhaseCtl pc; HostPublish pub; int prio; };
 static int track_chunk_pass(mtfhip_batch *b, const mtfhip_sm_desc *sm, const FusedArgs &fa, const TrackCtx &cx, const ChunkRun &r, int it, bool lean, bool use_step,
-	const PhaseCtl &pc) {
+	const FinishCtl &fc) {
 	if (use_step) {
 		TimedScope tsc(b->ctx, "track_step", r.s);
 		launch_track_step(r.bc, b->ctx->img, r.fc, *sm, r.tc, r.part, r.nblk_c, b->d_persist + r.t0, r.s);
@@ -369,25 +381,39 @@
 			b->desc.am == MTFHIP_AM_NCC ? SecondOrderNcc{r.part, r.nblk_c, r.tc.ncc} : SecondOrderNcc{nullptr, 0, nullptr});
 	}
 	TimedScope tsc(b->ctx, "finish_track", r.s);
-	launch_finish_track(r.bc, *sm, lean ? r.tl : r.tc, r.part, r.nblk_c, r.s, pc);
-	return MTFHIP_OK;
-}
-static int track_loop_chunked(mtfhip_batch *b, const mtfhip_sm_desc *sm, const FusedArgs &fa, const TrackState &ts, const TrackCtx &cx) {
+	TrackState tf = lean ? r.tl : r.tc;
+	tf.last_pass = it + 1 == cx.max_passes ? 1 : 0;
+	tf.finish_prio = fc.prio;
+	launch_finish_track(r.bc, *sm, tf, r.part, r.nblk_c, r.s, fc.pc, fc.pub, r.t0);
+	return MTFHIP_OK;
+}
+static int track_loop_chunked(mtfhip_batch *b, const mtfhip_sm_desc *sm, const FusedArgs &fa, const TrackState &ts, const TrackCtx &cx, unsigned long long &pub_seq) {
 	hipStream_t st = b->ctx->stream;
 	int chunk = track_chunk(b, sm, fa);
 	double phase_frac;
 	const int n_streams = track_open_queues(b, track_queues(b, fa), phase_frac);
-	if (n_streams == 2 && phase_frac > 0 && b->ctx->d_phase) HIP_TRY(hipMemsetAsync(b->ctx->d_phase, 0, sizeof(unsigned long long) * 4, st));
-	static const double stagger_env = std::getenv("MTFHIP_TRACK_STAGGER_US") ? std::atof(std::getenv("MTFHIP_TRACK_STAGGER_US")) : -1.0;
-	double stagger_us = stagger_env;
-	if (stagger_env < 0) stagger_us = 0.25 * ((double)b->B * b->N * 130.0 / 6.5e6 + 8.0) * (2.0 / n_streams);
+	if (!cx.words_ready && n_streams == 2 && phase_frac > 0 && b->ctx->d_phase) HIP_TRY(hipMemsetAsync(b->ctx->d_phase, 0, sizeof(unsigned long long) * 4, st));
 	const bool use_step = track_takes_step(b, fa, cx.so_term, n_streams);
 	if (use_step) TRY(ensure_persist_words(b, st));
 	const bool defer = track_defers_materialisation(b, sm, fa, cx.so_term, cx.resume, use_step);
 	if (defer) {
 		if (!b->d_last_ws) HIP_TRY(hipMalloc(&b->d_last_ws, sizeof(double) * 17 * (size_t)b->B));
 		if (!b->d_need_mat) HIP_TRY(hipMalloc(&b->d_need_mat, sizeof(int) * (size_t)b->B));
-		HIP_TRY(hipMemsetAsync(b->d_need_mat, 0, sizeof(int) * (size_t)b->B, st));
+		if (!cx.words_ready) HIP_TRY(hipMemsetAsync(b->d_need_mat, 0, sizeof(int) * (size_t)b->B, st));
+	}
+	const char *e_sg = std::getenv("MTFHIP_TRACK_STAGGER_US");
+	double stagger_us = e_sg ? std::atof(e_sg) : -1.0;
+	if (stagger_us < 0) stagger_us = 0.25 * ((double)b->B * b->N * (defer ? 8.75e-6 : 130.0 / 6.5e6) + 8.0) * (2.0 / n_streams);
+	FinishCtl fin{PhaseCtl{nullptr, nullptr, 0.0}, HostPublish{nullptr, 0, 0, nullptr, nullptr, 0, 0}, 0};
+	{
+		const char *e_pr = std::getenv("MTFHIP_FINISH_PRIO");
+		fin.prio = (e_pr && e_pr[0] == '0') ? 0 : 1;
+	}
+	const mtfhip_ctx *c = b->ctx;
+	const bool borrowed = c->img.data != c->img_owned && c->img.data != c->prev_owned;
+	if (cx.fused_io && b->h_pub_dev && !b->d_trace && !use_step && !cx.resume && !(borrowed && sm->epsilon > 0)) {
+		pub_seq = ++b->acc_seq;
+		fin.pub = HostPublish{b->h_pub_dev, b->slab_dbl_bytes, b->B, b->d_fin_count, b->h_flag_dev, pub_seq, publish_fenced()};
 	}
 	if (n_streams >= 2) {
 		const int part_sz = (b->B + n_streams - 1) / n_streams;
@@ -409,12 +435,12 @@
 				ChunkRun &r = runs[k];
 				if (r.done) continue;
 				if (n_streams >= 2 && it == 0 && k > g0 && stagger_us > 0) launch_queue_delay(stagger_us * (double)(k - g0), r.s);
-				PhaseCtl pc{nullptr, nullptr, 0.0};
+				fin.pc = PhaseCtl{nullptr, nullptr, 0.0};
 				if (n_streams == 2 && phase_frac > 0 && b->ctx->d_phase) {
 					const int qi = (int)((k - g0) & 1);
-					pc = PhaseCtl{b->ctx->d_phase + qi, b->ctx->d_phase + (1 - qi), phase_frac};
+					fin.pc = PhaseCtl{b->ctx->d_phase + qi, b->ctx->d_phase + (1 - qi), phase_frac};
 				}
-				TRY(track_chunk_pass(b, sm, fa, cx, r, it, lean, use_step, pc));
+				TRY(track_chunk_pass(b, sm, fa, cx, r, it, lean, use_step, fin));
 				if (loop_all_stopped(sm, cx.max_passes, it, r.tc.active, r.nt, r.s, h_flags)) r.done = true;
 				all_done = all_done && r.done;
 			}
@@ -447,8 +473,27 @@
 	else { fa.materialize = 0; fa.mode = 2; fa.active = nullptr; fa.rows_per_block = 1; fa.j0_recompute = 0; fa.inline_warp = 0; fa.fast_math = 0; fa.grid_regen = 0; fa.w0 = nullptr; }
 	const bool fresh = b->fresh_reinit && one_launch && !region_mode && !slab_uploaded && !resume && b->h_pub_dev && b->d_trace == nullptr;
 	b->fresh_reinit = false;
-	if (!slab_uploaded && !fresh) TRY(loop_upload_slab(b, st, b->hold_init_pull && b->init_mirror_seq != 0));
-	else b->warps_dirty = false;
+	const bool persisted = !mi && !one_launch && cx.so_term < 0 && persist_fits(b, sm, fa);
+	{
+		const char *e_io = std::getenv("MTFHIP_TRACK_FUSED_IO");
+		cx.fused_io = !mi && !one_launch && !persisted && !(e_io && e_io[0] == '0');
+	}
+	LoopWords lw{nullptr, 0, nullptr, nullptr, 0, 0.0, nullptr};
+	if (cx.fused_io && !resume) {
+		if (track_defers_materialisation(b, sm, fa, cx.so_term, resume, false)) {
+			if (!b->d_last_ws) HIP_TRY(hipMalloc(&b->d_last_ws, sizeof(double) * 17 * (size_t)b->B));
+			if (!b->d_need_mat) HIP_TRY(hipMalloc(&b->d_need_mat, sizeof(int) * (size_t)b->B));
+		}
+		if (sm->leven_marq && !b->d_lm) HIP_TRY(hipMalloc(&b->d_lm, sizeof(double) * kLmStride * (size_t)b->B));
+		if (track_queues(b, fa) == 2 && track_phase_frac() > 0) track_phase_words(b->ctx);
+		lw = LoopWords{b->d_need_mat, b->d_need_mat ? b->B : 0, b->ctx->d_phase, sm->leven_marq ? b->d_lm : nullptr, b->B, sm->lm_delta_init, b->d_fin_count};
+		cx.words_ready = true;
+	}
+	if (!slab_uploaded && !fresh) TRY(loop_upload_slab(b, st, b->hold_init_pull && b->init_mirror_seq != 0, cx.words_ready ? &lw : nullptr));
+	else {
+		b->warps_dirty = false;
+		if (cx.words_ready) { TimedScope tsc(b->ctx, "track_prologue", st); launch_track_prologue(nullptr, nullptr, 0, 0, 0, lw, st); }
+	}
 	fa.active = b->d_active;
 	if (ncc && !one_launch && !b->d_ncc_tm) return fail(MTFHIP_ERR_LOGIC, "track before init_template");
 	TrackState ts{b->d_acc, b->d_h0, b->d_corners, b->d_init_corners_hm, b->d_active, b->d_iters, ncc ? b->d_ncc : nullptr, ncc ? b->d_ncc_tm : nullptr, 0, nullptr, nullptr,
@@ -457,7 +502,7 @@
 	if (b->d_trace && !resume) HIP_TRY(hipMemsetAsync(b->d_trace, 0, sizeof(double) * kTraceStride * (size_t)b->trace_cap * b->B, st));
 	if (mi && b->d_trace) ts.f_ext = b->d_mi_f;
 	if (sm->leven_marq) {
-		if (resume) ts.lm = b->d_lm;
+		if (resume || cx.words_ready) ts.lm = b->d_lm;
 		else TRY(loop_lm_state(b, sm, st, &ts.lm));
 		if (mi) ts.f_ext = b->d_mi_f;
 	}
@@ -472,11 +517,10 @@
 		ts.fast_finish = (enabled && b->math_mode == MTFHIP_MATH_FAST && !ncc && !mi && cx.so_term < 0) ? 1 : 0;
 	}
 	unsigned long long pub_seq = 0;
-	bool persisted = false;
 	if (mi) TRY(track_loop_mi(b, sm, ts, cx));
 	else if (one_launch) TRY(track_loop_one_launch(b, sm, ts, cx, pub_seq));
-	else if ((persisted = cx.so_term < 0 && persist_fits(b, sm, fa))) TRY(track_loop_persist(b, sm, fa, ts, cx));
-	else TRY(track_loop_chunked(b, sm, fa, ts, cx));
+	else if (persisted) TRY(track_loop_persist(b, sm, fa, ts, cx));
+	else TRY(track_loop_chunked(b, sm, fa, ts, cx, pub_seq));
 	const char *h_res;
 	TRY(loop_read_back(b, st, pub_seq, n_iters, corners, &h_res));
 	const int *act = reinterpret_cast<const int *>(h_res + b->slab_dbl_bytes), *iters = act + b->B;
diff --git a/mtf_amd/csrc/kernels_fused.hip b/mtf_amd/csrc/kernels_fused.hip
--- a/mtf_amd/csrc/kernels_fused.hip
+++ b/mtf_amd/csrc/kernels_fused.hip
@@ -1,5 +1,6 @@
 #include "mtfhip_finish_device.h"
 #include "mtfhip_fused_device.h"
+#include "mtfhip_grid_device.h"
 
 namespace mtfhip {
 
@@ -18,9 +19,23 @@
 
 
 __global__ __launch_bounds__(256) void k_finish_track(BatchView bv, mtfhip_sm_desc sm, TrackState ts,
-	const double *partials, int nblk, PhaseCtl pc) {
-	if (ts.fast_finish) finish_track_fast_body(bv, sm, ts, partials, nblk, blockIdx.x);
-	else finish_track_body(bv, sm, ts, partials, nblk, blockIdx.x);
+	const double *partials, int nblk, PhaseCtl pc, HostPublish pub, int pub_t0) {
+	if (ts.finish_prio) __builtin_amdgcn_s_setprio(3);
+	const int t = blockIdx.x;
+	__shared__ int s_stopped;
+	if (pub.host && threadIdx.x == 0) __hip_atomic_store(&s_stopped, 0, __ATOMIC_RELAXED, __HIP_MEMORY_SCOPE_WAVEFRONT);
+	if (ts.fast_finish) finish_track_fast_body(bv, sm, ts, partials, nblk, t, pub.host ? &s_stopped : nullptr);
+	else finish_track_body(bv, sm, ts, partials, nblk, t, pub.host ? &s_stopped : nullptr);
+	if (pub.host && threadIdx.x < 64) {
+		__builtin_amdgcn_fence(__ATOMIC_ACQ_REL, "wavefront");
+		const int ran = __hip_atomic_load(&s_stopped, __ATOMIC_RELAXED, __HIP_MEMORY_SCOPE_WAVEFRONT);
+		if (ran == 3 || (ran && ts.last_pass)) {
+			const int lane = threadIdx.x;
+			const double wq = lane < 9 ? bv.warps[9 * t + lane] : 0.0, sq = lane < 8 ? bv.states[8 * t + lane] : 0.0, cq = lane < 8 ? ts.corners[8 * t + lane] : 0.0;
+			publish_target(pub, pub_t0 + t, wq, sq, cq, __hip_atomic_load(ts.n_iters + t, __ATOMIC_RELAXED, __HIP_MEMORY_SCOPE_WAVEFRONT), pub.B);
+		}
+	}
+	if (ts.finish_prio) __builtin_amdgcn_s_setprio(0);
 	if (pc.mine && blockIdx.x == 0 && threadIdx.x == 0) {
 		const unsigned long long prev = ld_coh(pc.mine), other = ld_coh(pc.other);
 		unsigned long long now = wall_clock64();
@@ -79,8 +94,8 @@
 	if (!launched) note_launch_error(hipErrorInvalidDeviceFunction, __FILE__, __LINE__);
 }
 void launch_finish_track(const BatchView &bv, const mtfhip_sm_desc &sm, const TrackState &ts, const double *partials,
-	int nblk, hipStream_t st, PhaseCtl pc) {
-	MTFHIP_LAUNCH(k_finish_track, dim3(bv.B), dim3(nblk > 8 ? 256 : (bv.am == MTFHIP_AM_NCC ? 128 : 64)), 0, st, bv, sm, ts, partials, nblk, pc);
+	int nblk, hipStream_t st, PhaseCtl pc, const HostPublish &pub, int pub_t0) {
+	MTFHIP_LAUNCH(k_finish_track, dim3(bv.B), dim3(nblk > 8 ? 256 : (bv.am == MTFHIP_AM_NCC ? 128 : 64)), 0, st, bv, sm, ts, partials, nblk, pc, pub, pub_t0);
 }
 
 void launch_finish_track_mi(const BatchView &bv, const mtfhip_sm_desc &sm, const TrackState &ts, int sum_std, int gmode,
diff --git a/mtf_amd/csrc/kernels_interface.hip b/mtf_amd/csrc/kernels_interface.hip
--- a/mtf_amd/csrc/kernels_interface.hip
+++ b/mtf_amd/csrc/kernels_interface.hip
@@ -480,6 +480,16 @@
 	if (i < n16 && !(i >= skip_lo && i < skip_hi)) dst[i] = src_host[i];
 	if (i < n_tail) dst_tail[i] = src_tail[i];
 }
+__global__ __launch_bounds__(256) void k_track_prologue(const uint4 *src_host, uint4 *dst, unsigned n16, const unsigned *src_tail, unsigned *dst_tail, unsigned n_tail,
+	unsigned skip_lo, unsigned skip_hi, LoopWords lw) {
+	const unsigned i = blockIdx.x * 256 + threadIdx.x;
+	if (i < n16 && !(i >= skip_lo && i < skip_hi)) dst[i] = src_host[i];
+	if (i < n_tail) dst_tail[i] = src_tail[i];
+	if (lw.zero_i && i < (unsigned)lw.n_zero_i) lw.zero_i[i] = 0;
+	if (lw.phase && i < 4) lw.phase[i] = 0ull;
+	if (lw.count && i == 0) *lw.count = 0;
+	if (lw.lm && i < (unsigned)lw.n_lm * kLmStride) lw.lm[i] = (i % kLmStride == 1) ? lw.lm_delta_init : 0.0;
+}
 __global__ __launch_bounds__(64) void k_finish(const double *partials, int nblk, double *out) {
 	const int t = blockIdx.x, k = threadIdx.x;
 	if (k >= ACC_COUNT) return;
@@ -619,6 +629,14 @@
 		reinterpret_cast<const unsigned *>(static_cast<const char *>(src_host) + 16 * (size_t)n16),
 		reinterpret_cast<unsigned *>(static_cast<char *>(dst) + 16 * (size_t)n16), n_tail, (unsigned)(skip_off / 16), (unsigned)((skip_off + skip_len) / 16));
 }
+void launch_track_prologue(const void *src_host, void *dst, size_t bytes, size_t skip_off, size_t skip_len, const LoopWords &lw, hipStream_t st) {
+	const unsigned n16 = src_host ? (unsigned)(bytes / 16) : 0, n_tail = src_host ? (unsigned)((bytes % 16) / 4) : 0;
+	const unsigned n_words = std::max(std::max((unsigned)(lw.zero_i ? lw.n_zero_i : 0), lw.lm ? (unsigned)lw.n_lm * kLmStride : 0u), 4u);
+	const unsigned blocks = (std::max(std::max(n16, n_tail), n_words) + 255) / 256;
+	MTFHIP_LAUNCH(k_track_prologue, dim3(blocks), dim3(256), 0, st, static_cast<const uint4 *>(src_host), static_cast<uint4 *>(dst), n16,
+		reinterpret_cast<const unsigned *>(static_cast<const char *>(src_host) + 16 * (size_t)n16),
+		reinterpret_cast<unsigned *>(static_cast<char *>(dst) + 16 * (size_t)n16), n_tail, (unsigned)(skip_off / 16), (unsigned)((skip_off + skip_len) / 16), lw);
+}
 void launch_finish_rows(double *partials, int nblk, int row_len, double *out, int B, hipStream_t st) {
 	MTFHIP_LAUNCH(k_finish_rows, dim3(B, (row_len + 127) / 128), dim3(128), 0, st, partials, nblk, row_len, out);
 }
diff --git a/mtf_amd/csrc/mtfhip_api_internal.h b/mtf_amd/csrc/mtfhip_api_internal.h
--- a/mtf_amd/csrc/mtfhip_api_internal.h
+++ b/mtf_amd/csrc/mtfhip_api_internal.h
@@ -613,9 +613,9 @@
 	}
 };
 int mi_iterate(mtfhip_batch *b, const mtfhip_sm_desc *sm, double *f, double *g, double *H);
-struct TrackCtx { int so_term, max_passes, nb2; bool resume, region_mode; };
+struct TrackCtx { int so_term, max_passes, nb2; bool resume, region_mode; bool fused_io = false, words_ready = false; };
 int track_loop_mi(mtfhip_batch *b, const mtfhip_sm_desc *sm, mtfhip::TrackState &ts, const TrackCtx &cx);
-int loop_upload_slab(mtfhip_batch *b, hipStream_t st, bool keep_ncc);
+int loop_upload_slab(mtfhip_batch *b, hipStream_t st, bool keep_ncc, const LoopWords *lw = nullptr);
 int loop_lm_state(mtfhip_batch *b, const mtfhip_sm_desc *sm, hipStream_t st, double **lm);
 bool loop_all_stopped(const mtfhip_sm_desc *sm, int max_passes, int it, const int *d_flags, int n, hipStream_t on, std::vector<int> &h_flags, hipError_t *err = nullptr);
 int loop_read_back(mtfhip_batch *b, hipStream_t st, unsigned long long pub_seq, int *n_iters, double *corners, const char **h_res);
diff --git a/mtf_amd/csrc/mtfhip_finish_device.h b/mtf_amd/csrc/mtfhip_finish_device.h
--- a/mtf_amd/csrc/mtfhip_finish_device.h
+++ b/mtf_amd/csrc/mtfhip_finish_device.h
@@ -13,13 +13,14 @@
 
 template <bool COH = false, bool ADDITIVE = false>
 __device__ __forceinline__ void finish_track_body(const BatchView &bv, const mtfhip_sm_desc &sm, const TrackState &ts,
-	const double *partials, int nblk, int t) {
+	const double *partials, int nblk, int t, int *stop_flag = nullptr) {
 	auto LD = [](const double *p) -> double { if constexpr (COH) return ld_coh(p); else return *p; };
 	auto LDI = [](const int *p) -> int { if constexpr (COH) return ld_coh(p); else return *p; };
 	auto ST = [](double *p, double v) { if constexpr (COH) st_coh(p, v); else *p = v; };
 	auto STI = [](int *p, int v) { if constexpr (COH) st_coh(p, v); else *p = v; };
 	auto stop_target = [&](const double *w_old, const double *s_old) {
 		STI(ts.active + t, 0);
+		if (stop_flag) __hip_atomic_store(stop_flag, 3, __ATOMIC_RELAXED, __HIP_MEMORY_SCOPE_WAVEFRONT);
 		if (ts.lean_pass) {
 			for (int q = 0; q < 9; ++q) ST(ts.warp_last + 9 * t + q, w_old[q]);
 			for (int q = 0; q < 8; ++q) ST(ts.state_last + 8 * t + q, s_old[q]);
@@ -73,6 +74,7 @@
 		}
 	}
 	if (!act) return;
+	if (stop_flag && lane == 0) __hip_atomic_store(stop_flag, 1, __ATOMIC_RELAXED, __HIP_MEMORY_SCOPE_WAVEFRONT);
 	FIN_STAMP(1);
 	if (wv0) {
 		h0s[lane] = v_h0;
@@ -341,13 +343,14 @@
 
 template <bool COH = false>
 __device__ __forceinline__ void finish_track_fast_body(const BatchView &bv, const mtfhip_sm_desc &sm, const TrackState &ts,
-	const double *partials, int nblk, int t) {
+	const double *partials, int nblk, int t, int *stop_flag = nullptr) {
 	auto LD = [](const double *p) -> double { if constexpr (COH) return ld_coh(p); else return *p; };
 	auto LDI = [](const int *p) -> int { if constexpr (COH) return ld_coh(p); else return *p; };
 	auto ST = [](double *p, double v) { if constexpr (COH) st_coh(p, v); else *p = v; };
 	auto STI = [](int *p, int v) { if constexpr (COH) st_coh(p, v); else *p = v; };
 	auto stop_target = [&](const double *w_old, const double *s_old) {
 		STI(ts.active + t, 0);
+		if (stop_flag) __hip_atomic_store(stop_flag, 3, __ATOMIC_RELAXED, __HIP_MEMORY_SCOPE_WAVEFRONT);
 		if (ts.lean_pass) {
 			for (int q = 0; q < 9; ++q) ST(ts.warp_last + 9 * t + q, w_old[q]);
 			for (int q = 0; q < 8; ++q) ST(ts.state_last + 8 * t + q, s_old[q]);
@@ -395,6 +398,7 @@
 		}
 	}
 	if (!act) return;
+	if (stop_flag && lane == 0) __hip_atomic_store(stop_flag, 1, __ATOMIC_RELAXED, __HIP_MEMORY_SCOPE_WAVEFRONT);
 	FIN_STAMP(1);
 	if (wv0) {
 		f_h0[lane] = v_h0;
diff --git a/mtf_amd/csrc/mtfhip_grid_device.h b/mtf_amd/csrc/mtfhip_grid_device.h
--- a/mtf_amd/csrc/mtfhip_grid_device.h
+++ b/mtf_amd/csrc/mtfhip_grid_device.h
@@ -82,7 +82,7 @@
 	for (int q = 0; q < 12; ++q) v[q] = readlane_f64(mine, q);
 }
 
-__device__ __forceinline__ void publish_target(const HostPublish &pub, int t, double wq, double sq, double cq, int n_it) {
+__device__ __forceinline__ void publish_target(const HostPublish &pub, int t, double wq, double sq, double cq, int n_it, int n_expected = 0) {
 	const int lane = threadIdx.x;
 	double *p = reinterpret_cast<double *>(pub.host);
 	const size_t Bt = (size_t)pub.B;
@@ -97,7 +97,7 @@
 	if (lane == 0) {
 		const int done = pub.fenced ? __hip_atomic_fetch_add(pub.count, 1, __ATOMIC_ACQ_REL, __HIP_MEMORY_SCOPE_AGENT)
 		                            : __hip_atomic_fetch_add(pub.count, 1, __ATOMIC_RELAXED, __HIP_MEMORY_SCOPE_AGENT);
-		if (done == (int)gridDim.x - 1) {
+		if (done == (n_expected ? n_expected : (int)gridDim.x) - 1) {
 			__hip_atomic_store(pub.count, 0, __ATOMIC_RELAXED, __HIP_MEMORY_SCOPE_AGENT);
 			if (pub.fenced) {
 				__threadfence_system();
diff --git a/mtf_amd/csrc/mtfhip_internal.h b/mtf_amd/csrc/mtfhip_internal.h
--- a/mtf_amd/csrc/mtfhip_internal.h
+++ b/mtf_amd/csrc/mtfhip_internal.h
@@ -100,6 +100,8 @@
 	double *state_last = nullptr;
 	int *need_mat = nullptr;
 	int lean_pass = 0;
+	int last_pass = 0;
+	int finish_prio = 0;
 };
 constexpr int kLmStride = 12;
 constexpr int kTraceStride = 96;
@@ -451,7 +453,9 @@
 	double hi_x, double hi_y, int force_unit_z, const void *src_host, void *dst, size_t bytes, int write_curr, hipStream_t st);
 struct PhaseCtl { unsigned long long *mine; const unsigned long long *other; double frac; };
 void launch_finish_track(const BatchView &bv, const mtfhip_sm_desc &sm, const TrackState &ts, const double *partials,
-	int nblk, hipStream_t st, PhaseCtl pc = PhaseCtl{nullptr, nullptr, 0.0});
+	int nblk, hipStream_t st, PhaseCtl pc = PhaseCtl{nullptr, nullptr, 0.0}, const HostPublish &pub = HostPublish{nullptr, 0, 0, nullptr, nullptr, 0, 0}, int pub_t0 = 0);
+struct LoopWords { int *zero_i; int n_zero_i; unsigned long long *phase; double *lm; int n_lm; double lm_delta_init; int *count; };
+void launch_track_prologue(const void *src_host, void *dst, size_t bytes, size_t skip_off, size_t skip_len, const LoopWords &lw, hipStream_t st);
 
 struct AlkArgs {
 	int ialk;
```

New measurement: 1.914 million iters/s, median of 6. 7.3% higher.
